# guowentian/dynamicppr

Measured on AMD Instinct MI355X. Metric: edge-updates/sec (ppr_throughput, summed over sources); ms_per_step = mean per-batch PPR update time, higher is better.
Workload: dtype f64

## Files before the change

dynamicppr_amd/csrc/dppr_engine.hip:

```cpp
#include <algorithm>
#include <atomic>
#include <cstdio>
#include <cstdlib>
#include <cstring>
#include <future>
#include <mutex>
#include <ctime>
#include <string>
#include <type_traits>
#include <unordered_map>
#include <vector>

#include <hip/hip_runtime.h>
#include <rocprim/rocprim.hpp>

#include "../../include/dppr.h"
#include "dppr_churn_plan.hpp"
#include "dppr_cut.hpp"
#include "dppr_devbuf.hpp"
#include "dppr_idspace.hpp"
#include "dppr_kernels.hpp"
#include "dppr_multi.hpp"
#include "dppr_gpush.hpp"
#include "dppr_binned.hpp"
#include "dppr_calib.hpp"
#include "dppr_topk.hpp"

using namespace dppr;

#include "dppr_host_state.hpp"
#include "dppr_host_graph.hpp"
#include "dppr_host_loop.hpp"
#include "dppr_host_group.hpp"
#include "dppr_host_query.hpp"


extern "C" {

int dppr_abi_version(void) { return DPPR_ABI_VERSION; }

const char *dppr_strerror(int status) {
    switch (status) {
    case DPPR_OK: return "ok";
    case DPPR_ERR_INVALID: return "invalid argument or call order";
    case DPPR_ERR_HIP: return "HIP runtime error";
    case DPPR_ERR_NOMEM: return "out of device memory";
    case DPPR_ERR_NO_DEVICE: return "no usable HIP device (the HIP path is mandatory; there is no CPU fallback)";
    case DPPR_ERR_NOT_CONVERGED: return "iteration cap hit before the frontier emptied";
    default: return "unknown status";
    }
}

const char *dppr_last_error(const dppr_engine *e) { return e ? e->err.c_str() : ""; }

int dppr_device_count(void) {
    int n = 0;
    return hipGetDeviceCount(&n) == hipSuccess ? n : 0;
}

int dppr_create(dppr_engine **out, int device, int32_t V, int32_t W, int directed, int32_t c, int32_t n_epochs) {
    if (!out || V <= 0 || W < 0 || c < 0 || n_epochs < 1) return DPPR_ERR_INVALID;
    *out = nullptr;
    int ndev = 0;
    if (hipGetDeviceCount(&ndev) != hipSuccess || ndev <= 0 || device < 0 || device >= ndev) return DPPR_ERR_NO_DEVICE;
    dppr_engine *e = new dppr_engine();
    dppr::g_live_engines.fetch_add(1, std::memory_order_relaxed);
    auto bail = [&](int code) {
        dppr_destroy(e);
        return code;
    };
#define HIP_TRY_C(call)                                                                 \
    do {                                                                                \
        const hipError_t _e = static_cast<hipError_t>(call);                            \
        if (_e != hipSuccess) {                                                         \
            fprintf(stderr, "dppr_create: %s at line %d\n", hipGetErrorString(_e), __LINE__); \
            return bail(_e == hipErrorOutOfMemory ? DPPR_ERR_NOMEM : DPPR_ERR_HIP);     \
        }                                                                               \
    } while (0)
    auto diag_env = [](const char *name) -> const char * {
        const char *v = getenv(name);
        if (v && !getenv("DPPR_QUIET_SWITCHES")) fprintf(stderr, "dppr_create: diagnostic switch %s=%s in effect (INTEGRATION.md, Environment variables)\n", name, v);
        return v;
    };
    if (const char *v = diag_env("DPPR_SWEEP_BITS")) e->sweep_bits = atoi(v) != 0;
    if (const char *v = diag_env("DPPR_HOT_BLOCKS")) e->hot_blocks = atoi(v) != 0;
    if (const char *v = diag_env("DPPR_GSWEEP_HOT")) e->gsweep_hot_rows = std::max(0, atoi(v));
    if (const char *v = diag_env("DPPR_GSWEEP_GRID")) e->gsweep_grid_cap = std::max(1, std::min(atoi(v), STAT_SLOTS));
    if (const char *v = diag_env("DPPR_RENUMBER")) e->renumber_on = atoi(v) != 0;
    if (const char *v = diag_env("DPPR_RENUMBER_PCT")) e->renumber_growth_pct = std::max(1, atoi(v));
    if (const char *v = diag_env("DPPR_RENUMBER_MIN")) e->renumber_min_parked = std::max(1, atoi(v));
    if (const char *v = diag_env("DPPR_GROUP_PUSH")) e->gpush_enter_pairs = std::max(-1, atoi(v));
    if (const char *v = diag_env("DPPR_GROUP_PUSH_FACTOR")) e->gpush_auto_factor = std::max(1, atoi(v));
    if (const char *v = diag_env("DPPR_GGROUPS_MIN")) e->ggroups_min = std::max(1, atoi(v));
    if (const char *v = diag_env("DPPR_COST_MODEL")) e->cost_model = atoi(v) != 0;
    if (const char *v = diag_env("DPPR_GROUPING_RADIX")) e->force_radix_grouping = atoi(v) != 0;
    if (const char *v = diag_env("DPPR_TEST_MERGE_MISS")) e->test_force_merge_miss = atoi(v) != 0;
    if (const char *v = diag_env("DPPR_BIN_INCREMENTAL")) e->bin_incremental = atoi(v) != 0;
    if (const char *v = diag_env("DPPR_BIN_RECUT_EVERY")) e->bin_recut_every = std::max(1, atoi(v));
    if (const char *v = diag_env("DPPR_BIN_FROZEN_REBUILD")) e->bin_frozen_rebuild = atoi(v) != 0;
    if (const char *v = diag_env("DPPR_GROUP_AT_SLIDE")) e->group_at_slide = atoi(v) != 0;
    if (const char *v = diag_env("DPPR_GROUP_FULL_ROWS")) e->group_full_rows = atoi(v) != 0;
    e->device = device;
    e->V = V;
    e->W = W;
    e->c = c;
    e->directed = directed ? 1 : 0;
    e->n_epochs = n_epochs;
    e->Ed = directed ? W : 2 * W;
    e->bits = 1;
    while ((1ll << e->bits) < (long long)V) e->bits++;
    HIP_TRY_C(hipSetDevice(device));
    HIP_TRY_C(hipStreamCreateWithFlags(&e->stream, hipStreamNonBlocking));
    {
        int least = 0, greatest = 0;
        if (hipDeviceGetStreamPriorityRange(&least, &greatest) != hipSuccess) least = 0;
        HIP_TRY_C(hipStreamCreateWithPriority(&e->bs, hipStreamNonBlocking, least));
    }
    HIP_TRY_C(hipEventCreate(&e->ev0));
    HIP_TRY_C(hipEventCreate(&e->ev1));
    for (auto &ev : e->evpool) HIP_TRY_C(hipEventCreate(&ev));
    HIP_TRY_C(e->dump_pin.alloc(dppr_engine::DUMP_PIN_BYTES));
    HIP_TRY_C(e->pinned.alloc((GMULTI_MAX + 2) * GS_MAX + 3 * GS_MAX + MAX_CHUNK * GS_MAX + 16));
    const size_t Wn = (size_t)std::max(W, 1), Edn = (size_t)std::max(e->Ed, 1), Ln = (size_t)std::max(4 * c, 1);
    HIP_TRY_C(e->w1.alloc(Wn));
    HIP_TRY_C(e->w2.alloc(Wn));
    HIP_TRY_C(e->outdeg.alloc((size_t)V));
    HIP_TRY_C(hipMemsetAsync(e->outdeg, 0, sizeof(int) * (size_t)V, e->stream));
    HIP_TRY_C(e->hub_slot_of.alloc((size_t)V));
    HIP_TRY_C(e->d_ext2int.alloc((size_t)V));
    HIP_TRY_C(e->d_xfer.alloc((size_t)V));
    e->init_ids(V);
    HIP_TRY_C(e->hub_hist.alloc(64));
    HIP_TRY_C(e->bar.alloc(1));
    HIP_TRY_C(e->keys_a.alloc(Edn));
    HIP_TRY_C(e->keys_b.alloc(Edn));
    HIP_TRY_C(e->in_sorted.alloc(Edn));
    if (e->directed) HIP_TRY_C(e->out_sorted.alloc(Edn));
    HIP_TRY_C(e->delpos.alloc((size_t)2 * (size_t)std::max(c, 1) + 16));
    {
        const size_t bn = (size_t)std::max(2 * c, 1);
        for (int k = 0; k < 4; ++k) {
            HIP_TRY_C(e->bk[k].alloc(bn));
            HIP_TRY_C(e->bks[k].alloc(bn));
        }
    }
    HIP_TRY_C(rocprim::radix_sort_keys(nullptr, e->sort_tmp_bytes, e->keys_a.get(), e->keys_b.get(), Edn, 0u,
                                       (unsigned)(2 * e->bits), e->stream));
    HIP_TRY_C(e->sort_tmp.alloc(std::max<size_t>(e->sort_tmp_bytes, 16)));
    for (int k = 0; k < 2; ++k) {
        HIP_TRY_C(e->su_k[k].alloc(Ln));
        HIP_TRY_C(e->su_v[k].alloc(Ln));
    }
    HIP_TRY_C(e->su_grp.alloc(4 * SU_GRP_MAX_BUCKETS + 8));
    HIP_TRY_C(hipMemsetAsync(e->su_grp, 0, sizeof(int) * (4 * SU_GRP_MAX_BUCKETS + 8), e->stream));
    HIP_TRY_C(e->su_term.alloc(Ln * GS_MAX));
    HIP_TRY_C(e->su_ins.alloc(Ln));
    HIP_TRY_C(rocprim::radix_sort_pairs(nullptr, e->su_tmp_bytes, e->su_k[0].get(), e->su_k[1].get(), e->su_v[0].get(), e->su_v[1].get(), Ln,
                                        0u, (unsigned)e->bits, e->stream));
    HIP_TRY_C(e->su_tmp.alloc(std::max<size_t>(e->su_tmp_bytes, 16)));
    e->epochs.resize((size_t)n_epochs);
    for (auto &ep : e->epochs) {
        HIP_TRY_C(ep.row_ptr.alloc((size_t)V + 1));
        HIP_TRY_C(ep.adj.alloc(Edn));
        HIP_TRY_C(ep.out_row_ptr.alloc((size_t)V + 1));
        HIP_TRY_C(ep.out_col.alloc(Edn));
        HIP_TRY_C(ep.b1.alloc(Ln));
        HIP_TRY_C(ep.b2.alloc(Ln));
        HIP_TRY_C(ep.deg_after.alloc(Ln));
        HIP_TRY_C(ep.ins.alloc(Ln));
        HIP_TRY_C(ep.sk.alloc(Ln));
        HIP_TRY_C(ep.sv.alloc(Ln));
        HIP_TRY_C(ep.grp_tile.alloc((size_t)V / WAVE + 3));
        HIP_TRY_C(ep.ggrp_tile.alloc((size_t)V / WAVE + 3));
        HIP_TRY_C(ep.hub_v.alloc(HUB_CAP));
        HIP_TRY_C(ep.hub_degp1.alloc(HUB_CAP));
    }
    HIP_TRY_C(hipStreamSynchronize(e->stream));
#undef HIP_TRY_C
    *out = e;
    return DPPR_OK;
}

void dppr_destroy(dppr_engine *e) {
    if (!e) return;
    if (e->pre.task.valid()) e->pre.task.wait();
    (void)hipSetDevice(e->device);
    if (e->stream) (void)hipStreamSynchronize(e->stream);
    if (e->bs) (void)hipStreamSynchronize(e->bs);
    if (e->ev0) (void)hipEventDestroy(e->ev0);
    if (e->ev1) (void)hipEventDestroy(e->ev1);
    for (auto &ev : e->evpool)
        if (ev) (void)hipEventDestroy(ev);
    if (e->stream) (void)hipStreamDestroy(e->stream);
    if (e->bs) (void)hipStreamDestroy(e->bs);
    dppr::g_live_engines.fetch_sub(1, std::memory_order_relaxed);
    delete e;
}

int dppr_set_schedule(dppr_engine *e, int schedule) {
    if (!e || (schedule != DPPR_SCHEDULE_EAGER && schedule != DPPR_SCHEDULE_SYNC)) return DPPR_ERR_INVALID;
    e->schedule = schedule;
    return DPPR_OK;
}

int dppr_set_batch_grouping(dppr_engine *e, int at_slide) {
    if (!e) return DPPR_ERR_INVALID;
    e->group_at_slide = at_slide != 0;
    return DPPR_OK;
}

int dppr_set_variant(dppr_engine *e, int variant) {
    if (!e || variant < 0 || variant > 3) return fail(e, DPPR_ERR_INVALID, "set_variant: 0 OPTIMIZED, 1 FAST_FRONTIER, 2 EAGER, 3 VANILLA");
    e->schedule = (variant == 1 || variant == 3) ? DPPR_SCHEDULE_SYNC : DPPR_SCHEDULE_EAGER;
    e->pre_extract = variant == 1 || variant == 3;
    e->status_dedup = variant == 2 || variant == 3;
    return DPPR_OK;
}

int dppr_set_phase_merge(dppr_engine *e, int on, int eps_divisor) {
    if (!e || eps_divisor < 0 || eps_divisor > 1024) return fail(e, DPPR_ERR_INVALID, "set_phase_merge: eps_divisor 1..1024 (0 keeps it)");
    e->merge_phases = on != 0;
    if (eps_divisor > 0) e->merge_div = eps_divisor;
    return DPPR_OK;
}

int dppr_set_profiling(dppr_engine *e, int on) {
    if (!e) return DPPR_ERR_INVALID;
    e->profiling = on != 0;
    return DPPR_OK;
}

int dppr_set_persistent(dppr_engine *e, int mode, int64_t timeout_us) {
    if (!e || mode < 0 || mode > 2 || e->loaded || !e->slots.empty())
        return fail(e, DPPR_ERR_INVALID, "set_persistent: call right after dppr_create, mode 0, 1 or 2");
    e->persist_mode = mode;
    if (timeout_us > 0) e->persist_ticks = (unsigned long long)timeout_us * 100ull;
    if (timeout_us < 0) {
        e->persist_ticks = 20000ull;
        e->persist_rollcall_extra = 1;
    }
    return DPPR_OK;
}

int dppr_set_tuning(dppr_engine *e, int hub_min_degree, int big_row_edges, int pull_min_frontier, int chunk_iters,
                    int pull_block) {
    if (!e || hub_min_degree < 1 || big_row_edges < 1 || e->loaded || !e->slots.empty())
        return fail(e, DPPR_ERR_INVALID, "set_tuning: call right after dppr_create, values >= 1");
    e->hub_min_degree = hub_min_degree;
    e->big_row = big_row_edges;
    e->pull_min_frontier = pull_min_frontier;
    if (chunk_iters > 0) {
        e->chunk_iters = std::min(chunk_iters, MAX_CHUNK);
        e->chunk_explicit = true;
    }
    if (pull_block >= 256 && pull_block <= 1024 && pull_block % 64 == 0) e->pull_block = pull_block;
    return DPPR_OK;
}

int dppr_set_sweep_bitmap(dppr_engine *e, int on) {
    if (!e) return DPPR_ERR_INVALID;
    e->sweep_bits = on != 0;
    return DPPR_OK;
}

int dppr_set_binned_sweep(dppr_engine *e, int mode, int ha_tiles, int hb_tiles, int64_t target_edges, int64_t min_ids, int64_t chunk_edges,
                          int64_t target_a_edges) {
    if (!e || mode < 0 || mode > 2 || ha_tiles < 0 || ha_tiles > BIN_MAX_HA_TILES || hb_tiles < 0 || hb_tiles > BIN_MAX_HB_TILES || target_edges < 0 || min_ids < 0 ||
        chunk_edges < 0 || target_a_edges < 0 || e->bin_ready || e->loaded)
        return fail(e, DPPR_ERR_INVALID, "set_binned_sweep: call right after dppr_create; mode 0..2, ha_tiles <= 272, hb_tiles <= 120");
    e->bin_mode = mode;
    if (ha_tiles > 0) e->bin_ha_tiles = ha_tiles;
    if (hb_tiles > 0) e->bin_hb_tiles = hb_tiles;
    if (target_edges > 0) e->bin_target = target_edges;
    if (min_ids > 0) e->bin_min_ids = min_ids;
    if (chunk_edges > 0) e->bin_chunk = chunk_edges;
    if (target_a_edges > 0) e->bin_target_a = target_a_edges;
    return DPPR_OK;
}

int dppr_set_resident_slots(dppr_engine *e, int sorted) {
    if (!e) return DPPR_ERR_INVALID;
    e->res_slots = sorted != 0;
    if (!e->res_slots)
        for (auto &ep : e->epochs) ep.res_valid = false;
    return DPPR_OK;
}

int dppr_set_resident_update(dppr_engine *e, int on) {
    if (!e) return DPPR_ERR_INVALID;
    e->res_update = on != 0;
    if (!e->res_update)
        for (auto &ep : e->epochs) ep.su_inline = false;
    return DPPR_OK;
}

int dppr_set_group_resident(dppr_engine *e, int on) {
    if (!e) return DPPR_ERR_INVALID;
    e->group_resident = on != 0;
    return DPPR_OK;
}

int dppr_set_group_push(dppr_engine *e, int enter_pairs, int list_cap, int64_t max_edges) {
    if (!e || enter_pairs < -1 || list_cap < 0 || max_edges < 0) return fail(e, DPPR_ERR_INVALID, "set_group_push: bad argument");
    e->gpush_enter_pairs = enter_pairs;
    if (list_cap > 0) e->gpush_list_cap = list_cap;
    e->gpush_max_edges = max_edges;
    return DPPR_OK;
}

int dppr_set_group_seeding(dppr_engine *e, int from_tails) {
    if (!e) return DPPR_ERR_INVALID;
    e->group_tail_seeding = from_tails != 0;
    return DPPR_OK;
}

int dppr_set_renumbering(dppr_engine *e, int on, int growth_pct, int min_parked) {
    if (!e || growth_pct < 0 || min_parked < 0) return fail(e, DPPR_ERR_INVALID, "set_renumbering: bad argument");
    e->renumber_on = on != 0;
    if (growth_pct > 0) e->renumber_growth_pct = growth_pct;
    if (min_parked > 0) e->renumber_min_parked = min_parked;
    e->renumber_next = std::min(e->renumber_next, renumber_threshold(e->n_int, e->renumber_growth_pct));
    return DPPR_OK;
}

int dppr_id_space(dppr_engine *e, int32_t *n_ids, int32_t *n_parked, int32_t *renumberings, int64_t *revivals) {
    if (!e) return DPPR_ERR_INVALID;
    if (n_ids) *n_ids = e->n_int;
    if (n_parked) *n_parked = e->n_parked;
    if (renumberings) *renumberings = e->renumberings;
    if (revivals) *revivals = e->revivals;
    return DPPR_OK;
}

int dppr_set_incremental_graph(dppr_engine *e, int on) {
    if (!e) return DPPR_ERR_INVALID;
    e->incremental = on != 0;
    return DPPR_OK;
}

int dppr_synchronize(dppr_engine *e) {
    if (!e) return DPPR_ERR_INVALID;
    HIP_TRY(hipSetDevice(e->device));
    HIP_TRY(hipStreamSynchronize(e->stream));
    HIP_TRY(hipStreamSynchronize(e->bs));
    return DPPR_OK;
}

int dppr_load_window(dppr_engine *e, const int32_t *e1, const int32_t *e2, int32_t n) {
    if (!e || n != e->W || (n > 0 && (!e1 || !e2))) return fail(e, DPPR_ERR_INVALID, "load_window: n must equal W");
    HIP_TRY(hipSetDevice(e->device));
    {
        std::vector<std::pair<uint64_t, int32_t>> fresh;
        for (int k = 0; k < 2; ++k) {
            const int32_t *a = k ? e2 : e1;
            for (int i = 0; i < n; ++i) {
                const int v = a[i];
                if (v < 0 || v >= e->V) return fail(e, DPPR_ERR_INVALID, "load_window: vertex id out of range");
                if (e->ext2int[(size_t)v] == -1) {
                    e->ext2int[(size_t)v] = -2;
                    fresh.emplace_back(id_hash(v), v);
                }
            }
        }
        std::vector<int32_t> indeg;
        if (fresh.size() > HOT_WINDOW_MIN) {
            indeg.assign((size_t)e->V, 0);
            for (int i = 0; i < n; ++i) {
                indeg[(size_t)e2[i]]++;
                if (!e->directed) indeg[(size_t)e1[i]]++;
            }
        }
        numbering_order(fresh, indeg.empty() ? nullptr : indeg.data(), e->hot_blocks);
        for (auto &kv : fresh) {
            e->ext2int[(size_t)kv.second] = -1;
            (void)to_int(e, kv.second);
        }
    }
    if (!translate(e, e1, n, e->h_tmp1) || !translate(e, e2, n, e->h_tmp2))
        return fail(e, DPPR_ERR_INVALID, "load_window: vertex id out of range");
    if (n > 0) {
        HIP_TRY(hipMemcpyAsync(e->w1, e->h_tmp1.data(), sizeof(int) * (size_t)n, hipMemcpyHostToDevice, e->bs));
        HIP_TRY(hipMemcpyAsync(e->w2, e->h_tmp2.data(), sizeof(int) * (size_t)n, hipMemcpyHostToDevice, e->bs));
    }
    e->head = 0;
    HIP_TRY(hipMemsetAsync(e->outdeg, 0, sizeof(int) * (size_t)e->V, e->bs));
    if (n > 0) {
        hipLaunchKernelGGL(k_deg_update, dim3(grid_for(n)), dim3(BLOCK), 0, e->bs, e->w1, e->w2, n, e->directed, 1,
                           e->outdeg);
        HIP_TRY(hipGetLastError());
    }
    for (auto &ep : e->epochs) ep.id = -1;
    Epoch &ep = e->epochs[0];
    ep.L = 0;
    ep.grouped = false;
    ep.su_inline = false;
    int rc = query_persist_cap(e);
    if (rc) return rc;
    rc = sort_window_full(e);
    if (rc) return rc;
    rc = build_epoch(e, ep);
    if (rc) return rc;
    ep.id = 0;
    e->newest = 0;
    e->renumber_next = renumber_threshold(e->n_int, e->renumber_growth_pct);
    e->loaded = true;
    e->batch_staged = false;
    HIP_TRY(hipStreamSynchronize(e->bs));
    return DPPR_OK;
}

int dppr_hint_next_batch(dppr_engine *e, const int32_t *b1, const int32_t *b2, int32_t L, const int32_t *n1, const int32_t *n2, int32_t c) {
    if (!e || e->broken || L < 0 || L > 4 * e->c || c < 0 || c > e->c || (L > 0 && (!b1 || !b2)) || (c > 0 && (!n1 || !n2))) return DPPR_ERR_INVALID;
    pre_join(e);
    dppr_engine::Pre &pr = e->pre;
    const int32_t *src[4] = {b1, b2, n1, n2};
    const int n[4] = {L, L, c, c};
    for (int k = 0; k < 4; ++k) {
        pr.src[k] = src[k];
        pr.n[k] = n[k];
        pr.out[k].resize((size_t)std::max(n[k], 1));
    }
    pr.epoch = e->renumber_epoch;
    pr.armed = true;
    pr.ok = false;
    pr.task = std::async(std::launch::async, [e] {
        bool ok = true;
        for (int k = 0; k < 4; ++k)
            if (e->pre.n[k] > 0) ok = e->lookup_only(e->pre.src[k], (size_t)e->pre.n[k], e->pre.out[k].data(), e->pre.miss[k]) && ok;
        return ok;
    });
    return DPPR_OK;
}

int dppr_set_batch(dppr_engine *e, const int32_t *b1, const int32_t *b2, const uint8_t *ins, int32_t L) {
    if (!e || e->broken || L < 0 || L > 4 * e->c || (L > 0 && (!b1 || !b2 || !ins)))
        return fail(e, DPPR_ERR_INVALID, "set_batch: length exceeds 4*max_batch");
    std::lock_guard<std::mutex> map_lk(e->map_mu);
    if (!ids_in_range(e, b1, L) || !ids_in_range(e, b2, L) || !translate(e, b1, L, e->st_b1) || !translate(e, b2, L, e->st_b2))
        return fail(e, DPPR_ERR_INVALID, "set_batch: vertex id out of range");
    e->st_b1.resize((size_t)L);
    e->st_b2.resize((size_t)L);
    e->st_ins.assign(ins, ins + L);
    e->batch_staged = true;
    HIP_TRY(hipSetDevice(e->device));
    return flush_moves(e);
}

static int slide_impl(dppr_engine *e, const int32_t *n1, const int32_t *n2, int32_t c, int32_t *out_epoch);

int dppr_slide(dppr_engine *e, const int32_t *n1, const int32_t *n2, int32_t c, int32_t *out_epoch) {
    if (e) e->build_concurrent = false;
    return slide_impl(e, n1, n2, c, out_epoch);
}

int dppr_slide_concurrent(dppr_engine *e, const int32_t *n1, const int32_t *n2, int32_t c, int32_t *out_epoch) {
    if (!e || e->n_epochs < 2) return fail(e, DPPR_ERR_INVALID, "slide_concurrent: needs n_epochs >= 2 (the epoch being built must not be the one being solved)");
    e->build_concurrent = true;
    const int rc = slide_impl(e, n1, n2, c, out_epoch);
    e->build_concurrent = false;
    return rc;
}

int dppr_renumbering_due(const dppr_engine *e) {
    return e && e->renumber_on && e->W > 0 && e->n_int >= e->renumber_next ? 1 : 0;
}

static int slide_impl(dppr_engine *e, const int32_t *n1, const int32_t *n2, int32_t c, int32_t *out_epoch) {
    if (!e || e->broken || !e->loaded || c < 0 || c > e->W || c > e->c || (c > 0 && (!n1 || !n2)))
        return fail(e, DPPR_ERR_INVALID, "slide: window not loaded, or c exceeds the window / max_batch of dppr_create");
    if (!ids_in_range(e, n1, c) || !ids_in_range(e, n2, c))
        return fail(e, DPPR_ERR_INVALID, "slide: vertex id out of range");
    HIP_TRY(hipSetDevice(e->device));
    const int W = e->W;
    static const bool slide_trace = getenv("DPPR_SLIDE_TRACE") != nullptr;
    timespec t_mark;
    clock_gettime(CLOCK_MONOTONIC, &t_mark);
    auto mark = [&](const char *what) {
        if (!slide_trace) return;
        (void)hipStreamSynchronize(e->bs);
        timespec now;
        clock_gettime(CLOCK_MONOTONIC, &now);
        fprintf(stderr, "[slide] %-34s %8.1f us\n", what, (now.tv_sec - t_mark.tv_sec) * 1e6 + (now.tv_nsec - t_mark.tv_nsec) * 1e-3);
        t_mark = now;
    };
    bool renumbered = false;
    {
        std::lock_guard<std::mutex> map_lk(e->map_mu);
        if (int rc = compact_ids(e, &renumbered)) return rc;
        if (renumbered) e->bin_words_valid = false;
        mark("renumbering check");
        if (!translate(e, n1, c, e->h_tmp1) || !translate(e, n2, c, e->h_tmp2))
            return fail(e, DPPR_ERR_INVALID, "slide: vertex id out of range");
        if (int rc = flush_moves(e)) return rc;
    }
    mark("translate new edges");
    n1 = e->h_tmp1.data();
    n2 = e->h_tmp2.data();
    const bool inc = e->incremental && c > 0 && 2 * c <= e->Ed && !renumbered;
    const int per = e->directed ? 1 : 2;
    int done = 0;
    while (done < c) {
        const int pos = (e->head + done) % W;
        const int len = std::min(c - done, W - pos);
        hipLaunchKernelGGL(k_deg_update, dim3(grid_for(len)), dim3(BLOCK), 0, e->bs, e->w1 + pos, e->w2 + pos, len,
                           e->directed, -1, e->outdeg);
        if (inc)
            hipLaunchKernelGGL(k_make_keys_seg, dim3(grid_for(len)), dim3(BLOCK), 0, e->bs, e->w1 + pos, e->w2 + pos,
                               len, e->directed, e->bits, e->bk[0] + (size_t)done * per, e->bk[2] + done);
        HIP_TRY(hipMemcpyAsync(e->w1 + pos, n1 + done, sizeof(int) * (size_t)len, hipMemcpyHostToDevice, e->bs));
        HIP_TRY(hipMemcpyAsync(e->w2 + pos, n2 + done, sizeof(int) * (size_t)len, hipMemcpyHostToDevice, e->bs));
        hipLaunchKernelGGL(k_deg_update, dim3(grid_for(len)), dim3(BLOCK), 0, e->bs, e->w1 + pos, e->w2 + pos, len,
                           e->directed, 1, e->outdeg);
        if (inc)
            hipLaunchKernelGGL(k_make_keys_seg, dim3(grid_for(len)), dim3(BLOCK), 0, e->bs, e->w1 + pos, e->w2 + pos,
                               len, e->directed, e->bits, e->bk[1] + (size_t)done * per, e->bk[3] + done);
        HIP_TRY(hipGetLastError());
        done += len;
    }
    if (W > 0) e->head = (e->head + c) % W;
    mark("ring, degrees, batch keys");
    const int id = e->newest + 1;
    Epoch &ep = e->epochs[id % e->n_epochs];
    ep.id = -1;
    ep.L = 0;
    ep.grouped = false;
    ep.su_inline = false;
    int rc;
    e->merge_miss_host = 0;
    if (inc) {
        HIP_TRY(hipMemsetAsync(e->hub_hist + MERGE_MISS_WORD, 0, sizeof(int), e->bs));
        rc = merge_batch_keys(e, e->in_sorted, e->bk[0], e->bks[0], c * per, e->bk[1], e->bks[1], c * per);
        if (!rc && e->directed) rc = merge_batch_keys(e, e->out_sorted, e->bk[2], e->bks[2], c, e->bk[3], e->bks[3], c);
        if (!rc) HIP_TRY(hipMemcpyAsync(&e->merge_miss_host, e->hub_hist + MERGE_MISS_WORD, sizeof(int), hipMemcpyDeviceToHost, e->bs));
    } else {
        rc = sort_window_full(e);
    }
    if (rc) return rc;
    mark("sorted keys (merge / full sort)");
    BinBatch bb;
    if (inc) {
        bb.del = e->bk[0];
        bb.ins = e->bk[1];
        bb.nd = bb.ni = c * per;
    }
    rc = build_epoch(e, ep, inc ? &bb : nullptr);
    if (rc) return rc;
    HIP_TRY(hipStreamSynchronize(e->bs));
    if (inc && (e->merge_miss_host != 0 || e->test_force_merge_miss)) {
        e->bin_force_full = true;
        e->merge_fallbacks++;
        rc = sort_window_full(e);
        if (rc) return rc;
        rc = build_epoch(e, ep);
        if (rc) return rc;
    }
    mark("hubs, CSRs, group cut + tables");
    ep.L = 0;
    ep.grouped = false;
    ep.max_bucket = 0;
    if (e->batch_staged) {
        const int L = (int)e->st_b1.size();
        ep.L = L;
        ep.max_bucket = largest_bucket(e->st_b1.data(), L);
        if (L > 0) {
            HIP_TRY(hipMemcpyAsync(ep.b1, e->st_b1.data(), sizeof(int) * (size_t)L, hipMemcpyHostToDevice, e->bs));
            HIP_TRY(hipMemcpyAsync(ep.b2, e->st_b2.data(), sizeof(int) * (size_t)L, hipMemcpyHostToDevice, e->bs));
            HIP_TRY(hipMemcpyAsync(ep.ins, e->st_ins.data(), (size_t)L, hipMemcpyHostToDevice, e->bs));
            if (e->group_at_slide) {
                hipLaunchKernelGGL(k_gather_deg, dim3(grid_for(L)), dim3(BLOCK), 0, e->bs, ep.b1, L, e->outdeg,
                                   ep.deg_after);
                HIP_TRY(hipGetLastError());
                if (int grc = epoch_group_records(e, ep)) return grc;
            }
        }
    }
    HIP_TRY(hipStreamSynchronize(e->bs));
    mark("batch records");
    e->batch_staged = false;
    ep.id = id;
    e->newest = id;
    if (out_epoch) *out_epoch = id;
    return DPPR_OK;
}

int dppr_add_source(dppr_engine *e, int32_t source, int32_t *out_slot) {
    if (!e || e->broken || source < 0 || source >= e->V) return fail(e, DPPR_ERR_INVALID, "add_source: vertex out of range");
    HIP_TRY(hipSetDevice(e->device));
    Slot s;
    s.source_ext = source;
    s.source = to_int(e, source);
    source = s.source;
    if (int rc = flush_moves(e)) return rc;
    const size_t V = (size_t)e->V;
    HIP_TRY(s.p.alloc(V));
    HIP_TRY(s.r.alloc(V));
    HIP_TRY(s.x.alloc(V));
    HIP_TRY(s.x2.alloc(V));
    HIP_TRY(hipMemsetAsync(s.x, 0, sizeof(double) * V, e->stream));
    HIP_TRY(hipMemsetAsync(s.x2, 0, sizeof(double) * V, e->stream));
    s.act_bytes = (V / 32 + 64) * sizeof(uint32_t);
    HIP_TRY(s.act[0].alloc(s.act_bytes / sizeof(uint32_t)));
    HIP_TRY(s.act[1].alloc(s.act_bytes / sizeof(uint32_t)));
    HIP_TRY(hipMemsetAsync(s.act[0], 0, s.act_bytes, e->stream));
    HIP_TRY(hipMemsetAsync(s.act[1], 0, s.act_bytes, e->stream));
    HIP_TRY(s.ft[0].alloc(V));
    HIP_TRY(s.ft[1].alloc(V));
    HIP_TRY(s.neg.alloc((size_t)std::max(4 * e->c, 1)));
    HIP_TRY(s.cnt.alloc(CNT_HDR + 2 * MAX_CHUNK));
    s.log = s.cnt + CNT_HDR;
// ... 516 lines not shown
    s.trace = on != 0;
    s.trace_ids.clear();
    s.trace_off.assign(1, 0);
    return DPPR_OK;
}

int dppr_trace_get(dppr_engine *e, int32_t slot, int64_t *n_iters, int64_t *n_ids, int64_t *offsets, int32_t *ids) {
    GET_SLOT(e, slot);
    const int64_t ni = s.trace_off.empty() ? 0 : (int64_t)s.trace_off.size() - 1;
    if (n_iters) *n_iters = ni;
    if (n_ids) *n_ids = (int64_t)s.trace_ids.size();
    if (offsets && !s.trace_off.empty()) memcpy(offsets, s.trace_off.data(), sizeof(int64_t) * s.trace_off.size());
    if (ids && !s.trace_ids.empty()) memcpy(ids, s.trace_ids.data(), sizeof(int32_t) * s.trace_ids.size());
    return DPPR_OK;
}

#define GET_GROUP(e, gid)                                                                             \
    if (!(e) || (gid) < 0 || (gid) >= (int)(e)->groups.size()) return fail((e), DPPR_ERR_INVALID, "bad group"); \
    if ((e)->broken) return fail((e), DPPR_ERR_INVALID, "engine unusable after a failed renumbering");           \
    Group &g = (e)->groups[(size_t)(gid)]

int dppr_add_source_group(dppr_engine *e, const int32_t *sources, int32_t n, int32_t *out_group) {
    if (!e || e->broken || !sources || n < 1 || n > GS_MAX) return fail(e, DPPR_ERR_INVALID, "add_source_group: 1..16 sources");
    if (!ids_in_range(e, sources, n)) return fail(e, DPPR_ERR_INVALID, "add_source_group: vertex out of range");
    HIP_TRY(hipSetDevice(e->device));
    Group g;
    g.n = n;
    g.gw = e->group_full_rows ? (n > OCT ? 2 * OCT : OCT) : row_width(n);
    g.spl = row_spl(g.gw);
    for (int s = 0; s < GS_MAX; ++s) g.src.s[s] = -1;
    for (int s = 0; s < n; ++s) g.src_ext[s] = sources[s];
    const size_t V = (size_t)e->V;
    g.act_bytes = (V / 32 + 1024 / 32 + 4) * sizeof(uint32_t);
    const size_t xw = (size_t)x_stride(g.gw);
    HIP_TRY_MSG("add_source_group: ", g.p.alloc((size_t)g.gw * V));
    HIP_TRY_MSG("add_source_group: ", g.r.alloc((size_t)g.gw * V));
    HIP_TRY_MSG("add_source_group: ", g.x.alloc(xw * V));
    HIP_TRY_MSG("add_source_group: ", g.x2.alloc(xw * V));
    HIP_TRY_MSG("add_source_group: ", g.act[0].alloc(g.act_bytes / sizeof(uint32_t)));
    HIP_TRY_MSG("add_source_group: ", g.act[1].alloc(g.act_bytes / sizeof(uint32_t)));
    HIP_TRY_MSG("add_source_group: ", g.cnt.alloc(5 * GS_MAX + MAX_CHUNK * GS_MAX));
    HIP_TRY_MSG("add_source_group: ", g.mlog.alloc((size_t)(GMULTI_MAX + 2) * GS_MAX));
    HIP_TRY_MSG("add_source_group: ", g.dstats.alloc(2));
    HIP_TRY_MSG("add_source_group: ", g.gq.alloc(3 * GQ_PAD));
    HIP_TRY_MSG("add_source_group: ", hipMemsetAsync(g.gq, 0, sizeof(int) * 3 * GQ_PAD, e->stream));
    HIP_TRY_MSG("add_source_group: ", hipMemsetAsync(g.act[0], 0, g.act_bytes, e->stream));
    HIP_TRY_MSG("add_source_group: ", hipMemsetAsync(g.act[1], 0, g.act_bytes, e->stream));
    HIP_TRY_MSG("add_source_group: ", hipMemsetAsync(g.cnt, 0, sizeof(int) * (5 * GS_MAX + MAX_CHUNK * GS_MAX), e->stream));
    HIP_TRY_MSG("add_source_group: ", hipMemsetAsync(g.dstats, 0, 2 * sizeof(IterStats), e->stream));
    for (int s = 0; s < n; ++s) (void)to_int(e, sources[s]);
    for (int s = 0; s < n; ++s) g.src.s[s] = e->ext2int[(size_t)sources[s]];
    if (int rc = flush_moves(e)) return rc;
    hipLaunchKernelGGL(k_ginit, dim3(grid_for((int64_t)e->V * g.gw)), dim3(BLOCK), 0, e->stream, g.p, g.r, e->V, g.gw, g.src);
    HIP_TRY_MSG("add_source_group: ", hipGetLastError());
    HIP_TRY_MSG("add_source_group: ", hipStreamSynchronize(e->stream));
    if (g.spl == 2) e->wide_groups = true;
    e->groups.push_back(std::move(g));
    e->any_groups = true;
    if (int rc = recut_stale_groups(e)) return rc;
    if (out_group) *out_group = (int)e->groups.size() - 1;
    return DPPR_OK;
}

int dppr_group_init_solve(dppr_engine *e, int32_t group, double eps, float *out_ms) {
    return dppr_group_init_solve_at(e, group, -1, eps, out_ms);
}

int dppr_group_init_solve_at(dppr_engine *e, int32_t group, int32_t epoch, double eps, float *out_ms) {
    GET_GROUP(e, group);
    GET_EPOCH(e, epoch);
    if (!(eps > 0)) return fail(e, DPPR_ERR_INVALID, "eps must be positive");
    HIP_TRY(hipSetDevice(e->device));
    HIP_TRY(hipEventRecord(e->ev0, e->stream));
    hipLaunchKernelGGL(k_ginit, dim3(grid_for((int64_t)e->V * g.gw)), dim3(BLOCK), 0, e->stream, g.p, g.r, e->V, g.gw, g.src);
    HIP_TRY(hipGetLastError());
    g.converged = false;
    g.park_eps = 0.0;
    int rc = group_loop(e, g, ep, 0, eps, false);
    if (rc) return rc;
    HIP_TRY(hipEventRecord(e->ev1, e->stream));
    HIP_TRY(hipEventSynchronize(e->ev1));
    float ms = 0;
    HIP_TRY(hipEventElapsedTime(&ms, e->ev0, e->ev1));
    if (out_ms) *out_ms = ms;
    g.converged = true;
    g.conv_eps = eps;
    g.last_epoch = ep.id;
    return DPPR_OK;
}

int dppr_group_update(dppr_engine *e, int32_t group, int32_t epoch, double eps, float *out_ms) {
    GET_GROUP(e, group);
    GET_EPOCH(e, epoch);
    if (!(eps > 0)) return fail(e, DPPR_ERR_INVALID, "eps must be positive");
    if (!epoch_in_sequence(g.last_epoch, ep.id)) return fail(e, DPPR_ERR_INVALID, "epoch out of sequence for this group");
    HIP_TRY(hipSetDevice(e->device));
    const bool merged = e->merge_phases && e->schedule == DPPR_SCHEDULE_EAGER;
    if (merged) eps = eps / e->merge_div;
    const bool tails = g.converged && g.conv_eps <= eps && e->group_tail_seeding;
    int rc = settle_parked(e, g.p, g.r, g.gw, eps, &g.park_eps, &g.st);
    if (rc) return rc;
    rc = prepare_epoch(e, ep);
    if (rc) return rc;
    HIP_TRY(hipEventRecord(e->ev0, e->stream));
    rc = group_stream_update(e, g, ep);
    if (rc) return rc;
    g.converged = false;
    if (merged) {
        rc = group_loop(e, g, ep, PHASE_BOTH, eps, tails);
        if (rc) return rc;
    } else {
        rc = group_loop(e, g, ep, 0, eps, tails);
        if (rc) return rc;
        rc = group_loop(e, g, ep, 1, eps, tails);
        if (rc) return rc;
    }
    HIP_TRY(hipEventRecord(e->ev1, e->stream));
    HIP_TRY(hipEventSynchronize(e->ev1));
    float ms = 0;
    HIP_TRY(hipEventElapsedTime(&ms, e->ev0, e->ev1));
    if (out_ms) *out_ms = ms;
    g.st.gpu_ms += ms;
    g.st.batches++;
    g.converged = true;
    g.conv_eps = eps;
    g.last_epoch = ep.id;
    return DPPR_OK;
}

int dppr_group_read(dppr_engine *e, int32_t group, int32_t index, double *p, double *r) {
    GET_GROUP(e, group);
    if (index < 0 || index >= g.n) return fail(e, DPPR_ERR_INVALID, "group_read: bad source index");
    HIP_TRY(hipSetDevice(e->device));
    std::lock_guard<std::mutex> map_lk(e->map_mu);
    int rc = sync_map(e);
    if (rc) return rc;
    const double *src[2] = {g.p, g.r};
    double *dst[2] = {p, r};
    for (int k = 0; k < 2; ++k) {
        if (!dst[k]) continue;
        hipLaunchKernelGGL(k_gint_to_ext, dim3(grid_for(e->V)), dim3(BLOCK), 0, e->stream, src[k], g.gw, index, e->d_ext2int,
                           e->V, e->d_xfer);
        HIP_TRY(hipMemcpyAsync(dst[k], e->d_xfer, sizeof(double) * (size_t)e->V, hipMemcpyDeviceToHost, e->stream));
        HIP_TRY(hipStreamSynchronize(e->stream));
    }
    return DPPR_OK;
}

static_assert(CHURN_LANES == GS_MAX, "dppr_churn_plan.hpp plans for the group size of dppr_multi.hpp");
static constexpr bool churn_geometry_agrees() {
    for (int n = 1; n <= GS_MAX; ++n)
        if (churn_row_width(n, false) != row_width(n) || churn_row_spl(row_width(n)) != row_spl(row_width(n)) ||
            churn_row_width(n, true) != (n > OCT ? 2 * OCT : OCT))
            return false;
    return true;
}
static_assert(churn_geometry_agrees(), "dppr_churn_plan.hpp restates row_width / row_spl of dppr_multi.hpp");

int dppr_group_sources(dppr_engine *e, int32_t group, int32_t *out_sources, int32_t *out_n) {
    GET_GROUP(e, group);
    if (out_sources)
        for (int s = 0; s < g.n; ++s) out_sources[s] = g.src_ext[s];
    if (out_n) *out_n = g.n;
    return DPPR_OK;
}

static int group_churn(dppr_engine *e, int32_t group, ChurnOp op, int32_t index, int32_t new_source, int32_t *out_index, float *out_ms) {
    static const char *const what[3] = {"group_replace_source", "group_add_source", "group_remove_source"};
    auto refuse = [&](const char *why) { return fail(e, DPPR_ERR_INVALID, (std::string(what[op]) + ": " + why).c_str()); };
    GET_GROUP(e, group);
    const ChurnPlan pl = churn_plan(op, g.n, g.gw, index, e->group_full_rows, e->wide_groups);
    if (!pl.ok) return refuse(op == CHURN_ADD ? "the group holds 16 sources" : op == CHURN_REMOVE && g.n <= 1 ? "the last source of a group cannot be removed" : "bad source index");
    if (op != CHURN_REMOVE && (new_source < 0 || new_source >= e->V)) return refuse("vertex out of range");
    if (!g.converged || g.last_epoch < 0) return refuse("the group is not converged (solve or update it first)");
    Epoch *epp = find_epoch(e, g.last_epoch);
    if (!epp) return refuse("the epoch the group was last solved on is not resident any more");
    const Epoch &ep = *epp;
    HIP_TRY(hipSetDevice(e->device));
    const size_t V = (size_t)e->V;
    const bool new_x = x_stride(pl.gw) != x_stride(g.gw);
    DevBuf<double> p2, r2, x_new, x2_new;
    if (pl.relayout) {
        HIP_TRY(p2.alloc((size_t)pl.gw * V));
        HIP_TRY(r2.alloc((size_t)pl.gw * V));
    }
    if (new_x) {
        HIP_TRY(x_new.alloc((size_t)x_stride(pl.gw) * V));
        HIP_TRY(x2_new.alloc((size_t)x_stride(pl.gw) * V));
    }
    int src_int = -1;
    if (op != CHURN_REMOVE) {
        (void)to_int(e, new_source);
        if (int rc = flush_moves(e)) return rc;
        src_int = e->ext2int[(size_t)new_source];
        if (pl.recut) e->wide_groups = true;
        if (int rc = recut_stale_groups(e)) return rc;
    }
    HIP_TRY(hipEventRecord(e->ev0, e->stream));
    if (pl.relayout) {
        ColMap cm;
        for (int s = 0; s < GS_MAX; ++s) cm.m[s] = pl.map[s];
        const int grid = grid_for((int64_t)e->V, BLOCK / pl.gw);
        hipLaunchKernelGGL(k_grow_remap, dim3(grid), dim3(BLOCK), 0, e->stream, p2.get(), g.p.get(), e->V, pl.gw, g.gw, cm);
        hipLaunchKernelGGL(k_grow_remap, dim3(grid), dim3(BLOCK), 0, e->stream, r2.get(), g.r.get(), e->V, pl.gw, g.gw, cm);
        HIP_TRY(hipGetLastError());
        g.p.swap(p2);
        g.r.swap(r2);
    }
    if (new_x) {
        g.x.swap(x_new);
        g.x2.swap(x2_new);
    }
    SrcN src;
    int src_ext[GS_MAX] = {0};
    for (int s = 0; s < GS_MAX; ++s) {
        src.s[s] = s < pl.n && pl.map[s] >= 0 ? g.src.s[pl.map[s]] : -1;
        src_ext[s] = s < pl.n && pl.map[s] >= 0 ? g.src_ext[pl.map[s]] : 0;
    }
    if (pl.lane >= 0) {
        src.s[pl.lane] = src_int;
        src_ext[pl.lane] = new_source;
    }
    g.src = src;
    memcpy(g.src_ext, src_ext, sizeof(src_ext));
    g.n = pl.n;
    g.gw = pl.gw;
    g.spl = pl.spl;
    if (pl.lane >= 0) {
        hipLaunchKernelGGL(k_gcol_init, dim3(grid_for(e->V)), dim3(BLOCK), 0, e->stream, g.p.get(), g.r.get(), e->V, g.gw, pl.lane, src_int);
        HIP_TRY(hipGetLastError());
        g.converged = false;
        if (int rc = group_solve_column(e, g, ep)) return rc;
    }
    HIP_TRY(hipEventRecord(e->ev1, e->stream));
    HIP_TRY(hipEventSynchronize(e->ev1));
    float ms = 0;
    HIP_TRY(hipEventElapsedTime(&ms, e->ev0, e->ev1));
    if (out_ms) *out_ms = ms;
    if (out_index) *out_index = pl.lane;
    g.converged = true;
    return DPPR_OK;
}

int dppr_group_replace_source(dppr_engine *e, int32_t group, int32_t index, int32_t new_source, float *out_ms) {
    return group_churn(e, group, CHURN_REPLACE, index, new_source, nullptr, out_ms);
}

int dppr_group_add_source(dppr_engine *e, int32_t group, int32_t new_source, int32_t *out_index, float *out_ms) {
    return group_churn(e, group, CHURN_ADD, -1, new_source, out_index, out_ms);
}

int dppr_group_remove_source(dppr_engine *e, int32_t group, int32_t index) {
    return group_churn(e, group, CHURN_REMOVE, index, -1, nullptr, nullptr);
}

static bool topk_args_ok(int32_t k, double min_p, const void *ids, const void *p, const void *cnt) {
    return k >= 1 && k <= DPPR_TOPK_MAX && min_p >= 0.0 && ids && p && cnt;
}
static bool read_at_args_ok(const dppr_engine *e, const int32_t *ids, int32_t m) {
    if (m < 0 || (m > 0 && !ids)) return false;
    for (int32_t i = 0; i < m; ++i)
        if (ids[i] < 0 || ids[i] >= e->V) return false;
    return true;
}

int dppr_topk(dppr_engine *e, int32_t slot, int32_t k, double min_p, int32_t *out_ids, double *out_p, double *out_r,
              int32_t *out_count) {
    GET_SLOT(e, slot);
    if (!topk_args_ok(k, min_p, out_ids, out_p, out_count))
        return fail(e, DPPR_ERR_INVALID, "topk: k in [1, DPPR_TOPK_MAX], min_p >= 0, non-null ids / p / count");
    std::lock_guard<std::mutex> map_lk(e->map_mu);
    return run_topk(e, s.p, s.r, 1, 1, k, min_p, out_ids, out_p, out_r, out_count);
}

int dppr_group_topk(dppr_engine *e, int32_t group, int32_t k, double min_p, int32_t *out_ids, double *out_p, double *out_r,
                    int32_t *out_counts) {
    GET_GROUP(e, group);
    if (!topk_args_ok(k, min_p, out_ids, out_p, out_counts))
        return fail(e, DPPR_ERR_INVALID, "group_topk: k in [1, DPPR_TOPK_MAX], min_p >= 0, non-null ids / p / counts");
    std::lock_guard<std::mutex> map_lk(e->map_mu);
    return run_topk(e, g.p, g.r, g.gw, g.n, k, min_p, out_ids, out_p, out_r, out_counts);
}

int dppr_read_at(dppr_engine *e, int32_t slot, const int32_t *ids, int32_t m, double *out_p, double *out_r) {
    GET_SLOT(e, slot);
    if (!read_at_args_ok(e, ids, m)) return fail(e, DPPR_ERR_INVALID, "read_at: ids in [0, V)");
    if (m == 0 || (!out_p && !out_r)) return DPPR_OK;
    std::lock_guard<std::mutex> map_lk(e->map_mu);
    return run_read_at(e, s.p, s.r, 1, 1, ids, m, out_p, out_r);
}

int dppr_group_read_at(dppr_engine *e, int32_t group, const int32_t *ids, int32_t m, double *out_p, double *out_r) {
    GET_GROUP(e, group);
    if (!read_at_args_ok(e, ids, m)) return fail(e, DPPR_ERR_INVALID, "group_read_at: ids in [0, V)");
    if (m == 0 || (!out_p && !out_r)) return DPPR_OK;
    std::lock_guard<std::mutex> map_lk(e->map_mu);
    return run_read_at(e, g.p, g.r, g.gw, g.n, ids, m, out_p, out_r);
}

int dppr_group_reset_stats(dppr_engine *e, int32_t group) {
    GET_GROUP(e, group);
    HIP_TRY(hipSetDevice(e->device));
    g.st = dppr_stats_t{};
    HIP_TRY(hipMemsetAsync(g.dstats, 0, 2 * sizeof(IterStats), e->stream));
    HIP_TRY(hipStreamSynchronize(e->stream));
    return DPPR_OK;
}

int dppr_group_stats(dppr_engine *e, int32_t group, dppr_stats_t *out) {
    GET_GROUP(e, group);
    if (!out) return DPPR_ERR_INVALID;
    HIP_TRY(hipSetDevice(e->device));
    static thread_local IterStats h[2];
    HIP_TRY(hipMemcpyAsync(h, g.dstats, sizeof(h), hipMemcpyDeviceToHost, e->stream));
    HIP_TRY(hipStreamSynchronize(e->stream));
    unsigned long long t = 0, ts = 0;
    for (int i = 0; i < STAT_SLOTS; ++i) {
        t += h[0].blk_E[i];
        ts += h[1].blk_E[i];
    }
    g.st.sum_E = (int64_t)(t + ts);
    g.st.sweep_E = (int64_t)ts;
    g.st.sum_N = g.st.sum_F;
    g.st.algorithmic_bytes = 8ll * g.st.inspected + 45ll * g.st.records + 72ll * g.st.sum_F + 24ll * g.st.sum_E +
                             4ll * g.st.sum_N;
    *out = g.st;
    return DPPR_OK;
}

#ifdef DPPR_STAMPS
extern "C" int dppr_debug_bin_stamps(unsigned long long *out, int which, int rows) {
    return hipMemcpyFromSymbol(out, HIP_SYMBOL(dppr::g_bin_stamps), sizeof(unsigned long long) * 6 * (size_t)rows,
                               sizeof(unsigned long long) * 6 * 16384 * (size_t)which) == hipSuccess ? 0 : -2;
}
extern "C" int dppr_debug_stamps(unsigned long long *out, int rows) {
    return hipMemcpyFromSymbol(out, HIP_SYMBOL(dppr::g_stamps), sizeof(unsigned long long) * 8 * (size_t)rows) == hipSuccess
               ? 0 : -2;
}
#endif

int dppr_bench_atomics(int device, int64_t table_elems, int64_t n, int scope, int reps, float *out_ms) {
    if (table_elems <= 0 || (table_elems & (table_elems - 1)) || n <= 0 || reps <= 0 || !out_ms) return DPPR_ERR_INVALID;
    int ndev = 0;
    if (hipGetDeviceCount(&ndev) != hipSuccess || device < 0 || device >= ndev) return DPPR_ERR_NO_DEVICE;
    if (hipSetDevice(device) != hipSuccess) return DPPR_ERR_HIP;
    DevBuf<double> table, sink;
    hipEvent_t a, b;
    if (table.alloc((size_t)table_elems) != 0) return DPPR_ERR_NOMEM;
    (void)sink.alloc(1);
    (void)hipMemset(table, 0, sizeof(double) * (size_t)table_elems);
    (void)hipEventCreate(&a);
    (void)hipEventCreate(&b);
    const int grid = 2048;
    auto launch = [&]() {
        if (scope == 2)
            hipLaunchKernelGGL(k_bench_scatter<0>, dim3(grid), dim3(BLOCK), 0, 0, table, (uint64_t)table_elems - 1, n);
        else if (scope == 3)
            hipLaunchKernelGGL(k_bench_scatter<1>, dim3(grid), dim3(BLOCK), 0, 0, table, (uint64_t)table_elems - 1, n);
        else if (scope == 0)
            hipLaunchKernelGGL(k_bench_atomics<__HIP_MEMORY_SCOPE_AGENT>, dim3(grid), dim3(BLOCK), 0, 0, table,
                               (uint64_t)table_elems - 1, n, sink);
        else
            hipLaunchKernelGGL(k_bench_atomics<__HIP_MEMORY_SCOPE_WORKGROUP>, dim3(grid), dim3(BLOCK), 0, 0, table,
                               (uint64_t)table_elems - 1, n, sink);
    };
    launch();
    (void)hipEventRecord(a, 0);
    for (int i = 0; i < reps; ++i) launch();
    (void)hipEventRecord(b, 0);
    hipError_t err = hipEventSynchronize(b);
    float ms = 0;
    (void)hipEventElapsedTime(&ms, a, b);
    *out_ms = ms / reps;
    (void)hipEventDestroy(a);
    (void)hipEventDestroy(b);
    return err == hipSuccess ? DPPR_OK : DPPR_ERR_HIP;
}

int dppr_bench_line_fills(int device, int64_t table_bytes, int64_t lines, int reps, float *out_ms) {
    if (table_bytes < 128 || (table_bytes & (table_bytes - 1)) || lines <= 0 || reps <= 0 || !out_ms) return DPPR_ERR_INVALID;
    int ndev = 0;
    if (hipGetDeviceCount(&ndev) != hipSuccess || device < 0 || device >= ndev) return DPPR_ERR_NO_DEVICE;
    if (hipSetDevice(device) != hipSuccess) return DPPR_ERR_HIP;
    DevBuf<double2> table;
    DevBuf<double> sink;
    if (table.alloc((size_t)table_bytes / sizeof(double2)) != 0) return DPPR_ERR_NOMEM;
    (void)sink.alloc(1);
    (void)hipMemset(table, 0, (size_t)table_bytes);
    hipEvent_t a, b;
    (void)hipEventCreate(&a);
    (void)hipEventCreate(&b);
    const int grid = 2048;
    const int per = (int)std::max<int64_t>(8, (lines + (int64_t)grid * 128 - 1) / ((int64_t)grid * 128) / 8 * 8);
    auto launch = [&]() {
        hipLaunchKernelGGL(k_bench_lines<8>, dim3(grid), dim3(1024), 0, 0, table, (uint64_t)(table_bytes / 128) - 1, per, sink);
    };
    launch();
    (void)hipEventRecord(a, 0);
    for (int i = 0; i < reps; ++i) launch();
    (void)hipEventRecord(b, 0);
    hipError_t err = hipEventSynchronize(b);
    float ms = 0;
    (void)hipEventElapsedTime(&ms, a, b);
    *out_ms = ms / reps * (float)((double)lines / ((double)grid * 128.0 * per));
    (void)hipEventDestroy(a);
    (void)hipEventDestroy(b);
    return err == hipSuccess ? DPPR_OK : DPPR_ERR_HIP;
}

int dppr_bench_stream_copy(int device, int64_t bytes, int reps, float *out_ms) {
    if (bytes < 16 || reps <= 0 || !out_ms) return DPPR_ERR_INVALID;
    int ndev = 0;
    if (hipGetDeviceCount(&ndev) != hipSuccess || device < 0 || device >= ndev) return DPPR_ERR_NO_DEVICE;
    if (hipSetDevice(device) != hipSuccess) return DPPR_ERR_HIP;
    DevBuf<unsigned char> src, dst;
    if (src.alloc((size_t)bytes) != 0 || dst.alloc((size_t)bytes) != 0) return DPPR_ERR_NOMEM;
    (void)hipMemset(src, 0, (size_t)bytes);
    (void)hipMemset(dst, 0, (size_t)bytes);
    hipEvent_t a, b;
    (void)hipEventCreate(&a);
    (void)hipEventCreate(&b);
    auto launch = [&]() { hipLaunchKernelGGL(k_bench_copy, dim3(4096), dim3(1024), 0, 0, reinterpret_cast<const double2 *>(src.get()),
                                            reinterpret_cast<double2 *>(dst.get()), bytes / 16); };
    launch();
    (void)hipEventRecord(a, 0);
    for (int i = 0; i < reps; ++i) launch();
    (void)hipEventRecord(b, 0);
    hipError_t err = hipEventSynchronize(b);
    float ms = 0;
    (void)hipEventElapsedTime(&ms, a, b);
    *out_ms = ms / reps;
    (void)hipEventDestroy(a);
    (void)hipEventDestroy(b);
    return err == hipSuccess ? DPPR_OK : DPPR_ERR_HIP;
}

int dppr_debug_bin_tables(dppr_engine *e, int32_t epoch, int32_t *n_a, int32_t *n_b, int32_t *n_edges, int32_t *n_runs, int32_t *n_tiles,
                          int32_t *acut, int32_t *bcut, uint16_t *hl, int32_t *tdelta, int32_t *tb, uint16_t *dl, int32_t *vb,
                          int64_t *patched, int64_t *rebuilt) {
    if (!e) return DPPR_ERR_INVALID;
    GET_EPOCH(e, epoch);
    if (patched) *patched = e->bin_patched;
    if (rebuilt) *rebuilt = e->bin_rebuilt;
    if (!ep.bin_valid) return fail(e, DPPR_ERR_INVALID, "debug_bin_tables: this epoch has no binned tables");
    HIP_TRY(hipSetDevice(e->device));
    if (n_a) *n_a = ep.n_a;
    if (n_b) *n_b = ep.n_b;
    if (n_edges) *n_edges = ep.Ed;
    if (n_runs) *n_runs = ep.n_runs;
    if (n_tiles) *n_tiles = ep.n_tiles;
    const size_t n_blk = ((size_t)ep.Ed + WAVE - 1) / WAVE, n_rb = ((size_t)ep.n_runs + WAVE - 1) / WAVE;
    if (acut) HIP_TRY(hipMemcpy(acut, ep.acut, sizeof(int) * ((size_t)ep.n_a + 1), hipMemcpyDeviceToHost));
    if (bcut) HIP_TRY(hipMemcpy(bcut, ep.bcut, sizeof(int) * ((size_t)ep.n_b + 1), hipMemcpyDeviceToHost));
    if (hl) HIP_TRY(hipMemcpy(hl, ep.hl, sizeof(uint16_t) * (size_t)ep.n_runs, hipMemcpyDeviceToHost));
    if (tdelta) HIP_TRY(hipMemcpy(tdelta, ep.tdelta, sizeof(int) * (size_t)ep.n_tiles, hipMemcpyDeviceToHost));
    if (tb) HIP_TRY(hipMemcpy(tb, ep.tb, sizeof(int) * (n_rb + 1), hipMemcpyDeviceToHost));
    if (dl) HIP_TRY(hipMemcpy(dl, ep.dl, sizeof(uint16_t) * (size_t)ep.Ed, hipMemcpyDeviceToHost));
    if (vb) HIP_TRY(hipMemcpy(vb, ep.vb, sizeof(int) * (n_blk + 1), hipMemcpyDeviceToHost));
    return DPPR_OK;
}

int dppr_debug_live_bytes(int64_t *device_bytes, int64_t *pinned_bytes) {
    if (device_bytes) *device_bytes = dppr::g_device_bytes.load(std::memory_order_relaxed);
    if (pinned_bytes) *pinned_bytes = dppr::g_pinned_bytes.load(std::memory_order_relaxed);
    return DPPR_OK;
}

unsigned long long dppr_heartbeat(const dppr_engine *e) { return e ? e->heartbeat.load(std::memory_order_relaxed) : 0ull; }

#ifndef DPPR_BUILD_ID
#define DPPR_BUILD_ID "unstamped"
#endif
const char *dppr_build_id(void) { return DPPR_BUILD_ID; }

}
```

dynamicppr_amd/csrc/dppr_host_group.hpp:

```cpp
#pragma once

namespace {

template <int N> using IC = std::integral_constant<int, N>;
template <class F>
void with_row(int gw, F &&f) {
    switch (gw) {
    case 2: f(IC<1>{}, IC<2>{}); break;
    case 4: f(IC<1>{}, IC<4>{}); break;
    case 6: f(IC<1>{}, IC<6>{}); break;
    case 8: f(IC<1>{}, IC<8>{}); break;
    case 10: f(IC<2>{}, IC<10>{}); break;
    case 12: f(IC<2>{}, IC<12>{}); break;
    case 14: f(IC<2>{}, IC<14>{}); break;
    default: f(IC<2>{}, IC<16>{}); break;
    }
}

int group_multi_capacity(dppr_engine *e, int spl) {
    int &cap = e->gmulti_cap[spl - 1];
    if (cap < 0) {
        int per_cu = 0, cus = 0;
        hipError_t rc = spl == 1 ? hipOccupancyMaxActiveBlocksPerMultiprocessor(&per_cu, k_gsweep<1, 8, 1024, true, 2>, GNT, 0)
                                 : hipOccupancyMaxActiveBlocksPerMultiprocessor(&per_cu, k_gsweep<2, 16, 512, true, 2>, GNT, 0);
        if (rc != hipSuccess || hipDeviceGetAttribute(&cus, hipDeviceAttributeMultiprocessorCount, e->device) != hipSuccess)
            per_cu = 0;
        cap = std::min(per_cu * cus, STAT_SLOTS);
    }
    return cap;
}

int group_push_tail(dppr_engine *e, Group &g, const Epoch &ep, int phase, double eps, long long pairs_at_entry, int *iters, bool *entered,
                    bool *converged, bool *owed) {
    *entered = false;
    *converged = false;
    const int GWM = GS_MAX;
    const int cap = std::max(1024, std::min(e->gpush_list_cap, e->V));
    if (g.plist[0].capacity() != (size_t)cap || !g.pctl) {
        HIP_TRY(loop_wait(e));
        g.plist[0].reset(); g.plist[1].reset(); g.ppre.reset(); g.pctl.reset();
        HIP_TRY(g.plist[0].alloc((size_t)cap));
        HIP_TRY(g.plist[1].alloc((size_t)cap));
        HIP_TRY(g.ppre.alloc((size_t)cap + 1));
        HIP_TRY(g.pctl.alloc(1));
    }
    static thread_local GPushCtl h;
    HIP_TRY(hipMemsetAsync(g.pctl, 0, sizeof(GPushCtl), e->stream));
    const int n_words = (ep.grp_n_int + 31) / 32;
    hipLaunchKernelGGL(k_gpush_list, dim3(grid_for(n_words)), dim3(BLOCK), 0, e->stream, g.act[0], n_words, g.plist[0], cap, g.pctl);
    const int rows_grid = grid_for(std::min<long long>(pairs_at_entry, cap), BLOCK / OCT);
    with_row(g.gw, [&](auto spl, auto gw) {
        hipLaunchKernelGGL((k_gpush_rows<decltype(spl)::value, decltype(gw)::value>), dim3(rows_grid), dim3(BLOCK), 0, e->stream, g.plist[0],
                           g.pctl, 0, g.x, g.r, false);
    });
    HIP_TRY(hipGetLastError());
    *entered = true;
    const int credit_first = *owed ? 1 : 0;
    const long long max_edges = e->gpush_max_edges > 0 ? e->gpush_max_edges : std::max<long long>(4096, 20ll * std::max(ep.n_ggroups, 1));
    const int grid = 256;
    static const bool trace = getenv("DPPR_GROUP_TRACE") != nullptr;
    int it_done = 0;
    long long known_n = pairs_at_entry;
    bool tiny_declined = false;
    long long last_adds = pairs_at_entry <= 64 ? 0 : -1;
    for (;;) {
        if (known_n <= TINY_N && last_adds >= 0 && last_adds <= TINY_E / 2 && !tiny_declined) {
            with_row(g.gw, [&](auto spl, auto gw) {
                hipLaunchKernelGGL((k_gpush_tiny<decltype(spl)::value, decltype(gw)::value>), dim3(1), dim3(1024), 0, e->stream, g.pctl, g.plist[0],
                                   g.plist[1], ep.row_ptr, ep.adj, ep.hub_degp1, g.r, g.p, g.act[0], phase, eps, g.dstats, GPUSH_LOG, credit_first);
            });
        } else {
        int m = 2;
        if (it_done == 0)
            for (long long f = pairs_at_entry; f > 128 && m < GPUSH_LOG; f >>= 2) ++m;
        tiny_declined = false;
        for (int k = 0; k < m; ++k) {
            hipLaunchKernelGGL(k_gpush_scan, dim3(1), dim3(1024), 0, e->stream, g.pctl, g.plist[0], g.plist[1], ep.row_ptr, g.ppre, cap - 1, max_edges);
            with_row(g.gw, [&](auto spl, auto gw) {
                constexpr int SPL = decltype(spl)::value, GW = decltype(gw)::value;
                hipLaunchKernelGGL((k_gpush_snap<SPL, GW>), dim3(grid), dim3(BLOCK), 0, e->stream, g.plist[0], g.plist[1], g.pctl, g.x, g.r, g.p,
                                   g.act[0], phase, eps, credit_first);
                hipLaunchKernelGGL((k_gpush_expand<SPL, GW>), dim3(grid), dim3(BLOCK), 0, e->stream, g.plist[0], g.plist[1], g.pctl, g.ppre,
                                   ep.row_ptr, ep.adj, ep.hub_degp1, g.x, g.r, g.act[0], g.plist[0], g.plist[1], cap, phase, eps, g.dstats);
            });
        }
        }
        HIP_TRY(hipGetLastError());
        HIP_TRY(hipMemcpyAsync(&h, g.pctl, sizeof(GPushCtl), hipMemcpyDeviceToHost, e->stream));
        HIP_TRY(loop_wait(e));
        for (int i = it_done; i < h.it; ++i) {
            long long F = 0;
            for (int s = 0; s < GWM; ++s) F += h.F[i & (GPUSH_LOG - 1)][s];
            if (F == 0) continue;
            g.st.iterations++;
            g.st.sum_F += F;
            ++*iters;
            if (trace)
                fprintf(stderr, "[gpush ] phase %d iteration +%d  frontier pairs %9lld  adds %lld\n", phase, i, F, h.atomics[i & (GPUSH_LOG - 1)]);
        }
        if (h.it == it_done && !h.stop && known_n <= TINY_N) tiny_declined = true;
        if (h.it > it_done) last_adds = h.atomics[(h.it - 1) & (GPUSH_LOG - 1)];
        it_done = h.it;
        known_n = h.n[h.it & 1];
        if (h.stop && h.it == 0 && h.overflow) {
            *entered = false;
            return DPPR_OK;
        }
        if (h.stop) {
            if (trace) fprintf(stderr, "[gpush ] phase %d: an iteration of %d vertices called itself off after %d iterations\n", phase, h.n[h.it & 1], h.it);
            HIP_TRY(hipMemsetAsync(g.cnt, 0, sizeof(int) * 3 * GWM, e->stream));
            with_row(g.gw, [&](auto spl, auto gw) {
                hipLaunchKernelGGL((k_gpush_leave<decltype(spl)::value, decltype(gw)::value>), dim3(grid_for(ep.grp_n_int, BLOCK / OCT)), dim3(BLOCK), 0,
                                   e->stream, ep.grp_n_int, g.act[0], g.x, g.r, g.p, h.it > 0 ? 1 : 0, phase, eps, g.cnt);
            });
            HIP_TRY(hipGetLastError());
            if (h.it > 0) *owed = false;
            return DPPR_OK;
        }
        if (h.n[h.it & 1] == 0) {
            *converged = true;
            return DPPR_OK;
        }
        if (it_done >= e->max_iters) return fail(e, DPPR_ERR_NOT_CONVERGED, "iteration cap hit");
    }
}

int group_loop(dppr_engine *e, Group &g, const Epoch &ep, int phase, double eps, bool tails) {
    const int hp = phase == PHASE_BOTH ? 0 : phase;
    int cur = 0;
    const int GWM = GS_MAX;
    HIP_TRY(hipMemsetAsync(g.cnt, 0, sizeof(int) * 3 * GWM, e->stream));
    if (tails) {
        HIP_TRY(hipMemsetAsync(g.act[0], 0, g.act_bytes, e->stream));
        if (ep.L > 0) {
            with_row(g.gw, [&](auto spl, auto gw) {
                hipLaunchKernelGGL((k_gseed_tails<decltype(spl)::value, decltype(gw)::value>), dim3(grid_for(ep.L, BLOCK / OCT)), dim3(BLOCK), 0,
                                   e->stream, batch_tails(e, ep), ep.L, g.r, g.x, g.p, g.act[0], phase, eps, g.cnt + cur * GWM);
            });
        }
    } else {
        with_row(g.gw, [&](auto spl, auto gw) {
            hipLaunchKernelGGL((k_gseed_dense<decltype(spl)::value, decltype(gw)::value>), dim3(grid_for(ep.grp_n_int, BLOCK / OCT)), dim3(BLOCK), 0,
                               e->stream, ep.grp_n_int, g.r, g.x, g.p, g.act[0], phase, eps, g.cnt + cur * GWM);
        });
        g.st.inspected += (int64_t)ep.grp_n_int * g.n;
    }
    HIP_TRY(hipGetLastError());
    int *log = g.cnt + 5 * GWM;
    auto any_left = [&](const int *c) {
        for (int s = 0; s < GWM; ++s)
            if (c[s] > 0) return true;
        return false;
    };
    HIP_TRY(hipMemcpyAsync(e->pinned, g.cnt + cur * GWM, sizeof(int) * GWM, hipMemcpyDeviceToHost, e->stream));
    HIP_TRY(loop_wait(e));
    bool more = any_left(e->pinned);
    int active_iters = 0;
    if (e->gsweep_grid_cap <= 0) {
        int cus = 0;
        if (hipDeviceGetAttribute(&cus, hipDeviceAttributeMultiprocessorCount, e->device) != hipSuccess || cus <= 0) cus = 256;
        e->gsweep_grid_cap = std::min(2 * cus, STAT_SLOTS);
    }
    const int sweep_grid = std::min(std::max(ep.n_ggroups, 1), e->gsweep_grid_cap);
    int follow = 4;
    bool owed = false;
    long long push_thr = e->gpush_enter_pairs == 0 ? 0 : e->gpush_enter_pairs > 0 ? e->gpush_enter_pairs : std::max(64, ep.n_ggroups * e->gpush_auto_factor);
    bool push_gave_up = false;
    int dense_len = -1;
    const int nvx = ep.ggrp_max_tiles * WAVE;
    for (int it = 0; more;) {
        if (it >= e->max_iters) return fail(e, DPPR_ERR_NOT_CONVERGED, "iteration cap hit");
        const int mcap = e->group_resident && e->persist_mode && e->persist_ok && e->chunk_iters > 1 ? group_multi_capacity(e, g.spl) : 0;
        if (mcap > 0 && ep.n_ggroups > 0 && ep.n_ggroups <= mcap) {
            int n = g.iter_hint[hp] > it ? g.iter_hint[hp] - it + RESIDENT_MARGIN : 2 * e->chunk_iters;
            n = std::max(2, std::min(n, GMULTI_MAX));
            if (e->chunk_explicit) n = std::min(n, std::max(e->chunk_iters, 2));
            HIP_TRY(hipMemsetAsync(g.mlog, 0, sizeof(int) * (size_t)(n + 2) * GWM, e->stream));
            HIP_TRY(hipMemsetAsync(e->bar, 0, sizeof(GridBar), e->stream));
            if (e->profiling) HIP_TRY(hipEventRecord(e->evpool[0], e->stream));
            int *status = g.mlog, *rows = g.mlog + GWM;
#define DPPR_LAUNCH_GMULTI(SPL, GW, NVX)                                                                                 \
    hipLaunchKernelGGL((k_gsweep<SPL, GW, NVX, true, 2>), dim3(ep.n_ggroups), dim3(GNT), 0, e->stream, ep.grp_n_int, ep.gtab,   \
                       ep.n_ggroups, g.cnt + cur * GWM, e->gsweep_hot_rows, ep.out_col, g.x, g.x2, g.act[0], g.act[1], g.r, g.p, \
                       g.cnt + 3 * GWM, g.cnt + 4 * GWM, phase, eps, g.dstats + 1, rows, n, e->bar, status, e->persist_ticks,    \
                       e->persist_rollcall_extra, owed ? 1 : 0, (int *)nullptr, (int *)nullptr)
            with_row(g.gw, [&](auto spl, auto gw) {
                constexpr int SPL = decltype(spl)::value, GW = decltype(gw)::value;
                if constexpr (SPL == 2) DPPR_LAUNCH_GMULTI(2, GW, 512);
                else if (nvx == 512) DPPR_LAUNCH_GMULTI(1, GW, 512);
                else DPPR_LAUNCH_GMULTI(1, GW, 1024);
            });
#undef DPPR_LAUNCH_GMULTI
            if (e->profiling) HIP_TRY(hipEventRecord(e->evpool[1], e->stream));
            HIP_TRY(hipGetLastError());
            HIP_TRY(hipMemcpyAsync(e->pinned, g.mlog, sizeof(int) * (size_t)(n + 2) * GWM, hipMemcpyDeviceToHost, e->stream));
            HIP_TRY(loop_wait(e));
            const int st = e->pinned[0];
            g.st.persist_launches++;
            if (st & GSM_FAULT) return fail(e, DPPR_ERR_HIP, "a grid barrier of the multi-sweep group launch timed out");
            if (st & GSM_ABORTED) {
                g.st.persist_aborts++;
                e->persist_ok = false;
                e->persist_retry = PERSIST_RETRY_BATCHES;
                continue;
            }
            const int sweeps = st & GSM_SWEEPS;
            for (int k = 0; k < sweeps; ++k) {
                const int *f = e->pinned + GWM + k * GWM;
                g.st.iterations++;
                g.st.pull_iterations++;
                for (int s = 0; s < GWM; ++s) g.st.sum_F += f[s];
                for (int s = 0; s < GWM; ++s) g.st.sweep_F += f[s];
                active_iters = it + k + 1;
            }
            if (e->profiling) {
                float ms = 0;
                HIP_TRY(hipEventElapsedTime(&ms, e->evpool[0], e->evpool[1]));
                g.st.push_ms += ms;
                g.st.push_launches++;
            }
            if (sweeps & 1) {
                std::swap(g.x, g.x2);
                std::swap(g.act[0], g.act[1]);
                owed = !owed;
            }
            it += sweeps;
            if (st & GSM_CONVERGED) break;
            HIP_TRY(hipMemcpyAsync(g.cnt, g.cnt + 3 * GWM, sizeof(int) * GWM, hipMemcpyDeviceToDevice, e->stream));
            HIP_TRY(hipMemsetAsync(g.cnt + GWM, 0, sizeof(int) * 2 * GWM, e->stream));
            cur = 0;
            more = any_left(e->pinned + GWM + sweeps * GWM);
            continue;
        }
        int n;
        if (it == 0) {
            int lo = 0;
            for (int h : (push_thr > 0 ? g.dense_hist : g.iter_hist)[hp]) lo = h > 0 && (lo == 0 || h < lo) ? h : lo;
            n = lo > 0 ? lo : e->chunk_iters;
            follow = 4;
        } else if (push_thr > 0 && !push_gave_up) {
            long long F = 0;
            for (int s = 0; s < GWM; ++s) F += e->pinned[cur * GWM + s];
            n = 1;
            for (long long f = F / 4; f > push_thr && n < e->chunk_iters; f /= 4) ++n;
        } else {
            n = std::min(follow, e->chunk_iters);
            follow *= 2;
        }
        if (e->chunk_explicit) n = std::min(n, std::max(e->chunk_iters, 1));
        n = std::max(1, std::min(n, MAX_CHUNK));
        for (int k = 0; k < n; ++k) {
            const int nxt = (cur + 1) % 3, zer = (cur + 2) % 3;
            if (e->profiling) HIP_TRY(hipEventRecord(e->evpool[2 * k], e->stream));
#define DPPR_LAUNCH_GSWEEP(SPL, GW, NVX) do { if (owed) DPPR_LAUNCH_GSWEEP_CM(SPL, GW, NVX, 1); else DPPR_LAUNCH_GSWEEP_CM(SPL, GW, NVX, 0); } while (0)
#define DPPR_LAUNCH_GSWEEP_CM(SPL, GW, NVX, CM)                                                                          \
    hipLaunchKernelGGL((k_gsweep<SPL, GW, NVX, false, CM>), dim3(sweep_grid), dim3(GNT), 0, e->stream, ep.grp_n_int, ep.gtab,  \
                       ep.n_ggroups, g.cnt + cur * GWM, e->gsweep_hot_rows, ep.out_col, g.x, g.x2, g.act[0], g.act[1], g.r, g.p,  \
                       g.cnt + nxt * GWM, g.cnt + zer * GWM, phase, eps, g.dstats + 1, log + k * GWM, 1, (GridBar *)nullptr,      \
                       (int *)nullptr, 0ull, 0, owed ? 1 : 0, g.gq + (g.gq_seq % 3) * GQ_PAD, g.gq + ((g.gq_seq + 1) % 3) * GQ_PAD)
            with_row(g.gw, [&](auto spl, auto gw) {
                constexpr int SPL = decltype(spl)::value, GW = decltype(gw)::value;
                if constexpr (SPL == 2) DPPR_LAUNCH_GSWEEP(2, GW, 512);
                else if (nvx == 512) DPPR_LAUNCH_GSWEEP(1, GW, 512);
                else DPPR_LAUNCH_GSWEEP(1, GW, 1024);
            });
#undef DPPR_LAUNCH_GSWEEP
#undef DPPR_LAUNCH_GSWEEP_CM
            if (e->profiling) HIP_TRY(hipEventRecord(e->evpool[2 * k + 1], e->stream));
            std::swap(g.x, g.x2);
            std::swap(g.act[0], g.act[1]);
            cur = nxt;
            g.gq_seq++;
            owed = !owed;
        }
        HIP_TRY(hipGetLastError());
        HIP_TRY(hipMemcpyAsync(e->pinned, g.cnt, sizeof(int) * (size_t)(5 * GWM + n * GWM), hipMemcpyDeviceToHost,
                               e->stream));
        HIP_TRY(loop_wait(e));
        for (int k = 0; k < n; ++k) {
            const int *f = e->pinned + 5 * GWM + k * GWM;
            if (!any_left(f)) continue;
            if (push_thr > 0 && dense_len < 0) {
                long long F = 0;
                for (int s = 0; s < GWM; ++s) F += f[s];
                if (F <= push_thr) dense_len = it + k;
            }
            g.st.iterations++;
            g.st.pull_iterations++;
            for (int s = 0; s < GWM; ++s) g.st.sum_F += f[s];
            for (int s = 0; s < GWM; ++s) g.st.sweep_F += f[s];
            active_iters = it + k + 1;
            if (e->profiling) {
                float ms = 0;
                HIP_TRY(hipEventElapsedTime(&ms, e->evpool[2 * k], e->evpool[2 * k + 1]));
                g.st.push_ms += ms;
                g.st.push_launches++;
                g.st.sweep_ms += ms;
                g.st.sweep_launches++;
                static const bool trace = getenv("DPPR_GROUP_TRACE") != nullptr;
                if (trace) {
                    long long F = 0;
                    for (int s = 0; s < GWM; ++s) F += f[s];
                    fprintf(stderr, "[gsweep] phase %d sweep %3d  frontier pairs %9lld  %7.1f us\n", phase, it + k, F, ms * 1e3);
                }
            }
        }
        more = any_left(e->pinned + cur * GWM);
        it += n;
        if (more && push_thr > 0 && !push_gave_up) {
            long long F = 0;
            for (int s = 0; s < GWM; ++s) F += e->pinned[cur * GWM + s];
            if (F <= push_thr) {
                if (dense_len < 0) dense_len = it;
                int pushed = 0;
                bool entered = false, conv = false;
                int rc = group_push_tail(e, g, ep, phase, eps, F, &pushed, &entered, &conv, &owed);
                if (rc) return rc;
                if (entered) {
                    active_iters = it + pushed;
                    it += pushed;
                    if (conv) more = false;
                    else {
                        cur = 0;
                        HIP_TRY(hipMemcpyAsync(e->pinned, g.cnt, sizeof(int) * GWM, hipMemcpyDeviceToHost, e->stream));
                        HIP_TRY(loop_wait(e));
                        more = any_left(e->pinned);
                        push_thr = std::max<long long>(F / 8, 1);
                        dense_len = -1;
                    }
                } else {
                    push_thr = std::max<long long>(F / 8, 1);
                    dense_len = -1;
                }
            }
        }
    }
    if (push_thr > 0) {
        for (int k = 3; k > 0; --k) g.dense_hist[hp][k] = g.dense_hist[hp][k - 1];
        g.dense_hist[hp][0] = dense_len >= 0 ? std::max(dense_len, 1) : std::max(active_iters, 1);
    }
    g.iter_hint[hp] = active_iters;
    for (int k = 3; k > 0; --k) g.iter_hist[hp][k] = g.iter_hist[hp][k - 1];
    g.iter_hist[hp][0] = active_iters;
    return DPPR_OK;
}

int group_solve_column(dppr_engine *e, Group &g, const Epoch &ep) {
    int hint[2], hist[2][4], dense[2][4];
    memcpy(hint, g.iter_hint, sizeof(hint));
    memcpy(hist, g.iter_hist, sizeof(hist));
    memcpy(dense, g.dense_hist, sizeof(dense));
    const int rc = group_loop(e, g, ep, 0, g.conv_eps, false);
    memcpy(g.iter_hint, hint, sizeof(hint));
    memcpy(g.iter_hist, hist, sizeof(hist));
    memcpy(g.dense_hist, dense, sizeof(dense));
    return rc;
}

int group_stream_update(dppr_engine *e, Group &g, const Epoch &ep) {
    const int L = ep.L;
    if (L == 0) return DPPR_OK;
    int rc = group_records_by_tail(e, ep, nullptr, 0, nullptr, 0);
    if (rc) return rc;
    SuSources srcs{};
    for (int s = 0; s < GS_MAX; ++s) srcs.s[s] = g.src.s[s];
    hipLaunchKernelGGL(k_su_terms, dim3(grid_for(L), g.n), dim3(BLOCK), 0, e->stream, batch_tails(e, ep), batch_order(e, ep), ep.b2,
                       ep.ins, L, g.p, g.gw, e->su_term, e->su_ins);
    hipLaunchKernelGGL(k_su_apply, dim3(grid_for(L), g.n), dim3(BLOCK), 0, e->stream, batch_tails(e, ep), batch_order(e, ep), e->su_term,
                       e->su_ins, ep.deg_after, L, g.r, g.gw, srcs, 0.0, (int *)nullptr, (int *)nullptr, (int *)nullptr,
                       (int *)nullptr);
    HIP_TRY(hipGetLastError());
    g.st.records += (int64_t)L * g.n;
    return DPPR_OK;
}

}
```

dynamicppr_amd/csrc/dppr_host_state.hpp:

```cpp
#pragma once

static constexpr int MAX_CHUNK = 64;
static constexpr int CNT_HDR = 16;
static constexpr int PERSIST_RETRY_BATCHES = 64;
static constexpr int GMULTI_MAX = 2 * MAX_CHUNK;
static constexpr int GQ_PAD = 32;
static constexpr int BIN_MAX_BLOCKS = 1 << 16, BIN_MAX_BIG = 4096, BIN_SMALL_INTS = BIN_MAX_BLOCKS + BIN_MAX_BIG + 1 + 64;
static constexpr int SU_SPLIT_MIN = 1 << 16;
static constexpr int MERGE_MISS_WORD = 44;
static constexpr int RESIDENT_MARGIN = 8;

namespace dppr {

inline std::atomic<long long> g_device_bytes{0}, g_pinned_bytes{0};

struct DeviceAlloc {
    static int alloc(void **p, size_t bytes) {
        const hipError_t rc = hipMalloc(p, bytes);
        if (rc == hipSuccess) g_device_bytes.fetch_add((long long)bytes, std::memory_order_relaxed);
        return (int)rc;
    }
    static int free(void *p, size_t bytes) {
        g_device_bytes.fetch_sub((long long)bytes, std::memory_order_relaxed);
        return (int)hipFree(p);
    }
};

struct PinnedAlloc {
    static int alloc(void **p, size_t bytes) {
        const hipError_t rc = hipHostMalloc(p, bytes, hipHostMallocDefault);
        if (rc == hipSuccess) g_pinned_bytes.fetch_add((long long)bytes, std::memory_order_relaxed);
        return (int)rc;
    }
    static int free(void *p, size_t bytes) {
        g_pinned_bytes.fetch_sub((long long)bytes, std::memory_order_relaxed);
        return (int)hipHostFree(p);
    }
};

template <class T> using DevBuf = Buf<T, DeviceAlloc>;
template <class T> using PinBuf = Buf<T, PinnedAlloc>;

}

namespace {

struct Epoch {
    DevBuf<int> row_ptr;
    DevBuf<Adj> adj;
    DevBuf<int> out_row_ptr;
    DevBuf<int> out_col;
    int Ed = 0;
    DevBuf<int> b1, b2, deg_after;
    DevBuf<uint8_t> ins;
    int L = 0;
    DevBuf<uint32_t> sk, sv;
    int max_bucket = 0;
    bool grouped = false;
    int id = -1;
    DevBuf<int> grp_tile;
    int n_groups = 0;
    int grp_n_int = 0;
    DevBuf<int> ggrp_tile;
    int n_ggroups = 0;
    int ggrp_max_tiles = 0;
    DevBuf<int> gtab;
    DevBuf<int> hub_v, hub_degp1;
    int n_hubs = 0;
    DevBuf<int> acut; int *bcut = nullptr;
    int n_a = 0, n_b = 0;
    DevBuf<BinChunk> chunks;
    int n_chunks = 0;
    DevBuf<uint16_t> hl, dl;
    DevBuf<int> vb, tb;
    DevBuf<int> tdelta;
    int n_runs = 0, n_tiles = 0;
    bool bin_valid = false;
    int bin_n_int = 0;
    DevBuf<uint32_t> res_pk;
    bool res_valid = false;
    DevBuf<int> su_rng;
    bool su_inline = false;
};

struct Slot {
    int source = 0;
    int source_ext = 0;
    DevBuf<double> p, r;
    DevBuf<double> x, x2;
    DevBuf<uint32_t> act[2];
    size_t act_bytes = 0;
    DevBuf<int> ft[2];
    DevBuf<int> neg;
    DevBuf<int> status;
    DevBuf<int> cnt;
    DevBuf<BigItem> big;
    int *log = nullptr;
    long long iter_seq = 0;
    double sweep_us = 0;
    double atomic_ns = 1.0 / 23.5;
    int iter_hint[2] = {0, 0};
    int iter_hist[2][4] = {{0, 0, 0, 0}, {0, 0, 0, 0}};
    bool start_dense[2] = {false, false};
    int last_F0[2] = {0, 0};
    DevBuf<IterStats> dstats;
    bool converged = false;
    double conv_eps = 0.0;
    double park_eps = 0.0;
    int last_epoch = -2;
    bool seed_lists_valid = false;
    bool phase0_done = false;
    double phase0_eps = 0.0;
    dppr_stats_t st{};
    bool trace = false;
    std::vector<int64_t> trace_off;
    std::vector<int32_t> trace_ids;
};

struct Group {
    int n = 0;
    int spl = 1;
    int gw = OCT;
    int src_ext[GS_MAX] = {0};
    SrcN src{};
    DevBuf<double> p, r, x, x2;
    DevBuf<uint32_t> act[2];
    size_t act_bytes = 0;
    DevBuf<int> cnt;
    DevBuf<int> gq;
    unsigned gq_seq = 0;
    DevBuf<int> mlog;
    DevBuf<IterStats> dstats;
    dppr_stats_t st{};
    int iter_hint[2] = {0, 0};
    int iter_hist[2][4] = {{0, 0, 0, 0}, {0, 0, 0, 0}};
    int dense_hist[2][4] = {{0, 0, 0, 0}, {0, 0, 0, 0}};
    DevBuf<int> plist[2];
    DevBuf<int> ppre;
    DevBuf<GPushCtl> pctl;
    bool converged = false;
    double conv_eps = 0.0;
    double park_eps = 0.0;
    int last_epoch = -2;
};

}

struct dppr_engine : dppr::IdSpace {
    int device = 0;
    int V = 0, W = 0, c = 0, directed = 1, n_epochs = 1;
    int Ed = 0;
    int bits = 1;
    int schedule = DPPR_SCHEDULE_EAGER;
    bool status_dedup = false;
    bool pre_extract = false;
    bool group_at_slide = false;
    int merge_miss_host = 0;
    long long merge_fallbacks = 0;
    bool test_force_merge_miss = false;
    bool launch_called_off = false;
    int raw_backoff = 0;
    bool merge_phases = false;
    int merge_div = 4;
    hipStream_t stream = nullptr;
    hipStream_t bs = nullptr;
    bool build_concurrent = false;
    std::mutex err_mu;
    std::mutex map_mu;
    unsigned map_gen_on_device = 0;
    hipEvent_t ev0 = nullptr, ev1 = nullptr;
    hipEvent_t evpool[2 * 64] = {};
    bool profiling = false;
    int pull_block = 0;
    int chunk_iters = 24;
    bool chunk_explicit = false;
    int persist_mode = 1;
    bool persist_ok = true;
    int persist_retry = 0;
    int persist_cap = 0;
    int res_slots = 1;
    int res_update = 1;
    DevBuf<double> res_arena;
    long long res_arena_stride = 0;
    unsigned long long persist_ticks = 5000000ull;
    int persist_rollcall_extra = 0;
    DevBuf<GridBar> bar;
    DevBuf<int> w1, w2;
    int head = 0;
    bool loaded = false;
    bool broken = false;
    DevBuf<int> outdeg;
    DevBuf<int> hub_slot_of;
    DevBuf<int> hub_hist;
    int hub_min_degree = HUB_MIN_DEGREE_DEFAULT;
    int big_row = BIG_ROW_DEFAULT;
    int pull_min_frontier = 0;
    DevBuf<uint64_t> in_sorted, out_sorted;
    DevBuf<uint64_t> keys_a, keys_b;
    DevBuf<unsigned char> sort_tmp;
    size_t sort_tmp_bytes = 0;
    DevBuf<int> su_grp;
    DevBuf<uint64_t> bk[4];
    DevBuf<uint64_t> bks[4];
    DevBuf<int> delpos;
    struct Pre {
        std::future<bool> task;
        const int32_t *src[4] = {nullptr, nullptr, nullptr, nullptr};
        int n[4] = {0, 0, 0, 0};
        std::vector<int32_t> out[4];
        std::vector<uint32_t> miss[4];
        unsigned long long epoch = 0;
        bool armed = false, ok = false;
    } pre;
    long long pre_hits = 0, pre_misses = 0;
    bool incremental = true;
    bool sweep_bits = false;
    bool hot_blocks = true;
    int gsweep_hot_rows = 24576;
    int gsweep_grid_cap = 0;
    bool group_resident = true;
    int gmulti_cap[2] = {-1, -1};
    bool any_groups = false;
    int ggroups_min = 256;
    bool force_radix_grouping = false;
    bool cost_model = true;
    bool group_full_rows = false;
    bool wide_groups = false;
    bool group_tail_seeding = true;
    int gpush_enter_pairs = -1;
    int gpush_list_cap = 1 << 20;
    long long gpush_max_edges = 0;
    int gpush_auto_factor = 2;
    int bin_mode = 1;
    int bin_ha_tiles = 128, bin_hb_tiles = 60;
    long long bin_target = 0;
    long long bin_target_a = 4ll << 20;
    long long bin_min_ids = 1ll << 19;
    DevBuf<int> bin_vblk_a;
    DevBuf<unsigned long long> bin_scan;
    DevBuf<int> bin_small;
    long long bin_chunk = 32768;
    DevBuf<double> bin_vals;
    DevBuf<uint64_t> bin_wb, bin_wa;
    DevBuf<int> bin_first;
    std::vector<int32_t> bin_cut_a, bin_cut_b;
    int bin_abits = 0, bin_bbits = 0;
    int bin_cut_ids = 0;
    bool bin_words_valid = false;
    int bin_slides_since_cut = 0;
    bool bin_incremental = true;
    int bin_recut_every = 32;
    bool bin_frozen_rebuild = false;
    bool bin_force_full = false;
    int bin_miss_host = 0;
    long long bin_patched = 0, bin_rebuilt = 0;
    DevBuf<unsigned char> bin_tmp;
    size_t bin_tmp_bytes = 0;
    bool bin_ready = false;
    std::vector<int32_t> h_tiles_in;
    DevBuf<uint32_t> su_k[2], su_v[2];
    DevBuf<double> su_term;
    DevBuf<uint8_t> su_ins;
    DevBuf<unsigned char> su_tmp;
    size_t su_tmp_bytes = 0;
    std::vector<int32_t> st_b1, st_b2;
    std::vector<uint8_t> st_ins;
    bool batch_staged = false;
    std::vector<Epoch> epochs;
    int newest = -1;
    std::vector<Slot> slots;
    std::vector<Group> groups;
    PinBuf<int> pinned;
    std::atomic<unsigned long long> heartbeat{0};
    PinBuf<char> dump_pin;
    static constexpr size_t DUMP_PIN_BYTES = sizeof(GridBar) + 4096;
    bool renumber_on = true;
    int renumber_growth_pct = 15;
    int renumber_min_parked = 1024;
    int renumber_next = 0;
    int renumberings = 0;
    std::vector<int32_t> mv_src, mv_dst, mv_zero;
    DevBuf<int> mv_idx;
    DevBuf<double> mv_tmp;
    DevBuf<int> d_ext2int;
    DevBuf<double> d_xfer;
    DevBuf<int> d_int2ext;
    unsigned i2e_gen_on_device = 0;
    DevBuf<unsigned char> tk_ws;
    DevBuf<unsigned long long> tk_out_key;
    DevBuf<int> tk_out_row;
    DevBuf<int> tk_cand;
    DevBuf<unsigned char> tk_res; PinBuf<unsigned char> tk_pin;
    DevBuf<unsigned char> ra_buf;
    std::vector<int32_t> h_tmp1, h_tmp2;
    std::vector<int32_t> h_tiles;
    int max_iters = 1 << 20;
    std::string err;
};

namespace {

inline void set_err(dppr_engine *e, const char *msg) {
    std::lock_guard<std::mutex> lk(e->err_mu);
    e->err = msg;
}

#define HIP_TRY(call)                                                                                   \
    do {                                                                                                \
        const hipError_t _e = static_cast<hipError_t>(call);                                            \
        if (_e != hipSuccess) {                                                                         \
            char _b[512];                                                                               \
            snprintf(_b, sizeof(_b), "%s in %s at line %d", hipGetErrorString(_e), __FILE__, __LINE__); \
            set_err(e, _b);                                                                             \
            return _e == hipErrorOutOfMemory ? DPPR_ERR_NOMEM : DPPR_ERR_HIP;                           \
        }                                                                                               \
    } while (0)

#define HIP_TRY_MSG(prefix, call)                                                 \
    do {                                                                          \
        const hipError_t _e = static_cast<hipError_t>(call);                      \
        if (_e != hipSuccess) {                                                   \
            set_err(e, (std::string(prefix) + hipGetErrorString(_e)).c_str());    \
            return _e == hipErrorOutOfMemory ? DPPR_ERR_NOMEM : DPPR_ERR_HIP;     \
        }                                                                         \
    } while (0)

inline int grid_for(int64_t n, int per_block = BLOCK, int cap = 2048) {
    int64_t g = (n + per_block - 1) / per_block;
    if (g < 1) g = 1;
    if (g > cap) g = cap;
    return (int)g;
}

constexpr long LOOP_SPIN_US = 2000;
inline hipError_t loop_sync(hipStream_t st) {
    static const bool spin = !(getenv("DPPR_SYNC_SPIN") && atoi(getenv("DPPR_SYNC_SPIN")) == 0);
    if (!spin) return hipStreamSynchronize(st);
    timespec t0;
    clock_gettime(CLOCK_MONOTONIC, &t0);
    hipError_t r;
    unsigned polls = 0;
    while ((r = hipStreamQuery(st)) == hipErrorNotReady) {
        if ((++polls & 15u) == 0) {
            timespec now;
            clock_gettime(CLOCK_MONOTONIC, &now);
            if ((now.tv_sec - t0.tv_sec) * 1000000L + (now.tv_nsec - t0.tv_nsec) / 1000L > LOOP_SPIN_US) return hipStreamSynchronize(st);
        }
        __builtin_ia32_pause();
    }
    return r;
}

inline hipError_t loop_wait(dppr_engine *e) {
    e->heartbeat.fetch_add(1, std::memory_order_relaxed);
    return loop_sync(e->stream);
}

int fail(dppr_engine *e, int code, const char *msg) {
    if (e) set_err(e, msg);
    return code;
}

inline void pre_join(dppr_engine *e) {
    if (e->pre.task.valid()) e->pre.ok = e->pre.task.get();
}

inline int to_int(dppr_engine *e, int ext) {
    pre_join(e);
    return e->to_int(ext);
}

int pre_find(dppr_engine *e, const int32_t *src, int n) {
    pre_join(e);
    if (!e->pre.armed || !e->pre.ok || e->pre.epoch != e->renumber_epoch || n <= 0) return -1;
    for (int k = 0; k < 4; ++k)
        if (e->pre.src[k] == src && e->pre.n[k] == n) {
            const std::vector<int32_t> &o = e->pre.out[k];
            const int step = std::max(1, n / 64);
            for (int i = 0; i < n; i = (i + step < n || i == n - 1) ? i + step : n - 1) {
                const int m = o[(size_t)i];
                if (m >= 0 && (m >= (int)e->int2ext.size() || e->int2ext[(size_t)m] != src[i])) {
                    e->pre.armed = false;
                    return -1;
                }
                if (i == n - 1) break;
            }
            return k;
        }
    return -1;
}

bool ids_in_range(dppr_engine *e, const int32_t *src, int n) {
    if (pre_find(e, src, n) >= 0) return true;
    for (int i = 0; i < n; ++i)
        if (src[i] < 0 || src[i] >= e->V) return false;
    return true;
}

bool translate(dppr_engine *e, const int32_t *src, int n, std::vector<int32_t> &dst) {
    const int k = pre_find(e, src, n);
    if (k >= 0) {
        e->pre.src[k] = nullptr;
        dst.swap(e->pre.out[k]);
        e->resolve(src, dst.data(), e->pre.miss[k]);
        e->pre_hits++;
        e->pre_misses += (long long)e->pre.miss[k].size();
        return true;
    }
    if (n > 0) e->pre.armed = false;
    dst.resize((size_t)std::max(n, 1));
    return e->translate(src, (size_t)std::max(n, 0), dst.data());
}

}
```

dynamicppr_amd/csrc/dppr_multi.hpp:

```cpp
#pragma once

#include "dppr_kernels.hpp"

namespace dppr {

constexpr int GS_MAX = 16;
constexpr int OCT = 8;

struct SrcN {
    int s[GS_MAX];
};

__device__ __forceinline__ unsigned oct_mask(uint64_t ballot) {
    return (unsigned)(ballot >> (lane_id() & ~(OCT - 1))) & 0xffu;
}

__host__ __device__ constexpr int row_width(int n_sources) { return n_sources <= 2 ? 2 : (n_sources + 1) / 2 * 2; }
__host__ __device__ constexpr int row_spl(int gw) { return gw > OCT ? 2 : 1; }
#ifndef DPPR_X_COMPACT
#define DPPR_X_COMPACT 0
#endif
__host__ __device__ constexpr int x_stride(int gw) { return DPPR_X_COMPACT ? gw : gw > 8 ? 16 : gw > 4 ? 8 : gw; }
template <int SPL, int GW>
__device__ __forceinline__ bool oct_live(int j) {
    static_assert(GW >= 2 && GW <= OCT * SPL && GW % 2 == 0 && (SPL == 1 || GW > OCT), "row width / lane split");
    if constexpr (GW == OCT * SPL) return true;
    else return j * SPL < GW;
}

__global__ __launch_bounds__(BLOCK) void k_ginit(double *__restrict__ p, double *__restrict__ r, int V, int gw, SrcN src) {
    const int64_t n = (int64_t)V * gw;
    for (int64_t i = (int64_t)blockIdx.x * BLOCK + threadIdx.x; i < n; i += (int64_t)gridDim.x * BLOCK) {
        const int v = (int)(i / gw), s = (int)(i % gw);
        p[i] = 0.0;
        r[i] = (src.s[s] == v) ? 1.0 : 0.0;
    }
}

template <int SPL, int GW>
__global__ __launch_bounds__(BLOCK) void k_gseed_dense(int V, const double *__restrict__ r, double *__restrict__ x,
                                                       double *__restrict__ p, uint32_t *__restrict__ act, int phase,
                                                       double eps, int *__restrict__ cnt_out) {
    __shared__ int s_cnt[GS_MAX];
    if (threadIdx.x < GS_MAX) s_cnt[threadIdx.x] = 0;
    __syncthreads();
    const int j = threadIdx.x & (OCT - 1);
    const bool live = oct_live<SPL, GW>(j);
    int nleg[SPL];
#pragma unroll
    for (int q = 0; q < SPL; ++q) nleg[q] = 0;
    uint8_t *act8 = reinterpret_cast<uint8_t *>(act);
    const int vper = BLOCK / OCT;
    const int Vpad = (V + 7) & ~7;
    for (int vb = blockIdx.x * vper; vb < Vpad; vb += gridDim.x * vper) {
        const int v = vb + (int)threadIdx.x / OCT;
        bool any = false;
        double rv[SPL];
        bool lg[SPL];
#pragma unroll
        for (int q = 0; q < SPL; ++q) {
            rv[q] = v < V && live ? r[(size_t)v * GW + j * SPL + q] : 0.0;
            lg[q] = v < V && live && legal(rv[q], phase, eps);
            any |= lg[q];
            nleg[q] += lg[q] ? 1 : 0;
        }
        const uint64_t bal = __ballot(any);
        const unsigned m = oct_mask(bal);
        if (m && live) {
#pragma unroll
            for (int q = 0; q < SPL; ++q) {
                const size_t i = (size_t)v * GW + j * SPL + q;
                x[(size_t)v * x_stride(GW) + j * SPL + q] = rv[q];
                if (lg[q]) p[i] = p[i] + ALPHA * rv[q];
            }
        }
        if (lane_id() == 0) {
            unsigned byte = 0;
#pragma unroll
            for (int k = 0; k < 8; ++k) byte |= ((bal >> (k * OCT)) & 0xffull) ? (1u << k) : 0u;
            const int v0 = vb + wave_id() * 8;
            if (v0 < Vpad) act8[v0 >> 3] = (uint8_t)byte;
        }
    }
#pragma unroll
    for (int q = 0; q < SPL; ++q)
        if (nleg[q]) atomicAdd(&s_cnt[j * SPL + q], nleg[q]);
    __syncthreads();
    if (threadIdx.x < GW && s_cnt[threadIdx.x]) atomicAdd(&cnt_out[threadIdx.x], s_cnt[threadIdx.x]);
}

template <int SPL, int GW>
__global__ __launch_bounds__(BLOCK) void k_gseed_tails(const uint32_t *__restrict__ skeys, int L, const double *__restrict__ r,
                                                       double *__restrict__ x, double *__restrict__ p,
                                                       uint32_t *__restrict__ act, int phase, double eps,
                                                       int *__restrict__ cnt_out) {
    __shared__ int s_cnt[GS_MAX];
    if (threadIdx.x < GS_MAX) s_cnt[threadIdx.x] = 0;
    __syncthreads();
    const int j = threadIdx.x & (OCT - 1);
    const bool live = oct_live<SPL, GW>(j);
    int nleg[SPL];
#pragma unroll
    for (int q = 0; q < SPL; ++q) nleg[q] = 0;
    const int per = BLOCK / OCT;
    const int Lpad = (L + per - 1) / per * per;
    for (int i0 = blockIdx.x * per; i0 < Lpad; i0 += gridDim.x * per) {
        const int i = i0 + (int)threadIdx.x / OCT;
        int u = -1;
        if (i < L) {
            u = (int)skeys[i];
            if (i > 0 && (int)skeys[i - 1] == u) u = -1;
        }
        bool any = false;
        double rv[SPL];
        bool lg[SPL];
#pragma unroll
        for (int q = 0; q < SPL; ++q) {
            rv[q] = u >= 0 && live ? r[(size_t)u * GW + j * SPL + q] : 0.0;
            lg[q] = u >= 0 && live && legal(rv[q], phase, eps);
            any |= lg[q];
            nleg[q] += lg[q] ? 1 : 0;
        }
        if (oct_mask(__ballot(any))) {
            if (live) {
#pragma unroll
                for (int q = 0; q < SPL; ++q) {
                    const size_t k = (size_t)u * GW + j * SPL + q;
                    x[(size_t)u * x_stride(GW) + j * SPL + q] = rv[q];
                    if (lg[q]) p[k] = p[k] + ALPHA * rv[q];
                }
            }
            if (j == 0) atomicOr(&act[u >> 5], 1u << (u & 31));
        }
    }
#pragma unroll
    for (int q = 0; q < SPL; ++q)
        if (nleg[q]) atomicAdd(&s_cnt[j * SPL + q], nleg[q]);
    __syncthreads();
    if (threadIdx.x < GW && s_cnt[threadIdx.x]) atomicAdd(&cnt_out[threadIdx.x], s_cnt[threadIdx.x]);
}

constexpr int GNT = 1024;
constexpr int GT_HDR = 8;
__host__ __device__ constexpr int GT_STRIDE(int nvx) { return (GT_HDR + nvx + 1 + GNT / OCT + nvx / 2 + 3) / 4 * 4; }

template <int NVX>
__global__ __launch_bounds__(GNT) void k_gtables(int V, const int *__restrict__ grp_tile, int n_groups,
                                                 const int *__restrict__ out_row_ptr, int *__restrict__ tables) {
    constexpr int NW = GNT / WAVE, NOCT = GNT / OCT, EB = 8;
    __shared__ int s_wcnt[NW];
    const int tid = threadIdx.x, lane = lane_id(), w = wave_id();
    for (int g = blockIdx.x; g < n_groups; g += gridDim.x) {
        __syncthreads();
        int *T = tables + (size_t)g * GT_STRIDE(NVX);
        const int t0 = grp_tile[g], t1 = grp_tile[g + 1];
        const int v0 = t0 * WAVE;
        const int nv = min((t1 - t0) * WAVE, V - v0);
        const int E0 = out_row_ptr[v0];
        const int Eg = out_row_ptr[v0 + nv] - E0;
        int rs = 0, d = 0;
        if (tid < nv) {
            rs = out_row_ptr[v0 + tid] - E0;
            d = out_row_ptr[v0 + tid + 1] - E0 - rs;
        }
        const int per = ((Eg + NOCT - 1) / NOCT + EB - 1) / EB * EB;
        const uint64_t ne = __ballot(d > 0);
        if (lane == 0) s_wcnt[w] = __popcll(ne);
        __syncthreads();
        int woff = 0, ncomp = 0;
#pragma unroll
        for (int k = 0; k < NW; ++k) {
            const int c = s_wcnt[k];
            woff += k < w ? c : 0;
            ncomp += c;
        }
        int *cstart = T + GT_HDR, *ostart = T + GT_HDR + NVX + 1;
        unsigned short *cvid = reinterpret_cast<unsigned short *>(T + GT_HDR + NVX + 1 + NOCT);
        if (tid <= NVX && tid >= ncomp) cstart[tid] = Eg;
        if (tid == 0 && NVX >= GNT) cstart[NVX] = Eg;
        if (tid < NOCT) ostart[tid] = 0;
        if (tid < NVX && tid >= ncomp) cvid[tid] = 0;
        if (tid == 0) {
            T[0] = v0; T[1] = nv; T[2] = E0; T[3] = Eg; T[4] = per; T[5] = ncomp; T[6] = 0; T[7] = 0;
        }
        asm volatile("s_waitcnt vmcnt(0)" ::: "memory");
        __syncthreads();
        if (d > 0) {
            const int idx = woff + mbcnt(ne);
            cstart[idx] = rs;
            cvid[idx] = (unsigned short)tid;
            const int o_first = (rs + per - 1) / per, o_last = min((rs + d + per - 1) / per - 1, NOCT - 1);
            for (int o = o_first; o <= o_last; ++o) ostart[o] = idx;
        }
    }
}

template <bool COH>
__device__ __forceinline__ double gs_ld(const double *p) {
    if constexpr (COH)
        return __longlong_as_double((long long)__hip_atomic_load(reinterpret_cast<const unsigned long long *>(p),
                                                                 __ATOMIC_RELAXED, __HIP_MEMORY_SCOPE_AGENT));
    else
        return *p;
}
template <bool COH>
__device__ __forceinline__ uint32_t gs_ldu(const uint32_t *p) {
    if constexpr (COH) return __hip_atomic_load(p, __ATOMIC_RELAXED, __HIP_MEMORY_SCOPE_AGENT);
    else return *p;
}
template <bool COH>
__device__ __forceinline__ void gs_st(double *p, double v) {
    if constexpr (COH)
        __hip_atomic_store(reinterpret_cast<unsigned long long *>(p), (unsigned long long)__double_as_longlong(v),
                           __ATOMIC_RELAXED, __HIP_MEMORY_SCOPE_AGENT);
    else
        *p = v;
}
template <bool COH>
__device__ __forceinline__ void gs_stu(uint32_t *p, uint32_t v) {
    if constexpr (COH) __hip_atomic_store(p, v, __ATOMIC_RELAXED, __HIP_MEMORY_SCOPE_AGENT);
    else *p = v;
}

#ifndef DPPR_GS_NT
#define DPPR_GS_NT 0
#endif
#ifndef DPPR_WHATIF
#define DPPR_WHATIF 0
#endif
template <bool COH, int BIT>
__device__ __forceinline__ double gs_ld_once(const double *p) {
    if constexpr (!COH && (DPPR_GS_NT & BIT)) return __builtin_nontemporal_load(p);
    else return gs_ld<COH>(p);
}
template <bool COH, int BIT>
__device__ __forceinline__ void gs_st_once(double *p, double v) {
    if constexpr (!COH && (DPPR_GS_NT & BIT)) __builtin_nontemporal_store(v, p);
    else gs_st<COH>(p, v);
}

constexpr int GSM_ABORTED = 1 << 30;
constexpr int GSM_FAULT = 1 << 29;
constexpr int GSM_CONVERGED = 1 << 28;
constexpr int GSM_SWEEPS = (1 << 16) - 1;

template <int SPL, int GW, int NVX, bool MULTI, int CM>
__global__ __launch_bounds__(GNT, MULTI ? 4 : 8) void k_gsweep(int V, const int *__restrict__ gtab, int n_groups,
                                                   const int *cnt_in, int hot_rows,
                                                   const int *__restrict__ out_col, double *x_a, double *x_b,
                                                   uint32_t *act_a, uint32_t *act_b, double *r, double *p, int *cnt_out,
                                                   int *cnt_zero, int phase, double eps, IterStats *__restrict__ stats,
                                                   int *log_slot, int n_iter, GridBar *bar, int *status,
                                                   unsigned long long limit_ticks, int rollcall_extra, int credit0,
                                                   int *q_take, int *q_zero) {
    constexpr int NOCT = GNT / OCT, WORDS = NVX / 32, XS = x_stride(GW);
    static_assert(sizeof(double) * NVX * GW <= 64 * 1024, "two workgroups per CU");
    constexpr int EB = 8;
    constexpr int GB = EB / SPL;
#ifndef DPPR_GS_FU
#define DPPR_GS_FU (4 / SPL)
#endif
    constexpr int FU_WANT = CM == 0 && SPL == 2 ? 2 * (DPPR_GS_FU) : (DPPR_GS_FU);
    constexpr int FU = MULTI ? NVX / NOCT : FU_WANT <= NVX / NOCT ? FU_WANT : NVX / NOCT;
    static_assert(MULTI == (CM == 2), "the multi-sweep form decides per sweep, a one-sweep launch is compiled for its mode");
    static_assert(NVX % NOCT == 0 && (NVX / NOCT) % FU == 0, "vertex phase covers the group in whole steps");
    __shared__ double s_acc[NVX * GW];
    __shared__ int s_cstart[NVX + 1];
    __shared__ unsigned short s_cvid[NVX];
    __shared__ int s_ostart[NOCT];
    __shared__ uint32_t s_actin[WORDS], s_actout[WORDS], s_touched[WORDS];
    __shared__ int s_cnt[GS_MAX];
    __shared__ unsigned long long s_edges;
    __shared__ int s_flag[2];
    __shared__ int s_ticket;
    const int tid0 = threadIdx.x, lane = lane_id(), w = wave_id();
    const int j = tid0 & (OCT - 1);
    auto opaque = [](int v) {
#ifndef DPPR_NO_OPAQUE
        asm volatile("" : "+v"(v));
#endif
        return v;
    };

    bool stamp_dense = false;
    if constexpr (!MULTI) {
        const int my_cnt = lane < GW ? cnt_in[lane] : 0;
        if (blockIdx.x == 0 && tid0 < GW) {
            cnt_zero[tid0] = 0;
            log_slot[tid0] = my_cnt;
        }
        if (blockIdx.x == 0 && tid0 == 0) *q_zero = 0;
        if (__ballot(my_cnt != 0) == 0) return;
#ifdef DPPR_STAMPS
#if defined(DPPR_STAMP_MID)
        {
            const long long tot = __builtin_amdgcn_readlane(wave_inclusive_scan(my_cnt), WAVE - 1);
            stamp_dense = tot * 16 > (long long)V && tot * 2 < (long long)V;
        }
#elif defined(DPPR_STAMP_SPARSE)
        stamp_dense = (long long)__builtin_amdgcn_readlane(wave_inclusive_scan(my_cnt), WAVE - 1) * 64 < (long long)V;
#else
        stamp_dense = (long long)__builtin_amdgcn_readlane(wave_inclusive_scan(my_cnt), WAVE - 1) > 4ll * V;
#endif
#endif
    }
    (void)stamp_dense;
#ifdef DPPR_STAMPS
    if (stamp_dense) STAMP(7);
    if (!MULTI && stamp_dense && tid0 == 0 && blockIdx.x < 4096) g_stamps[blockIdx.x * 8 + 5] = wall_clock64();
#endif
    for (int k = tid0; k < NVX * GW; k += GNT) s_acc[k] = 0.0;
    if (tid0 < WORDS) {
        s_actout[tid0] = 0u;
        s_touched[tid0] = 0u;
    }
    if (tid0 < GS_MAX) s_cnt[tid0] = 0;
    if (tid0 == 0) {
        s_edges = 0ull;
        s_flag[0] = 1;
        s_flag[1] = 0;
    }
    int nleg[SPL];
#pragma unroll
    for (int q = 0; q < SPL; ++q) nleg[q] = 0;
    unsigned ecount = 0;

    const unsigned G = gridDim.x;
    const unsigned subs_used = G < (unsigned)BAR_SUBS ? G : (unsigned)BAR_SUBS;
    const unsigned long long n_sub = lane < (int)subs_used ? (G - lane + BAR_SUBS - 1) / BAR_SUBS : 0;
    const int my_rep = (blockIdx.x / BAR_SUBS) % BAR_REPS;
    if constexpr (MULTI) {
        const unsigned long long t_entry = wall_clock64();
        __syncthreads();
        if (tid0 == 0)
            __hip_atomic_fetch_add(&bar->roll[blockIdx.x % BAR_SUBS].w, 1ull << 32, __ATOMIC_RELAXED, __HIP_MEMORY_SCOPE_AGENT);
        if (w == 0) {
            if (blockIdx.x == 0) {
                unsigned polls = 0;
                bool all_here = false;
                for (;;) {
                    const unsigned long long word = lane < (int)subs_used ? bar_load(&bar->roll[lane].w) : 0;
                    if (__ballot((word >> 32) >= n_sub + (lane == 0 ? (unsigned long long)rollcall_extra : 0ull)) == ~0ull) {
                        all_here = true;
                        break;
                    }
                    if ((polls++ & 31u) == 0 && (bar_load(&bar->gen.w) != 0 || wall_clock64() - t_entry > limit_ticks)) break;
                    __builtin_amdgcn_s_sleep(1);
                }
                if (lane == 0) (void)bar_cas(&bar->gen.w, 0ull, all_here ? BAR_READY : BAR_ABORT);
            }
            if (lane == 0) {
                unsigned long long word;
                unsigned polls = 0;
                while ((word = bar_load(&bar->gen.w)) == 0) {
                    if ((polls++ & 31u) == 0 && wall_clock64() - t_entry > limit_ticks) (void)bar_cas(&bar->gen.w, 0ull, BAR_ABORT);
                    __builtin_amdgcn_s_sleep(1);
                }
                s_flag[0] = word != BAR_ABORT;
            }
        }
        __syncthreads();
        if (!s_flag[0]) {
            if (blockIdx.x == 0 && tid0 == 0) *status = GSM_ABORTED;
            return;
        }
    }

    constexpr int STRIDE = GT_STRIDE(NVX);
    int hv0 = 0, hnv = 0, hE0 = 0, hEg = 0, hper = 0;
    if ((int)blockIdx.x < n_groups) {
        const int *H = gtab + (size_t)blockIdx.x * STRIDE;
        hv0 = H[0]; hnv = H[1]; hE0 = H[2]; hEg = H[3]; hper = H[4];
    }
    int sweeps_done = 0;
    bool converged = false, fault = false;
    for (int g = blockIdx.x; g < n_groups;) {
        __syncthreads();
        int ticket = 0, g_next = n_groups;
        if (!MULTI && tid0 == 0) ticket = (int)gridDim.x + atomicAdd(q_take, 1);
        const int *T = gtab + (size_t)g * STRIDE;
        const int tid = opaque(tid0);
        const int j = tid & (OCT - 1), oid = tid / OCT;
        const bool live = oct_live<SPL, GW>(j);
        const int v0 = hv0, nv = hnv, E0 = hE0, Eg = hEg, per = hper;
        const int e_begin = oid * per, e_end = min(Eg, e_begin + per);
        const int *cols = out_col + E0;
        {
            const int c0 = tid < NVX ? T[GT_HDR + tid] : 0;
            const int os = tid < NOCT ? T[GT_HDR + NVX + 1 + tid] : 0;
            const unsigned short cv = tid < NVX ? reinterpret_cast<const unsigned short *>(T + GT_HDR + NVX + 1 + NOCT)[tid] : 0;
            if (tid < WORDS) s_actin[tid] = tid * 32 < nv ? gs_ldu<MULTI>(act_a + (v0 >> 5) + tid) : 0u;
            if (tid < NVX) {
                s_cstart[tid] = c0;
                s_cvid[tid] = cv;
            }
            if (tid < NOCT) s_ostart[tid] = os;
            if (tid == 0) s_cstart[NVX] = Eg;
        }
        int mycol = e_begin + j < e_end ? ld_stream(&cols[e_begin + j]) : -1;
        int ncol = e_begin + EB + j < e_end ? ld_stream(&cols[e_begin + EB + j]) : -1;

        for (int it = 0; it < (MULTI ? n_iter : 1); ++it) {
            const double *x = (it & 1) ? x_b : x_a;
            double *x_new = (it & 1) ? x_a : x_b;
            const uint32_t *act_in = (it & 1) ? act_b : act_a;
            uint32_t *act_out = (it & 1) ? act_a : act_b;
            const bool credit = CM == 2 ? ((credit0 ^ it) & 1) != 0 : CM == 1;
            if constexpr (MULTI) {
                const int *row = it == 0 ? cnt_in : log_slot + (size_t)it * GS_MAX;
                const int f = lane < GW ? (int)gs_ldu<true>(reinterpret_cast<const uint32_t *>(row + lane)) : 0;
                if (it == 0 && blockIdx.x == 0 && tid < GW) log_slot[tid] = f;
                if (__ballot(f != 0) == 0) {
                    converged = true;
                    break;
                }
            }
#define GSTAMP(i) do { if (MULTI ? it == 12 : stamp_dense) STAMP(i); } while (0)
            GSTAMP(0);
            if (it > 0) {
                if (tid < WORDS) s_actin[tid] = tid * 32 < nv ? gs_ldu<MULTI>(act_in + (v0 >> 5) + tid) : 0u;
                mycol = e_begin + j < e_end ? ld_stream(&cols[e_begin + j]) : -1;
                ncol = e_begin + EB + j < e_end ? ld_stream(&cols[e_begin + EB + j]) : -1;
            }
            __syncthreads();

            if (e_begin < e_end) {
                int crow = s_ostart[oid];
                int row_beg = s_cstart[crow], row_end = s_cstart[crow + 1];
                double den = (double)(row_end - row_beg + 1);
                double rcp = 1.0 / den;
                double acc[SPL];
#pragma unroll
                for (int q = 0; q < SPL; ++q) acc[q] = 0.0;
                auto flush = [&]() {
                    const int vl = s_cvid[crow];
                    bool nz = false;
#pragma unroll
                    for (int q = 0; q < SPL; ++q) {
                        if (acc[q] != 0.0) lds_add(&s_acc[vl * GW + j * SPL + q], acc[q]);
                        nz |= acc[q] != 0.0;
                        acc[q] = 0.0;
                    }
                    if (nz) atomicOr(&s_touched[vl >> 5], 1u << (vl & 31));
                };
                uint32_t aw = mycol >= 0 ? gs_ldu<MULTI>(act_in + (mycol >> 5)) : 0u;
                for (int e = e_begin; e < e_end; e += EB) {
                    const bool a = mycol >= 0 && ((aw >> (mycol & 31)) & 1u);
                    const uint32_t naw = ncol >= 0 ? gs_ldu<MULTI>(act_in + (ncol >> 5)) : 0u;
                    const int nncol = e + 2 * EB + j < e_end ? ld_stream(&cols[e + 2 * EB + j]) : -1;
                    const unsigned m = oct_mask(__ballot(a));
#pragma unroll
                    for (int h = 0; h < EB; h += GB) {
                        const unsigned mh = (m >> h) & ((1u << GB) - 1u);
                        if (mh) {
                            double xv[GB][SPL];
#pragma unroll
                            for (int k = 0; k < GB; ++k) {
                                const int ck = __shfl(mycol, (lane & ~(OCT - 1)) + h + k, WAVE);
#pragma unroll
                                for (int q = 0; q < SPL; ++q) xv[k][q] = 0.0;
#if DPPR_WHATIF & 4
                                if (((mh >> k) & 1u) && live) { xv[k][0] = 1e-7 * (ck & 7); }
                                else
#endif
#if DPPR_WHATIF & 16
                                if (((mh >> k) & 1u) && live) {
#pragma unroll
                                    for (int q = 0; q < SPL; ++q) xv[k][q] = gs_ld<MULTI>(x + (size_t)(ck & 4095) * XS + j * SPL + q);
                                } else
#endif
                                if (((mh >> k) & 1u) && live) {
                                    if (MULTI || !(DPPR_GS_NT & 1) || ck < hot_rows) {
#pragma unroll
                                        for (int q = 0; q < SPL; ++q) xv[k][q] = gs_ld<MULTI>(x + (size_t)ck * XS + j * SPL + q);
                                    } else {
#pragma unroll
                                        for (int q = 0; q < SPL; ++q) xv[k][q] = gs_ld_once<MULTI, 1>(x + (size_t)ck * XS + j * SPL + q);
                                    }
                                }
                            }
#pragma unroll
                            for (int k = 0; k < GB; ++k) {
                                if ((mh >> k) & 1u) {
                                    const int ek = e + h + k;
                                    if (ek >= row_end) {
                                        flush();
                                        do {
                                            ++crow;
                                            row_beg = row_end;
                                            row_end = s_cstart[crow + 1];
                                        } while (ek >= row_end);
                                        den = (double)(row_end - row_beg + 1);
                                        rcp = 1.0 / den;
                                    }
#pragma unroll
                                    for (int q = 0; q < SPL; ++q) {
                                        if (legal(xv[k][q], phase, eps)) {
                                            acc[q] += push_term(xv[k][q], den, rcp);
                                            ++ecount;
                                        }
                                    }
                                }
                            }
                        }
                    }
                    mycol = ncol;
                    aw = naw;
                    ncol = nncol;
                }
                flush();
            }
            if (!MULTI && tid0 == 0) s_ticket = ticket;
            GSTAMP(1);
            __syncthreads();
            GSTAMP(2);
            if constexpr (!MULTI) {
                g_next = __builtin_amdgcn_readfirstlane(s_ticket);
                if (g_next < n_groups) {
                    const int *H = gtab + (size_t)g_next * STRIDE;
                    hv0 = H[0]; hnv = H[1]; hE0 = H[2]; hEg = H[3]; hper = H[4];
                }
            }

            for (int i0 = 0; i0 < NVX / NOCT; i0 += FU) {
                const int tid_v = opaque(tid0);
                const int j = tid_v & (OCT - 1), oid = tid_v / OCT;
                const bool live = oct_live<SPL, GW>(j);
                int vl[FU];
                bool tch[FU], wasact[FU];
                double cur[FU][SPL], pv[FU][SPL];
#pragma unroll
                for (int i = 0; i < FU; ++i) {
                    vl[i] = oid + (i0 + i) * NOCT;
                    const unsigned bit = 1u << (vl[i] & 31);
                    wasact[i] = (s_actin[vl[i] >> 5] & bit) != 0;
                    tch[i] = vl[i] < nv && (wasact[i] || (s_touched[vl[i] >> 5] & bit) != 0);
#pragma unroll
                    for (int q = 0; q < SPL; ++q) {
                        cur[i][q] = 0.0;
                        pv[i][q] = 0.0;
                    }
                    if (tch[i] && live) {
                        const size_t base = (size_t)(v0 + vl[i]) * GW + j * SPL;
                        const double *row = wasact[i] ? x + (size_t)(v0 + vl[i]) * XS + j * SPL : r + base;
#pragma unroll
                        for (int q = 0; q < SPL; ++q) {
#if DPPR_WHATIF & 2
                            if (!wasact[i])
#endif
                            cur[i][q] = gs_ld_once<MULTI, 2>(row + q);
#if DPPR_WHATIF & 2
                            else cur[i][q] = 1.0;
#endif
#if !(DPPR_WHATIF & 1)
                            if (credit) pv[i][q] = gs_ld_once<MULTI, 2>(p + base + q);
#endif
                        }
                    }
                }
#pragma unroll
                for (int i = 0; i < FU; ++i) {
                    if (tch[i]) {
                        const size_t base = (size_t)(v0 + vl[i]) * GW + j * SPL;
                        double rn[SPL];
                        bool lg[SPL], pushed[SPL], any = false, changed = false;
#pragma unroll
                        for (int q = 0; q < SPL; ++q) {
                            double a = 0.0;
                            if (live) {
                                double *ap = &s_acc[vl[i] * GW + j * SPL + q];
                                a = *ap;
                                *ap = 0.0;
                            }
                            pushed[q] = wasact[i] && legal(cur[i][q], phase, eps);
                            rn[q] = pushed[q] ? a : cur[i][q] + a;
                            lg[q] = legal(rn[q], phase, eps);
                            any |= lg[q];
                            changed |= rn[q] != cur[i][q];
                            nleg[q] += lg[q] ? 1 : 0;
                        }
#if !(DPPR_WHATIF & 1)
                        if (credit && live) {
#pragma unroll
                            for (int q = 0; q < SPL; ++q) {
                                if (pushed[q] || lg[q]) {
                                    double pn = pv[i][q];
                                    if (pushed[q]) pn = pn + ALPHA * cur[i][q];
                                    if (lg[q]) pn = pn + ALPHA * rn[q];
                                    gs_st_once<false, 4>(p + base + q, pn);
                                }
                            }
                        }
#endif
                        if (oct_mask(__ballot(any))) {
                            if (live && !(DPPR_WHATIF & 8)) {
#pragma unroll
                                for (int q = 0; q < SPL; ++q) gs_st_once<MULTI, 4>(x_new + (size_t)(v0 + vl[i]) * XS + j * SPL + q, rn[q]);
                            }
                            if (j == 0) atomicOr(&s_actout[vl[i] >> 5], 1u << (vl[i] & 31));
                        } else if ((wasact[i] || changed) && live) {
#pragma unroll
                            for (int q = 0; q < SPL; ++q) gs_st_once<false, 4>(r + base + q, rn[q]);
                        }
                    }
                }
            }
            GSTAMP(3);
            __syncthreads();
            GSTAMP(4);
            if (tid < WORDS) {
                if (tid * 32 < nv) gs_stu<MULTI>(act_out + (v0 >> 5) + tid, s_actout[tid]);
                s_actout[tid] = 0u;
                s_touched[tid] = 0u;
            }
            if constexpr (MULTI) {
#pragma unroll
                for (int q = 0; q < SPL; ++q) {
                    if (nleg[q]) atomicAdd(&s_cnt[j * SPL + q], nleg[q]);
                    nleg[q] = 0;
                }
                asm volatile("s_waitcnt vmcnt(0)" ::: "memory");
                __syncthreads();
                GSTAMP(5);
                if (tid < GW) {
                    if (s_cnt[tid])
                        __hip_atomic_fetch_add(log_slot + (size_t)(it + 1) * GS_MAX + tid, s_cnt[tid], __ATOMIC_RELAXED,
                                               __HIP_MEMORY_SCOPE_AGENT);
                    s_cnt[tid] = 0;
                }
                if (w == 0) {
                    asm volatile("s_waitcnt vmcnt(0)" ::: "memory");
                    if (lane < BAR_REPS)
                        __hip_atomic_fetch_add(&bar->sub[it & 1][lane][blockIdx.x % BAR_SUBS].w, 1ull << 32, __ATOMIC_RELAXED,
                                               __HIP_MEMORY_SCOPE_AGENT);
                    const unsigned long long rounds = (unsigned long long)((it >> 1) + 1);
                    unsigned polls = 0;
                    const unsigned long long t_start = wall_clock64();
                    bool ok = true;
                    for (;;) {
                        const unsigned long long word = lane < (int)subs_used ? bar_load(&bar->sub[it & 1][my_rep][lane].w) : 0;
                        if (__ballot((word >> 32) >= n_sub * rounds) == ~0ull) break;
                        if ((polls++ & 63u) == 63u && wall_clock64() - t_start > limit_ticks + 100000000ull) {
                            ok = false;
                            break;
                        }
                        __builtin_amdgcn_s_sleep(BAR_POLL_SLEEP);
                    }
                    if (lane == 0 && !ok) s_flag[1] = 1;
                }
                __syncthreads();
                GSTAMP(6);
                sweeps_done = it + 1;
                if (s_flag[1]) {
                    fault = true;
                    break;
                }
            }
        }
        if constexpr (MULTI) break;
        g = g_next;
    }
    const int tid = tid0;
    if constexpr (MULTI) {
        if (blockIdx.x == 0 && tid < GS_MAX) {
            const int f = (tid < GW && !converged && !fault)
                              ? (int)gs_ldu<true>(reinterpret_cast<const uint32_t *>(log_slot + (size_t)sweeps_done * GS_MAX + tid)) : 0;
            cnt_out[tid] = f;
            cnt_zero[tid] = 0;
        }
        if (blockIdx.x == 0 && tid == 0)
            *status = sweeps_done | (fault ? GSM_FAULT : 0) | (converged ? GSM_CONVERGED : 0);
        if (ecount) atomicAdd(&s_edges, (unsigned long long)ecount);
        __syncthreads();
        if (tid == 0 && s_edges) stats->blk_E[blockIdx.x] += s_edges;
        return;
    }
#ifdef DPPR_STAMPS
    if (!MULTI && stamp_dense && tid == 0 && blockIdx.x < 4096) g_stamps[blockIdx.x * 8 + 6] = wall_clock64();
#endif
#pragma unroll
    for (int q = 0; q < SPL; ++q)
        if (nleg[q]) atomicAdd(&s_cnt[j * SPL + q], nleg[q]);
    if (ecount) atomicAdd(&s_edges, (unsigned long long)ecount);
    __syncthreads();
    if (tid < GW && s_cnt[tid]) atomicAdd(&cnt_out[tid], s_cnt[tid]);
    if (tid == 0 && s_edges) stats->blk_E[blockIdx.x] += s_edges;
}

__global__ __launch_bounds__(BLOCK) void k_gint_to_ext(const double *__restrict__ a_int, int gw, int lane_s,
                                                       const int *__restrict__ ext2int, int V,
                                                       double *__restrict__ a_ext) {
    for (int v = blockIdx.x * BLOCK + threadIdx.x; v < V; v += gridDim.x * BLOCK) {
        const int m = ext2int[v];
        a_ext[v] = m >= 0 ? a_int[(size_t)m * gw + lane_s] : 0.0;
    }
}

}
```

dynamicppr_amd/engine.py:

```python
from __future__ import annotations

import ctypes as C
import os
import subprocess

import numpy as np

_HERE = os.path.dirname(os.path.abspath(__file__))
LIB_PATH = os.environ.get("DPPR_LIB") or os.path.join(_HERE, "libdppr_hip.so")

SCHEDULE_EAGER = 0
SCHEDULE_SYNC = 1


class DpprError(RuntimeError):
    pass


class Stats(C.Structure):
    _fields_ = [("iterations", C.c_int64), ("sum_F", C.c_int64), ("sum_E", C.c_int64), ("sum_N", C.c_int64),
                ("records", C.c_int64), ("inspected", C.c_int64), ("batches", C.c_int64),
                ("pull_iterations", C.c_int64),
                ("algorithmic_bytes", C.c_int64), ("gpu_ms", C.c_double), ("push_ms", C.c_double),
                ("push_launches", C.c_int64), ("persist_launches", C.c_int64), ("persist_aborts", C.c_int64),
                ("binned_sweeps", C.c_int64), ("sweep_F", C.c_int64), ("sweep_E", C.c_int64), ("sweep_ms", C.c_double),
                ("sweep_launches", C.c_int64)]

    def as_dict(self):
        return {k: getattr(self, k) for k, _ in self._fields_}


def build(force: bool = False) -> str:
    csrc = os.path.join(_HERE, "csrc")
    srcs = [os.path.join(csrc, f) for f in os.listdir(csrc) if f.endswith((".hip", ".hpp"))]
    srcs.append(os.path.join(os.path.dirname(_HERE), "include", "dppr.h"))
    stale = (not os.path.exists(LIB_PATH)) or any(os.path.getmtime(s) > os.path.getmtime(LIB_PATH) for s in srcs)
    if force or stale:
        subprocess.check_call(["make", "-C", csrc, "-s", "all"])
    return LIB_PATH


_lib = None
EXPORTS = [
    "dppr_abi_version", "dppr_strerror", "dppr_last_error", "dppr_create", "dppr_destroy", "dppr_set_schedule", "dppr_set_profiling", "dppr_set_tuning", "dppr_set_persistent", "dppr_set_incremental_graph",
    "dppr_load_window", "dppr_set_batch", "dppr_slide", "dppr_add_source", "dppr_init_solve", "dppr_update",
    "dppr_incremental_batch_update", "dppr_execute_main_loop", "dppr_read", "dppr_write", "dppr_stats",
    "dppr_reset_stats", "dppr_inspect", "dppr_read_graph", "dppr_graph_edges", "dppr_read_out_graph", "dppr_trace_enable",
    "dppr_trace_get", "dppr_synchronize", "dppr_bench_atomics",
    "dppr_add_source_group", "dppr_group_init_solve", "dppr_group_update", "dppr_group_read", "dppr_group_stats",
    "dppr_group_reset_stats", "dppr_set_group_seeding", "dppr_seed_lists", "dppr_set_sweep_bitmap", "dppr_set_group_resident", "dppr_set_resident_slots", "dppr_set_resident_update",
    "dppr_set_renumbering", "dppr_id_space", "dppr_set_group_push", "dppr_set_binned_sweep", "dppr_device_count", "dppr_set_phase_merge", "dppr_init_solve_at", "dppr_group_init_solve_at", "dppr_set_variant", "dppr_set_batch_grouping",
    "dppr_time_batch_grouping", "dppr_debug_dump", "dppr_hint_next_batch",
    "dppr_bench_line_fills", "dppr_bench_stream_copy", "dppr_build_id", "dppr_heartbeat", "dppr_slide_concurrent", "dppr_renumbering_due", "dppr_debug_bin_tables",
    "dppr_debug_grouping", "dppr_topk", "dppr_group_topk", "dppr_read_at", "dppr_group_read_at", "dppr_debug_live_bytes",
    "dppr_group_sources", "dppr_group_replace_source", "dppr_group_add_source", "dppr_group_remove_source",
]


def lib():
    global _lib
    if _lib is not None:
        return _lib
    if not os.path.exists(LIB_PATH):
        raise DpprError(f"{LIB_PATH} is missing: run `python -c 'import __graft_entry__ as g; g.build()'` "
                        "(the HIP extension is mandatory, there is no CPU fallback)")
    L = C.CDLL(LIB_PATH)
    vp, ip, dp, u8p = C.c_void_p, C.POINTER(C.c_int32), C.POINTER(C.c_double), C.POINTER(C.c_uint8)
    i64p, fp = C.POINTER(C.c_int64), C.POINTER(C.c_float)
    L.dppr_abi_version.restype = C.c_int
    L.dppr_strerror.argtypes = [C.c_int]
    L.dppr_strerror.restype = C.c_char_p
    L.dppr_last_error.argtypes = [vp]
    L.dppr_last_error.restype = C.c_char_p
    L.dppr_create.argtypes = [C.POINTER(vp), C.c_int, C.c_int32, C.c_int32, C.c_int, C.c_int32, C.c_int32]
    L.dppr_destroy.argtypes = [vp]
    L.dppr_destroy.restype = None
    L.dppr_set_schedule.argtypes = [vp, C.c_int]
    L.dppr_set_profiling.argtypes = [vp, C.c_int]
    L.dppr_set_incremental_graph.argtypes = [vp, C.c_int]
    L.dppr_set_renumbering.argtypes = [vp, C.c_int, C.c_int, C.c_int]
    L.dppr_set_group_push.argtypes = [vp, C.c_int, C.c_int, C.c_int64]
    L.dppr_id_space.argtypes = [vp, C.POINTER(C.c_int32), C.POINTER(C.c_int32), C.POINTER(C.c_int32), C.POINTER(C.c_int64)]
    L.dppr_set_tuning.argtypes = [vp, C.c_int, C.c_int, C.c_int, C.c_int, C.c_int]
    L.dppr_set_persistent.argtypes = [vp, C.c_int, C.c_int64]
    L.dppr_load_window.argtypes = [vp, ip, ip, C.c_int32]
    L.dppr_set_batch.argtypes = [vp, ip, ip, u8p, C.c_int32]
    L.dppr_slide.argtypes = [vp, ip, ip, C.c_int32, ip]
    L.dppr_add_source.argtypes = [vp, C.c_int32, ip]
    L.dppr_init_solve.argtypes = [vp, C.c_int32, C.c_double, fp]
    L.dppr_init_solve_at.argtypes = [vp, C.c_int32, C.c_int32, C.c_double, fp]
    L.dppr_group_init_solve_at.argtypes = [vp, C.c_int32, C.c_int32, C.c_double, fp]
    L.dppr_update.argtypes = [vp, C.c_int32, C.c_int32, C.c_double, fp]
    L.dppr_incremental_batch_update.argtypes = [vp, C.c_int32, C.c_int32]
    L.dppr_execute_main_loop.argtypes = [vp, C.c_int32, C.c_int32, C.c_int, C.c_double]
    L.dppr_read.argtypes = [vp, C.c_int32, dp, dp]
    L.dppr_write.argtypes = [vp, C.c_int32, dp, dp]
    L.dppr_stats.argtypes = [vp, C.c_int32, C.POINTER(Stats)]
    L.dppr_reset_stats.argtypes = [vp, C.c_int32]
    L.dppr_inspect.argtypes = [vp, C.c_int32, C.c_int, C.c_double, ip, ip]
    L.dppr_read_graph.argtypes = [vp, C.c_int32, ip, ip, ip]
    L.dppr_graph_edges.argtypes = [vp, C.c_int32, ip]
    L.dppr_read_out_graph.argtypes = [vp, C.c_int32, ip, ip]
    L.dppr_trace_enable.argtypes = [vp, C.c_int32, C.c_int]
    L.dppr_trace_get.argtypes = [vp, C.c_int32, i64p, i64p, i64p, ip]
    L.dppr_synchronize.argtypes = [vp]
    L.dppr_add_source_group.argtypes = [vp, ip, C.c_int32, ip]
    L.dppr_group_init_solve.argtypes = [vp, C.c_int32, C.c_double, fp]
    L.dppr_group_update.argtypes = [vp, C.c_int32, C.c_int32, C.c_double, fp]
    L.dppr_group_read.argtypes = [vp, C.c_int32, C.c_int32, dp, dp]
    L.dppr_group_stats.argtypes = [vp, C.c_int32, C.POINTER(Stats)]
    L.dppr_set_sweep_bitmap.argtypes = [vp, C.c_int]
    L.dppr_set_phase_merge.argtypes = [vp, C.c_int, C.c_int]
    L.dppr_set_variant.argtypes = [vp, C.c_int]
    L.dppr_set_batch_grouping.argtypes = [vp, C.c_int]
    L.dppr_set_binned_sweep.argtypes = [vp, C.c_int, C.c_int, C.c_int, C.c_int64, C.c_int64, C.c_int64, C.c_int64]
    L.dppr_set_group_resident.argtypes = [vp, C.c_int]
    L.dppr_set_resident_slots.argtypes = [vp, C.c_int]
    L.dppr_set_resident_update.argtypes = [vp, C.c_int]
    L.dppr_seed_lists.argtypes = [vp, C.c_int32, C.c_int, ip, ip]
    L.dppr_group_reset_stats.argtypes = [vp, C.c_int32]
    L.dppr_set_group_seeding.argtypes = [vp, C.c_int]
    L.dppr_bench_atomics.argtypes = [C.c_int, C.c_int64, C.c_int64, C.c_int, C.c_int, fp]
    L.dppr_time_batch_grouping.argtypes = [vp, C.c_int32, C.c_int32, fp]
    L.dppr_debug_dump.argtypes = [vp, C.c_char_p, C.c_int32]
    L.dppr_hint_next_batch.argtypes = [vp, ip, ip, C.c_int32, ip, ip, C.c_int32]
    L.dppr_bench_line_fills.argtypes = [C.c_int, C.c_int64, C.c_int64, C.c_int, fp]
    L.dppr_bench_stream_copy.argtypes = [C.c_int, C.c_int64, C.c_int, fp]
    L.dppr_build_id.restype = C.c_char_p
    L.dppr_heartbeat.argtypes = [vp]
    L.dppr_slide_concurrent.argtypes = [vp, ip, ip, C.c_int32, ip]
    L.dppr_renumbering_due.argtypes = [vp]
    u16p = C.POINTER(C.c_uint16)
    L.dppr_debug_bin_tables.argtypes = [vp, C.c_int32, ip, ip, ip, ip, ip, ip, ip, u16p, ip, ip, u16p, ip, i64p, i64p]
    u32p = C.POINTER(C.c_uint32)
    L.dppr_debug_grouping.argtypes = [vp, C.c_int32, C.c_int32, u32p, u32p, ip, ip, ip]
    L.dppr_heartbeat.restype = C.c_ulonglong
    L.dppr_topk.argtypes = [vp, C.c_int32, C.c_int32, C.c_double, ip, dp, dp, ip]
    L.dppr_group_topk.argtypes = [vp, C.c_int32, C.c_int32, C.c_double, ip, dp, dp, ip]
    L.dppr_read_at.argtypes = [vp, C.c_int32, ip, C.c_int32, dp, dp]
    L.dppr_group_read_at.argtypes = [vp, C.c_int32, ip, C.c_int32, dp, dp]
    L.dppr_debug_live_bytes.argtypes = [i64p, i64p]
    L.dppr_group_sources.argtypes = [vp, C.c_int32, ip, ip]
    L.dppr_group_replace_source.argtypes = [vp, C.c_int32, C.c_int32, C.c_int32, fp]
    L.dppr_group_add_source.argtypes = [vp, C.c_int32, C.c_int32, ip, fp]
    L.dppr_group_remove_source.argtypes = [vp, C.c_int32, C.c_int32]
    for name in EXPORTS:
        if name not in ("dppr_strerror", "dppr_last_error", "dppr_destroy", "dppr_build_id", "dppr_heartbeat"):
            getattr(L, name).restype = C.c_int
    _lib = L
    return L


def _i32(a):
    a = np.ascontiguousarray(a, dtype=np.int32)
    return a, a.ctypes.data_as(C.POINTER(C.c_int32))


class Engine:

    def __init__(self, V, W, directed, max_batch, n_epochs=1, device=0, schedule=SCHEDULE_EAGER,
                 hub_min_degree=None, big_row_edges=None, pull_min_frontier=None, chunk_iters=None, pull_block=None,
                 persistent=None, persist_timeout_us=None, sweep_bitmap=None, binned=None, merge_phases=None, variant=None, group_at_slide=None, resident_slots=None, resident_update=None):
        self._L = lib()
        self._h = C.c_void_p()
        self._batch_len, self._staged_len = {0: 0}, 0
        self._group_n = {}
        self.V, self.W, self.directed, self.c = int(V), int(W), int(directed), int(max_batch)
        rc = self._L.dppr_create(C.byref(self._h), int(device), self.V, self.W, self.directed, self.c, int(n_epochs))
        if rc:
            self._h = C.c_void_p()
            raise DpprError(f"dppr_create: {self._L.dppr_strerror(rc).decode()}")
        self.set_schedule(schedule)
        if variant is not None:
            self._ck(self._L.dppr_set_variant(self._h, int(variant)), "set_variant")
        if any(v is not None for v in (hub_min_degree, big_row_edges, pull_min_frontier, chunk_iters, pull_block)):
            self._ck(self._L.dppr_set_tuning(self._h, int(hub_min_degree or 256), int(big_row_edges or 512),
                                             int(pull_min_frontier or 0), int(chunk_iters or 0),
                                             int(pull_block or 0)), "set_tuning")
        if sweep_bitmap is not None:
            self._ck(self._L.dppr_set_sweep_bitmap(self._h, int(sweep_bitmap)), "set_sweep_bitmap")
        if group_at_slide is not None:
            self._ck(self._L.dppr_set_batch_grouping(self._h, int(group_at_slide)), "set_batch_grouping")
        if resident_slots is not None:
            self.set_resident_slots(resident_slots)
        if resident_update is not None:
            self._ck(self._L.dppr_set_resident_update(self._h, int(resident_update)), "set_resident_update")
        if merge_phases is not None:
            self.set_phase_merge(bool(merge_phases), 0 if merge_phases is True or not merge_phases else int(merge_phases))
        if binned is not None:
            args = (binned,) if isinstance(binned, int) else tuple(binned)
            args = tuple(int(a) for a in args) + (0,) * (7 - len(args))
            self._ck(self._L.dppr_set_binned_sweep(self._h, *args), "set_binned_sweep")
        if persistent is not None or persist_timeout_us is not None:
            self._ck(self._L.dppr_set_persistent(self._h, 1 if persistent is None else int(persistent),
                                                 int(persist_timeout_us or 0)), "set_persistent")

    def _ck(self, rc, what):
        if rc:
            raise DpprError(f"{what}: {self._L.dppr_strerror(rc).decode()} ({self._L.dppr_last_error(self._h).decode()})")

    def close(self):
        if getattr(self, "_h", None) and self._h.value:
            self._L.dppr_destroy(self._h)
            self._h = C.c_void_p()

    def __del__(self):
        try:
            self.close()
        except Exception:
            pass

    def set_schedule(self, schedule):
        self._ck(self._L.dppr_set_schedule(self._h, int(schedule)), "set_schedule")

    def set_phase_merge(self, on, eps_divisor=0):
        self._ck(self._L.dppr_set_phase_merge(self._h, int(on), int(eps_divisor)), "set_phase_merge")

    def bin_tables(self, epoch=-1, arrays=True):
        na, nb, ne, nr, nt, pa, rb = C.c_int32(), C.c_int32(), C.c_int32(), C.c_int32(), C.c_int32(), C.c_int64(), C.c_int64()
        rc = self._L.dppr_debug_bin_tables(self._h, int(epoch), C.byref(na), C.byref(nb), C.byref(ne), C.byref(nr), C.byref(nt),
                                           None, None, None, None, None, None, None, C.byref(pa), C.byref(rb))
        out = {"patched": pa.value, "rebuilt": rb.value}
        if rc:
            return None if not arrays else dict(out, valid=False)
        out.update(valid=True, n_a=na.value, n_b=nb.value, n_edges=ne.value, n_runs=nr.value, n_tiles=nt.value)
        if arrays:
            n_blk, n_rb = (ne.value + 63) // 64, (nr.value + 63) // 64
            acut, bcut = np.empty(na.value + 1, np.int32), np.empty(nb.value + 1, np.int32)
            hl, dl = np.empty(max(nr.value, 1), np.uint16), np.empty(max(ne.value, 1), np.uint16)
            tdelta, tb, vb = np.empty(max(nt.value, 1), np.int32), np.empty(n_rb + 1, np.int32), np.empty(n_blk + 1, np.int32)
            i32, u16 = C.POINTER(C.c_int32), C.POINTER(C.c_uint16)
            self._ck(self._L.dppr_debug_bin_tables(self._h, int(epoch), None, None, None, None, None, acut.ctypes.data_as(i32), bcut.ctypes.data_as(i32),
                                                   hl.ctypes.data_as(u16), tdelta.ctypes.data_as(i32), tb.ctypes.data_as(i32), dl.ctypes.data_as(u16),
                                                   vb.ctypes.data_as(i32), None, None), "debug_bin_tables")
            out.update(acut=acut, bcut=bcut, hl=hl[:nr.value], tdelta=tdelta[:nt.value], tb=tb, dl=dl[:ne.value], vb=vb)
        return out

    def renumbering_due(self):
        return bool(self._L.dppr_renumbering_due(self._h))

    def set_batch_grouping(self, at_slide):
        self._ck(self._L.dppr_set_batch_grouping(self._h, int(at_slide)), "set_batch_grouping")

    def set_incremental_graph(self, on):
        self._ck(self._L.dppr_set_incremental_graph(self._h, int(on)), "set_incremental_graph")

    def set_group_push(self, enter_pairs=-1, list_cap=0, max_edges=0):
        self._ck(self._L.dppr_set_group_push(self._h, int(enter_pairs), int(list_cap), int(max_edges)), "set_group_push")

    def set_renumbering(self, on, growth_pct=0, min_parked=0):
        self._ck(self._L.dppr_set_renumbering(self._h, int(on), int(growth_pct), int(min_parked)), "set_renumbering")

    def id_space(self):
        a, b, c, d = C.c_int32(), C.c_int32(), C.c_int32(), C.c_int64()
        self._ck(self._L.dppr_id_space(self._h, C.byref(a), C.byref(b), C.byref(c), C.byref(d)), "id_space")
        return {"ids": a.value, "parked": b.value, "renumberings": c.value, "revivals": d.value}

    def set_profiling(self, on):
        self._ck(self._L.dppr_set_profiling(self._h, int(on)), "set_profiling")

    def load_window(self, e1, e2):
        a, pa = _i32(e1)
        b, pb = _i32(e2)
        self._ck(self._L.dppr_load_window(self._h, pa, pb, len(a)), "load_window")
        self._batch_len = {0: 0}
        self._staged_len = 0

    def set_batch(self, b1, b2, ins):
        a, pa = _i32(b1)
        b, pb = _i32(b2)
        i = np.ascontiguousarray(ins, dtype=np.uint8)
        self._ck(self._L.dppr_set_batch(self._h, pa, pb, i.ctypes.data_as(C.POINTER(C.c_uint8)), len(a)), "set_batch")
        self._staged_len = len(a)

    def hint_next_batch(self, b1, b2, n1, n2):
        arrs = [_i32(x) for x in (b1, b2, n1, n2)]
        if len(arrs[0][0]) != len(arrs[1][0]) or len(arrs[2][0]) != len(arrs[3][0]):
            raise DpprError("hint_next_batch: b1 / b2 and n1 / n2 must have equal lengths")
        self._hint_keep = [a for a, _ in arrs]
        self._ck(self._L.dppr_hint_next_batch(self._h, arrs[0][1], arrs[1][1], len(arrs[0][0]), arrs[2][1], arrs[3][1], len(arrs[2][0])),
                 "hint_next_batch")
        return tuple(self._hint_keep)

    def slide(self, n1, n2, concurrent=False):
        a, pa = _i32(n1)
        b, pb = _i32(n2)
        ep = C.c_int32(-1)
        fn = self._L.dppr_slide_concurrent if concurrent else self._L.dppr_slide
        self._ck(fn(self._h, pa, pb, len(a), C.byref(ep)), "slide")
        self._batch_len[ep.value] = self._staged_len
        self._staged_len = 0
        return ep.value

    def add_source(self, s):
        slot = C.c_int32(-1)
        self._ck(self._L.dppr_add_source(self._h, int(s), C.byref(slot)), "add_source")
        return slot.value

    def init_solve(self, slot, eps, epoch=-1):
        ms = C.c_float(0)
        self._ck(self._L.dppr_init_solve_at(self._h, slot, int(epoch), float(eps), C.byref(ms)), "init_solve")
        return ms.value

    def update(self, slot, eps, epoch=-1):
        ms = C.c_float(0)
        self._ck(self._L.dppr_update(self._h, slot, int(epoch), float(eps), C.byref(ms)), "update")
        return ms.value

    def incremental_batch_update(self, slot, epoch=-1):
        self._ck(self._L.dppr_incremental_batch_update(self._h, slot, int(epoch)), "incremental_batch_update")

    def execute_main_loop(self, slot, phase, eps, epoch=-1):
        self._ck(self._L.dppr_execute_main_loop(self._h, slot, int(epoch), int(phase), float(eps)), "execute_main_loop")

    def read(self, slot):
        p = np.empty(self.V, dtype=np.float64)
        r = np.empty(self.V, dtype=np.float64)
        dp = C.POINTER(C.c_double)
        self._ck(self._L.dppr_read(self._h, slot, p.ctypes.data_as(dp), r.ctypes.data_as(dp)), "read")
        return p, r

    def write(self, slot, p, r):
        p = np.ascontiguousarray(p, dtype=np.float64)
        r = np.ascontiguousarray(r, dtype=np.float64)
        dp = C.POINTER(C.c_double)
        self._ck(self._L.dppr_write(self._h, slot, p.ctypes.data_as(dp), r.ctypes.data_as(dp)), "write")

    def stats(self, slot):
        st = Stats()
        self._ck(self._L.dppr_stats(self._h, slot, C.byref(st)), "stats")
        return st.as_dict()

    def reset_stats(self, slot):
        self._ck(self._L.dppr_reset_stats(self._h, slot), "reset_stats")

    def inspect(self, slot, phase, eps):
        out = np.empty(self.V, dtype=np.int32)
        n = C.c_int32(0)
        self._ck(self._L.dppr_inspect(self._h, slot, int(phase), float(eps),
                                      out.ctypes.data_as(C.POINTER(C.c_int32)), C.byref(n)), "inspect")
        return out[:n.value].copy()

    def seed_lists(self, slot, phase):
        out = np.empty(max(4 * self.c, 1), dtype=np.int32)
        n = C.c_int32(0)
        self._ck(self._L.dppr_seed_lists(self._h, slot, int(phase), out.ctypes.data_as(C.POINTER(C.c_int32)),
                                         C.byref(n)), "seed_lists")
        return out[:n.value].copy()

    def read_graph(self, epoch=-1):
        ne = C.c_int32(0)
        self._ck(self._L.dppr_graph_edges(self._h, int(epoch), C.byref(ne)), "graph_edges")
        row = np.empty(self.V + 1, dtype=np.int32)
        col = np.empty(max(ne.value, 1), dtype=np.int32)
        deg = np.empty(self.V, dtype=np.int32)
        ip = C.POINTER(C.c_int32)
        self._ck(self._L.dppr_read_graph(self._h, int(epoch), row.ctypes.data_as(ip), col.ctypes.data_as(ip),
                                         deg.ctypes.data_as(ip)), "read_graph")
        return row, col[:ne.value], deg

    def read_out_graph(self, epoch=-1):
        ne = C.c_int32(0)
        self._ck(self._L.dppr_graph_edges(self._h, int(epoch), C.byref(ne)), "graph_edges")
        row = np.empty(self.V + 1, dtype=np.int32)
        col = np.empty(max(ne.value, 1), dtype=np.int32)
        ip = C.POINTER(C.c_int32)
        self._ck(self._L.dppr_read_out_graph(self._h, int(epoch), row.ctypes.data_as(ip), col.ctypes.data_as(ip)),
                 "read_out_graph")
        return row, col[:ne.value]

    def trace_enable(self, slot, on=True):
        self._ck(self._L.dppr_trace_enable(self._h, slot, int(on)), "trace_enable")

    def trace_get(self, slot):
        ni, nd = C.c_int64(0), C.c_int64(0)
        self._ck(self._L.dppr_trace_get(self._h, slot, C.byref(ni), C.byref(nd), None, None), "trace_get")
        off = np.zeros(ni.value + 1, dtype=np.int64)
        ids = np.zeros(max(nd.value, 1), dtype=np.int32)
        self._ck(self._L.dppr_trace_get(self._h, slot, None, None, off.ctypes.data_as(C.POINTER(C.c_int64)),
                                        ids.ctypes.data_as(C.POINTER(C.c_int32))), "trace_get")
        return [ids[off[i]:off[i + 1]].copy() for i in range(ni.value)]

    def add_source_group(self, sources):
        a, pa = _i32(sources)
        gid = C.c_int32(-1)
        self._ck(self._L.dppr_add_source_group(self._h, pa, len(a), C.byref(gid)), "add_source_group")
        self._group_n[gid.value] = len(a)
        return gid.value

    def group_init_solve(self, group, eps, epoch=-1):
        ms = C.c_float(0)
        self._ck(self._L.dppr_group_init_solve_at(self._h, group, int(epoch), float(eps), C.byref(ms)), "group_init_solve")
        return ms.value

    def group_update(self, group, eps, epoch=-1):
        ms = C.c_float(0)
        self._ck(self._L.dppr_group_update(self._h, group, int(epoch), float(eps), C.byref(ms)), "group_update")
        return ms.value

    def group_read(self, group, index):
        p = np.empty(self.V, dtype=np.float64)
        r = np.empty(self.V, dtype=np.float64)
        dp = C.POINTER(C.c_double)
        self._ck(self._L.dppr_group_read(self._h, group, int(index), p.ctypes.data_as(dp), r.ctypes.data_as(dp)),
                 "group_read")
        return p, r

    def group_sources(self, group):
        out = np.empty(16, dtype=np.int32)
        n = C.c_int32(0)
        self._ck(self._L.dppr_group_sources(self._h, int(group), out.ctypes.data_as(C.POINTER(C.c_int32)), C.byref(n)), "group_sources")
        self._group_n[group] = n.value
        return [int(v) for v in out[:n.value]]

    def group_replace_source(self, group, index, source):
        ms = C.c_float(0)
        self._ck(self._L.dppr_group_replace_source(self._h, int(group), int(index), int(source), C.byref(ms)), "group_replace_source")
        return ms.value

    def group_add_source(self, group, source):
        idx, ms = C.c_int32(-1), C.c_float(0)
        self._ck(self._L.dppr_group_add_source(self._h, int(group), int(source), C.byref(idx), C.byref(ms)), "group_add_source")
        self._group_n[group] = idx.value + 1
        return idx.value, ms.value

    def group_remove_source(self, group, index):
        self._ck(self._L.dppr_group_remove_source(self._h, int(group), int(index)), "group_remove_source")
        self.group_sources(group)

    def topk(self, slot, k, min_p=0.0):
        ids, p, r, cnt = self._topk(self._L.dppr_topk, slot, 1, k, min_p, "topk")
        return ids[0, :cnt[0]].copy(), p[0, :cnt[0]].copy(), r[0, :cnt[0]].copy()

    def group_topk(self, group, k, min_p=0.0):
        ids, p, r, cnt = self._topk(self._L.dppr_group_topk, group, self._group_n.get(group, 1), k, min_p, "group_topk")
        return [(ids[i, :c].copy(), p[i, :c].copy(), r[i, :c].copy()) for i, c in enumerate(cnt)]

    def _topk(self, fn, which, n, k, min_p, what):
        kk = max(int(k), 1)
        ids = np.empty((n, kk), dtype=np.int32)
        p = np.empty((n, kk), dtype=np.float64)
        r = np.empty((n, kk), dtype=np.float64)
        cnt = np.empty(n, dtype=np.int32)
        ip, dp = C.POINTER(C.c_int32), C.POINTER(C.c_double)
        self._ck(fn(self._h, int(which), int(k), float(min_p), ids.ctypes.data_as(ip), p.ctypes.data_as(dp),
                    r.ctypes.data_as(dp), cnt.ctypes.data_as(ip)), what)
        return ids, p, r, cnt

    def read_at(self, slot, ids):
        a, pa = _i32(ids)
        p = np.empty(len(a), dtype=np.float64)
        r = np.empty(len(a), dtype=np.float64)
        dp = C.POINTER(C.c_double)
        self._ck(self._L.dppr_read_at(self._h, int(slot), pa, len(a), p.ctypes.data_as(dp), r.ctypes.data_as(dp)), "read_at")
        return p, r

    def group_read_at(self, group, ids):
        a, pa = _i32(ids)
        n = self._group_n.get(group, 1)
        p = np.empty((len(a), n), dtype=np.float64)
        r = np.empty((len(a), n), dtype=np.float64)
        dp = C.POINTER(C.c_double)
        self._ck(self._L.dppr_group_read_at(self._h, int(group), pa, len(a), p.ctypes.data_as(dp), r.ctypes.data_as(dp)),
                 "group_read_at")
        return p, r

    def group_stats(self, group):
        st = Stats()
        self._ck(self._L.dppr_group_stats(self._h, group, C.byref(st)), "group_stats")
        return st.as_dict()

    def group_reset_stats(self, group):
        self._ck(self._L.dppr_group_reset_stats(self._h, group), "group_reset_stats")

    def set_resident_slots(self, sorted_slots):
        self._ck(self._L.dppr_set_resident_slots(self._h, int(sorted_slots)), "set_resident_slots")

    def set_group_resident(self, on):
        self._ck(self._L.dppr_set_group_resident(self._h, int(on)), "set_group_resident")

    def set_group_seeding(self, from_tails):
        self._ck(self._L.dppr_set_group_seeding(self._h, int(from_tails)), "set_group_seeding")

    def synchronize(self):
        self._ck(self._L.dppr_synchronize(self._h), "synchronize")

    def time_batch_grouping(self, epoch=-1, reps=5):
        ms = C.c_float(0)
        self._ck(self._L.dppr_time_batch_grouping(self._h, int(epoch), int(reps), C.byref(ms)), "time_batch_grouping")
        return ms.value

    def debug_grouping(self, epoch=-1, path=0):
        L = self._batch_len.get(max(self._batch_len) if epoch < 0 else int(epoch), 0)
        cap = max(4 * self.c, 1)
        tails, index = np.zeros(cap, np.uint32), np.zeros(cap, np.uint32)
        raw = np.zeros(cap, np.int32)
        taken, nb = C.c_int32(0), C.c_int32(0)
        u32p = C.POINTER(C.c_uint32)
        self._ck(self._L.dppr_debug_grouping(self._h, int(epoch), int(path), tails.ctypes.data_as(u32p), index.ctypes.data_as(u32p),
                                             raw.ctypes.data_as(C.POINTER(C.c_int32)), C.byref(taken), C.byref(nb)), "debug_grouping")
        return tails[:L].copy(), index[:L].copy(), raw[:L].copy(), taken.value, nb.value

    def debug_dump(self):
        buf = C.create_string_buffer(1 << 16)
        n = self._L.dppr_debug_dump(self._h, buf, len(buf))
        return buf.raw[:max(n, 0)].decode(errors="replace")


def bench_atomics(table_elems, n, scope=0, reps=5, device=0):
    ms = C.c_float(0)
    rc = lib().dppr_bench_atomics(int(device), int(table_elems), int(n), int(scope), int(reps), C.byref(ms))
    if rc:
        raise DpprError(f"bench_atomics: {lib().dppr_strerror(rc).decode()}")
    return ms.value


def bench_line_fills(table_bytes=1 << 30, lines=1 << 26, reps=3, device=0):
    ms = C.c_float(0)
    rc = lib().dppr_bench_line_fills(int(device), int(table_bytes), int(lines), int(reps), C.byref(ms))
    if rc:
        raise DpprError(f"bench_line_fills: {lib().dppr_strerror(rc).decode()}")
    return ms.value


def bench_stream_copy(nbytes=1 << 30, reps=5, device=0):
    ms = C.c_float(0)
    rc = lib().dppr_bench_stream_copy(int(device), int(nbytes), int(reps), C.byref(ms))
    if rc:
        raise DpprError(f"bench_stream_copy: {lib().dppr_strerror(rc).decode()}")
    return ms.value


def live_bytes():
    dev, pin = C.c_int64(0), C.c_int64(0)
    rc = lib().dppr_debug_live_bytes(C.byref(dev), C.byref(pin))
    if rc:
        raise DpprError(f"debug_live_bytes: {lib().dppr_strerror(rc).decode()}")
    return dev.value, pin.value


def build_id():
    return lib().dppr_build_id().decode()
```

include/dppr.h:

```cpp
#ifndef DPPR_H
#define DPPR_H

#include <stdint.h>

#ifdef __cplusplus
extern "C" {
#endif

#define DPPR_ABI_VERSION 6

typedef struct dppr_engine dppr_engine;

typedef enum dppr_status {
    DPPR_OK = 0,
    DPPR_ERR_INVALID = -1,
    DPPR_ERR_HIP = -2,
    DPPR_ERR_NOMEM = -3,
    DPPR_ERR_NO_DEVICE = -4,
    DPPR_ERR_NOT_CONVERGED = -5
} dppr_status;

#define DPPR_SCHEDULE_EAGER 0
#define DPPR_SCHEDULE_SYNC 1

typedef struct dppr_stats_t {
    int64_t iterations;
    int64_t sum_F;
    int64_t sum_E;
    int64_t sum_N;
    int64_t records;
    int64_t inspected;
    int64_t batches;
    int64_t pull_iterations;
    int64_t algorithmic_bytes;
    double gpu_ms;
    double push_ms;
    int64_t push_launches;
    int64_t persist_launches;
    int64_t persist_aborts;
    int64_t binned_sweeps;
    int64_t sweep_F;
    int64_t sweep_E;
    double sweep_ms;
    int64_t sweep_launches;
} dppr_stats_t;


int dppr_device_count(void);

int dppr_set_batch_grouping(dppr_engine *e, int at_slide);

int dppr_set_variant(dppr_engine *e, int variant);

int dppr_set_phase_merge(dppr_engine *e, int on, int eps_divisor);

int dppr_create(dppr_engine **out, int device, int32_t vertex_count, int32_t window_edges,
                int directed, int32_t max_batch, int32_t n_epochs);
void dppr_destroy(dppr_engine *e);
const char *dppr_strerror(int status);
const char *dppr_last_error(const dppr_engine *e);
int dppr_abi_version(void);
int dppr_set_schedule(dppr_engine *e, int schedule);
int dppr_set_profiling(dppr_engine *e, int on);
int dppr_set_tuning(dppr_engine *e, int hub_min_degree, int big_row_edges, int pull_min_frontier,
                    int chunk_iters, int pull_block);
int dppr_set_persistent(dppr_engine *e, int mode, int64_t timeout_us);

int dppr_set_sweep_bitmap(dppr_engine *e, int on);

int dppr_set_binned_sweep(dppr_engine *e, int mode, int ha_tiles, int hb_tiles, int64_t target_edges, int64_t min_ids,
                          int64_t chunk_edges, int64_t target_a_edges);


int dppr_load_window(dppr_engine *e, const int32_t *e1, const int32_t *e2, int32_t n);

int dppr_set_batch(dppr_engine *e, const int32_t *edge1, const int32_t *edge2,
                   const uint8_t *is_insert, int32_t length);

int dppr_slide(dppr_engine *e, const int32_t *new_e1, const int32_t *new_e2, int32_t c,
               int32_t *out_epoch);

int dppr_slide_concurrent(dppr_engine *e, const int32_t *new_e1, const int32_t *new_e2, int32_t c, int32_t *out_epoch);
int dppr_renumbering_due(const dppr_engine *e);

int dppr_set_incremental_graph(dppr_engine *e, int on);

int dppr_set_renumbering(dppr_engine *e, int on, int growth_pct, int min_parked);
int dppr_id_space(dppr_engine *e, int32_t *n_ids, int32_t *n_parked, int32_t *renumberings, int64_t *revivals);


int dppr_add_source(dppr_engine *e, int32_t source_vertex, int32_t *out_slot);

int dppr_init_solve(dppr_engine *e, int32_t slot, double eps, float *out_ms);
int dppr_init_solve_at(dppr_engine *e, int32_t slot, int32_t epoch, double eps, float *out_ms);

int dppr_update(dppr_engine *e, int32_t slot, int32_t epoch, double eps, float *out_ms);

int dppr_incremental_batch_update(dppr_engine *e, int32_t slot, int32_t epoch);
int dppr_seed_lists(dppr_engine *e, int32_t slot, int phase, int32_t *out_ids, int32_t *out_count);
int dppr_execute_main_loop(dppr_engine *e, int32_t slot, int32_t epoch, int phase, double eps);

int dppr_read(dppr_engine *e, int32_t slot, double *p, double *r);
int dppr_write(dppr_engine *e, int32_t slot, const double *p, const double *r);

int dppr_stats(dppr_engine *e, int32_t slot, dppr_stats_t *out);
int dppr_reset_stats(dppr_engine *e, int32_t slot);

int dppr_add_source_group(dppr_engine *e, const int32_t *sources, int32_t n , int32_t *out_group);
int dppr_group_init_solve(dppr_engine *e, int32_t group, double eps, float *out_ms);
int dppr_group_init_solve_at(dppr_engine *e, int32_t group, int32_t epoch, double eps, float *out_ms);
int dppr_group_update(dppr_engine *e, int32_t group, int32_t epoch, double eps, float *out_ms);
int dppr_group_read(dppr_engine *e, int32_t group, int32_t index, double *p, double *r);
int dppr_group_stats(dppr_engine *e, int32_t group, dppr_stats_t *out);
int dppr_group_reset_stats(dppr_engine *e, int32_t group);

int dppr_group_sources(dppr_engine *e, int32_t group, int32_t *out_sources , int32_t *out_n);
int dppr_group_replace_source(dppr_engine *e, int32_t group, int32_t index, int32_t new_source, float *out_ms);
int dppr_group_add_source(dppr_engine *e, int32_t group, int32_t new_source, int32_t *out_index, float *out_ms);
int dppr_group_remove_source(dppr_engine *e, int32_t group, int32_t index);

#define DPPR_TOPK_MAX 8192
int dppr_topk(dppr_engine *e, int32_t slot, int32_t k, double min_p,
              int32_t *out_ids, double *out_p, double *out_r , int32_t *out_count);
int dppr_group_topk(dppr_engine *e, int32_t group, int32_t k, double min_p,
                    int32_t *out_ids , double *out_p , double *out_r ,
                    int32_t *out_counts );
int dppr_read_at(dppr_engine *e, int32_t slot, const int32_t *ids, int32_t m, double *out_p, double *out_r);
int dppr_group_read_at(dppr_engine *e, int32_t group, const int32_t *ids, int32_t m,
                       double *out_p , double *out_r );

int dppr_set_group_resident(dppr_engine *e, int on);
int dppr_set_resident_slots(dppr_engine *e, int sorted);
int dppr_set_resident_update(dppr_engine *e, int on);
int dppr_set_group_push(dppr_engine *e, int enter_pairs, int list_cap, int64_t max_edges);

int dppr_set_group_seeding(dppr_engine *e, int from_tails);


int dppr_inspect(dppr_engine *e, int32_t slot, int phase, double eps, int32_t *out_ids, int32_t *out_count);

int dppr_read_graph(dppr_engine *e, int32_t epoch, int32_t *row_ptr, int32_t *col, int32_t *out_degree);
int dppr_graph_edges(dppr_engine *e, int32_t epoch, int32_t *out_directed_edges);
int dppr_read_out_graph(dppr_engine *e, int32_t epoch, int32_t *row_ptr, int32_t *col);

int dppr_trace_enable(dppr_engine *e, int32_t slot, int on);
int dppr_trace_get(dppr_engine *e, int32_t slot, int64_t *n_iters, int64_t *n_ids,
                   int64_t *offsets, int32_t *ids);

int dppr_synchronize(dppr_engine *e);

int dppr_hint_next_batch(dppr_engine *e, const int32_t *b1, const int32_t *b2, int32_t L, const int32_t *n1, const int32_t *n2, int32_t c);

int dppr_time_batch_grouping(dppr_engine *e, int32_t epoch, int32_t reps, float *out_ms);
int dppr_debug_grouping(dppr_engine *e, int32_t epoch, int32_t path, uint32_t *tails_out, uint32_t *index_out, int32_t *raw_tails_out,
                        int32_t *path_taken, int32_t *nb_out);

int dppr_debug_dump(dppr_engine *e, char *buf, int32_t cap);
int dppr_debug_bin_tables(dppr_engine *e, int32_t epoch, int32_t *n_a, int32_t *n_b, int32_t *n_edges, int32_t *n_runs, int32_t *n_tiles,
                          int32_t *acut, int32_t *bcut, uint16_t *hl, int32_t *tdelta, int32_t *tb, uint16_t *dl, int32_t *vb,
                          int64_t *patched, int64_t *rebuilt);
int dppr_debug_live_bytes(int64_t *device_bytes, int64_t *pinned_bytes);

unsigned long long dppr_heartbeat(const dppr_engine *e);

int dppr_bench_atomics(int device, int64_t table_elems, int64_t n, int scope, int reps, float *out_ms);
int dppr_bench_line_fills(int device, int64_t table_bytes, int64_t lines, int reps, float *out_ms);
int dppr_bench_stream_copy(int device, int64_t bytes, int reps, float *out_ms);

const char *dppr_build_id(void);

#ifdef __cplusplus
}
#endif
#endif
```

Baseline: 55.26 million.

## Switch group sweeps to a persistent capped-grid tail kernel once frontier shrinks

```diff
diff --git a/dynamicppr_amd/csrc/dppr_engine.hip b/dynamicppr_amd/csrc/dppr_engine.hip
--- a/dynamicppr_amd/csrc/dppr_engine.hip
+++ b/dynamicppr_amd/csrc/dppr_engine.hip
@@ -305,6 +305,13 @@
     e->gpush_enter_pairs = enter_pairs;
     if (list_cap > 0) e->gpush_list_cap = list_cap;
     e->gpush_max_edges = max_edges;
+    return DPPR_OK;
+}
+
+int dppr_set_group_tail(dppr_engine *e, int64_t enter_pairs, int grid_cap) {
+    if (!e || enter_pairs < -1 || enter_pairs > INT32_MAX || grid_cap < 0) return fail(e, DPPR_ERR_INVALID, "set_group_tail: bad argument");
+    e->gtail_enter_pairs = (int)enter_pairs;
+    e->gtail_grid_cap = std::min(grid_cap, STAT_SLOTS);
     return DPPR_OK;
 }
 
@@ -1427,8 +1434,18 @@
     GET_GROUP(e, group);
     HIP_TRY(hipSetDevice(e->device));
     g.st = dppr_stats_t{};
+    g.tail_launches = g.tail_sweeps = 0;
+    g.tail_ms = 0;
     HIP_TRY(hipMemsetAsync(g.dstats, 0, 2 * sizeof(IterStats), e->stream));
     HIP_TRY(hipStreamSynchronize(e->stream));
+    return DPPR_OK;
+}
+
+int dppr_group_tail_stats(dppr_engine *e, int32_t group, int64_t *launches, int64_t *sweeps, double *ms) {
+    GET_GROUP(e, group);
+    if (launches) *launches = g.tail_launches;
+    if (sweeps) *sweeps = g.tail_sweeps;
+    if (ms) *ms = g.tail_ms;
     return DPPR_OK;
 }
 
diff --git a/dynamicppr_amd/csrc/dppr_host_group.hpp b/dynamicppr_amd/csrc/dppr_host_group.hpp
--- a/dynamicppr_amd/csrc/dppr_host_group.hpp
+++ b/dynamicppr_amd/csrc/dppr_host_group.hpp
@@ -23,6 +23,19 @@
         int per_cu = 0, cus = 0;
         hipError_t rc = spl == 1 ? hipOccupancyMaxActiveBlocksPerMultiprocessor(&per_cu, k_gsweep<1, 8, 1024, true, 2>, GNT, 0)
                                  : hipOccupancyMaxActiveBlocksPerMultiprocessor(&per_cu, k_gsweep<2, 16, 512, true, 2>, GNT, 0);
+        if (rc != hipSuccess || hipDeviceGetAttribute(&cus, hipDeviceAttributeMultiprocessorCount, e->device) != hipSuccess)
+            per_cu = 0;
+        cap = std::min(per_cu * cus, STAT_SLOTS);
+    }
+    return cap;
+}
+
+int group_tail_capacity(dppr_engine *e, int spl) {
+    int &cap = e->gtail_cap[spl - 1];
+    if (cap < 0) {
+        int per_cu = 0, cus = 0;
+        hipError_t rc = spl == 1 ? hipOccupancyMaxActiveBlocksPerMultiprocessor(&per_cu, k_gsweep<1, 8, 1024, true, 3>, GNT, 0)
+                                 : hipOccupancyMaxActiveBlocksPerMultiprocessor(&per_cu, k_gsweep<2, 16, 512, true, 3>, GNT, 0);
         if (rc != hipSuccess || hipDeviceGetAttribute(&cus, hipDeviceAttributeMultiprocessorCount, e->device) != hipSuccess)
             per_cu = 0;
         cap = std::min(per_cu * cus, STAT_SLOTS);
@@ -168,10 +181,33 @@
     bool push_gave_up = false;
     int dense_len = -1;
     const int nvx = ep.ggrp_max_tiles * WAVE;
+    const long long tail_thr = e->gtail_enter_pairs == 0 ? 0 : e->gtail_enter_pairs > 0 ? (long long)e->gtail_enter_pairs
+                                                          : std::max<long long>(1, (long long)ep.grp_n_int * g.n / std::max(1, e->gtail_auto_div));
+    auto pairs_of = [&](const int *c) {
+        long long F = 0;
+        for (int s = 0; s < GWM; ++s) F += c[s];
+        return F;
+    };
+    long long F_now = pairs_of(e->pinned);
+    int rb_next = 0;
+    bool first_chunk = true;
+    bool seen_dense = false;
+    int tail_start = -1;
+    auto note_frontier = [&](int sweep, long long F) {
+        if (push_thr > 0 && dense_len < 0 && F <= push_thr) dense_len = sweep;
+        if (tail_thr > 0 && F > tail_thr) seen_dense = true;
+        else if (tail_thr > 0 && seen_dense && tail_start < 0) tail_start = sweep;
+    };
+    static const bool trace = getenv("DPPR_GROUP_TRACE") != nullptr;
     for (int it = 0; more;) {
         if (it >= e->max_iters) return fail(e, DPPR_ERR_NOT_CONVERGED, "iteration cap hit");
         const int mcap = e->group_resident && e->persist_mode && e->persist_ok && e->chunk_iters > 1 ? group_multi_capacity(e, g.spl) : 0;
-        if (mcap > 0 && ep.n_ggroups > 0 && ep.n_ggroups <= mcap) {
+        int tail_grid = 0;
+        if (mcap > 0 && tail_thr > 0 && ep.n_ggroups > 0 && (ep.n_ggroups > mcap || (e->gtail_grid_cap > 0 && ep.n_ggroups > e->gtail_grid_cap))) {
+            tail_grid = std::min(ep.n_ggroups, group_tail_capacity(e, g.spl));
+            if (e->gtail_grid_cap > 0) tail_grid = std::min(tail_grid, e->gtail_grid_cap);
+        }
+        if (mcap > 0 && ep.n_ggroups > 0 && ep.n_ggroups <= mcap && tail_grid == 0) {
             int n = g.iter_hint[hp] > it ? g.iter_hint[hp] - it + RESIDENT_MARGIN : 2 * e->chunk_iters;
             n = std::max(2, std::min(n, GMULTI_MAX));
             if (e->chunk_explicit) n = std::min(n, std::max(e->chunk_iters, 2));
@@ -183,7 +219,7 @@
     hipLaunchKernelGGL((k_gsweep<SPL, GW, NVX, true, 2>), dim3(ep.n_ggroups), dim3(GNT), 0, e->stream, ep.grp_n_int, ep.gtab,   \
                        ep.n_ggroups, g.cnt + cur * GWM, e->gsweep_hot_rows, ep.out_col, g.x, g.x2, g.act[0], g.act[1], g.r, g.p, \
                        g.cnt + 3 * GWM, g.cnt + 4 * GWM, phase, eps, g.dstats + 1, rows, n, e->bar, status, e->persist_ticks,    \
-                       e->persist_rollcall_extra, owed ? 1 : 0, (int *)nullptr, (int *)nullptr)
+                       e->persist_rollcall_extra, owed ? 1 : 0, (int *)nullptr, (int *)nullptr, -1ll, LLONG_MAX, 0, 1)
             with_row(g.gw, [&](auto spl, auto gw) {
                 constexpr int SPL = decltype(spl)::value, GW = decltype(gw)::value;
                 if constexpr (SPL == 2) DPPR_LAUNCH_GMULTI(2, GW, 512);
@@ -230,25 +266,114 @@
             HIP_TRY(hipMemsetAsync(g.cnt + GWM, 0, sizeof(int) * 2 * GWM, e->stream));
             cur = 0;
             more = any_left(e->pinned + GWM + sweeps * GWM);
+            F_now = pairs_of(e->pinned + GWM + sweeps * GWM);
             continue;
         }
-        int n;
-        if (it == 0) {
-            int lo = 0;
-            for (int h : (push_thr > 0 ? g.dense_hist : g.iter_hist)[hp]) lo = h > 0 && (lo == 0 || h < lo) ? h : lo;
-            n = lo > 0 ? lo : e->chunk_iters;
-            follow = 4;
-        } else if (push_thr > 0 && !push_gave_up) {
-            long long F = 0;
-            for (int s = 0; s < GWM; ++s) F += e->pinned[cur * GWM + s];
-            n = 1;
-            for (long long f = F / 4; f > push_thr && n < e->chunk_iters; f /= 4) ++n;
+        auto chunk_after = [&](int at, long long F) {
+            int n;
+            if (at == 0) {
+                int lo = 0;
+                for (int h : (push_thr > 0 ? g.dense_hist : g.iter_hist)[hp]) lo = h > 0 && (lo == 0 || h < lo) ? h : lo;
+                n = lo > 0 ? lo : e->chunk_iters;
+                follow = 4;
+            } else if (push_thr > 0 && !push_gave_up) {
+                n = 1;
+                for (long long f = F / 4; f > push_thr && n < e->chunk_iters; f /= 4) ++n;
+            } else {
+                n = std::min(follow, e->chunk_iters);
+                follow *= 2;
+            }
+            if (e->chunk_explicit) n = std::min(n, std::max(e->chunk_iters, 1));
+            return std::max(1, std::min(n, MAX_CHUNK));
+        };
+        if (it >= rb_next) rb_next = it + chunk_after(it, F_now);
+        if (tail_grid > 0 && F_now <= tail_thr) {
+            int n = GMULTI_MAX;
+            if (e->chunk_explicit) n = std::min(n, std::max(e->chunk_iters, 2));
+            n = std::max(2, std::min(n, e->max_iters - it + 1));
+            const bool lo_on = push_thr > 0 && !push_gave_up;
+            HIP_TRY(hipMemsetAsync(g.mlog, 0, sizeof(int) * (size_t)(n + 2) * GWM, e->stream));
+            HIP_TRY(hipMemsetAsync(e->bar, 0, sizeof(GridBar), e->stream));
+            if (e->profiling) HIP_TRY(hipEventRecord(e->evpool[0], e->stream));
+            int *status = g.mlog, *rows = g.mlog + GWM;
+#define DPPR_LAUNCH_GTAIL(SPL, GW, NVX)                                                                                  \
+    hipLaunchKernelGGL((k_gsweep<SPL, GW, NVX, true, 3>), dim3(tail_grid), dim3(GNT), 0, e->stream, ep.grp_n_int, ep.gtab,      \
+                       ep.n_ggroups, g.cnt + cur * GWM, e->gsweep_hot_rows, ep.out_col, g.x, g.x2, g.act[0], g.act[1], g.r, g.p, \
+                       g.cnt + 3 * GWM, g.cnt + 4 * GWM, phase, eps, g.dstats, rows, n, e->bar, status, e->persist_ticks,        \
+                       e->persist_rollcall_extra, owed ? 1 : 0, (int *)nullptr, (int *)nullptr, lo_on ? push_thr : -1ll, tail_thr, \
+                       rb_next - it, std::max(1, std::min(e->chunk_iters, MAX_CHUNK)))
+            with_row(g.gw, [&](auto spl, auto gw) {
+                constexpr int SPL = decltype(spl)::value, GW = decltype(gw)::value;
+                if constexpr (SPL == 2) DPPR_LAUNCH_GTAIL(2, GW, 512);
+                else if (nvx == 512) DPPR_LAUNCH_GTAIL(1, GW, 512);
+                else DPPR_LAUNCH_GTAIL(1, GW, 1024);
+            });
+#undef DPPR_LAUNCH_GTAIL
+            if (e->profiling) HIP_TRY(hipEventRecord(e->evpool[1], e->stream));
+            HIP_TRY(hipGetLastError());
+            HIP_TRY(hipMemcpyAsync(e->pinned, g.mlog, sizeof(int) * (size_t)(n + 2) * GWM, hipMemcpyDeviceToHost, e->stream));
+            HIP_TRY(loop_wait(e));
+            const int st = e->pinned[0];
+            g.tail_launches++;
+            if (st & GSM_FAULT) return fail(e, DPPR_ERR_HIP, "a grid barrier of the multi-sweep group launch timed out");
+            if (st & GSM_ABORTED) {
+                g.st.persist_aborts++;
+                e->persist_ok = false;
+                e->persist_retry = PERSIST_RETRY_BATCHES;
+                HIP_TRY(hipMemcpyAsync(e->pinned, g.cnt + cur * GWM, sizeof(int) * GWM, hipMemcpyDeviceToHost, e->stream));
+                HIP_TRY(loop_wait(e));
+                continue;
+            }
+            const int sweeps = st & GSM_SWEEPS;
+            for (int k = 0; k < sweeps; ++k) {
+                const long long F = pairs_of(e->pinned + GWM + k * GWM);
+                note_frontier(it + k, F);
+                g.st.iterations++;
+                g.st.pull_iterations++;
+                g.tail_sweeps++;
+                g.st.sum_F += F;
+                active_iters = it + k + 1;
+            }
+            if (e->profiling) {
+                float ms = 0;
+                HIP_TRY(hipEventElapsedTime(&ms, e->evpool[0], e->evpool[1]));
+                g.tail_ms += ms;
+                if (trace) {
+                    fprintf(stderr, "[gtail ] phase %d sweeps %3d..%3d  %7.1f us  (%.1f per sweep)  frontier pairs", phase, it, it + sweeps - 1, ms * 1e3,
+                            ms * 1e3 / std::max(sweeps, 1));
+                    for (int k = 0; k <= sweeps; ++k) fprintf(stderr, " %lld", pairs_of(e->pinned + GWM + k * GWM));
+                    fprintf(stderr, "\n");
+                }
+            }
+            if (sweeps & 1) {
+                std::swap(g.x, g.x2);
+                std::swap(g.act[0], g.act[1]);
+                owed = !owed;
+            }
+            rb_next = lo_on ? it + e->pinned[1] : it + sweeps;
+            it += sweeps;
+            F_now = (st & GSM_CONVERGED) ? 0 : pairs_of(e->pinned + GWM + sweeps * GWM);
+            more = F_now > 0;
+            if (more) {
+                HIP_TRY(hipMemcpyAsync(g.cnt, g.cnt + 3 * GWM, sizeof(int) * GWM, hipMemcpyDeviceToDevice, e->stream));
+                HIP_TRY(hipMemsetAsync(g.cnt + GWM, 0, sizeof(int) * 2 * GWM, e->stream));
+                cur = 0;
+            }
         } else {
-            n = std::min(follow, e->chunk_iters);
-            follow *= 2;
-        }
-        if (e->chunk_explicit) n = std::min(n, std::max(e->chunk_iters, 1));
-        n = std::max(1, std::min(n, MAX_CHUNK));
+        int n = rb_next - it;
+        if (tail_grid > 0) {
+            int m = n;
+            if (first_chunk) {
+                int lo = 0;
+                for (int h : g.tail_hist[hp]) lo = h > 0 && (lo == 0 || h < lo) ? h : lo;
+                if (lo > it) m = lo - it;
+            } else {
+                m = 1;
+                for (long long f = F_now / 4; f > tail_thr && m < e->chunk_iters; f /= 4) ++m;
+            }
+            n = std::max(1, std::min(n, m));
+        }
+        first_chunk = false;
         for (int k = 0; k < n; ++k) {
             const int nxt = (cur + 1) % 3, zer = (cur + 2) % 3;
             if (e->profiling) HIP_TRY(hipEventRecord(e->evpool[2 * k], e->stream));
@@ -257,7 +382,8 @@
     hipLaunchKernelGGL((k_gsweep<SPL, GW, NVX, false, CM>), dim3(sweep_grid), dim3(GNT), 0, e->stream, ep.grp_n_int, ep.gtab,  \
                        ep.n_ggroups, g.cnt + cur * GWM, e->gsweep_hot_rows, ep.out_col, g.x, g.x2, g.act[0], g.act[1], g.r, g.p,  \
                        g.cnt + nxt * GWM, g.cnt + zer * GWM, phase, eps, g.dstats + 1, log + k * GWM, 1, (GridBar *)nullptr,      \
-                       (int *)nullptr, 0ull, 0, owed ? 1 : 0, g.gq + (g.gq_seq % 3) * GQ_PAD, g.gq + ((g.gq_seq + 1) % 3) * GQ_PAD)
+                       (int *)nullptr, 0ull, 0, owed ? 1 : 0, g.gq + (g.gq_seq % 3) * GQ_PAD, g.gq + ((g.gq_seq + 1) % 3) * GQ_PAD, \
+                       -1ll, LLONG_MAX, 0, 1)
             with_row(g.gw, [&](auto spl, auto gw) {
                 constexpr int SPL = decltype(spl)::value, GW = decltype(gw)::value;
                 if constexpr (SPL == 2) DPPR_LAUNCH_GSWEEP(2, GW, 512);
@@ -280,11 +406,7 @@
         for (int k = 0; k < n; ++k) {
             const int *f = e->pinned + 5 * GWM + k * GWM;
             if (!any_left(f)) continue;
-            if (push_thr > 0 && dense_len < 0) {
-                long long F = 0;
-                for (int s = 0; s < GWM; ++s) F += f[s];
-                if (F <= push_thr) dense_len = it + k;
-            }
+            note_frontier(it + k, pairs_of(f));
             g.st.iterations++;
             g.st.pull_iterations++;
             for (int s = 0; s < GWM; ++s) g.st.sum_F += f[s];
@@ -297,7 +419,6 @@
                 g.st.push_launches++;
                 g.st.sweep_ms += ms;
                 g.st.sweep_launches++;
-                static const bool trace = getenv("DPPR_GROUP_TRACE") != nullptr;
                 if (trace) {
                     long long F = 0;
                     for (int s = 0; s < GWM; ++s) F += f[s];
@@ -307,9 +428,10 @@
         }
         more = any_left(e->pinned + cur * GWM);
         it += n;
-        if (more && push_thr > 0 && !push_gave_up) {
-            long long F = 0;
-            for (int s = 0; s < GWM; ++s) F += e->pinned[cur * GWM + s];
+        F_now = pairs_of(e->pinned + cur * GWM);
+        }
+        if (more && push_thr > 0 && !push_gave_up && it >= rb_next) {
+            const long long F = F_now;
             if (F <= push_thr) {
                 if (dense_len < 0) dense_len = it;
                 int pushed = 0;
@@ -319,12 +441,14 @@
                 if (entered) {
                     active_iters = it + pushed;
                     it += pushed;
+                    rb_next = it;
                     if (conv) more = false;
                     else {
                         cur = 0;
                         HIP_TRY(hipMemcpyAsync(e->pinned, g.cnt, sizeof(int) * GWM, hipMemcpyDeviceToHost, e->stream));
                         HIP_TRY(loop_wait(e));
                         more = any_left(e->pinned);
+                        F_now = pairs_of(e->pinned);
                         push_thr = std::max<long long>(F / 8, 1);
                         dense_len = -1;
                     }
@@ -338,6 +462,10 @@
     if (push_thr > 0) {
         for (int k = 3; k > 0; --k) g.dense_hist[hp][k] = g.dense_hist[hp][k - 1];
         g.dense_hist[hp][0] = dense_len >= 0 ? std::max(dense_len, 1) : std::max(active_iters, 1);
+    }
+    if (tail_thr > 0) {
+        for (int k = 3; k > 0; --k) g.tail_hist[hp][k] = g.tail_hist[hp][k - 1];
+        g.tail_hist[hp][0] = tail_start >= 0 ? std::max(tail_start, 1) : std::max(active_iters, 1);
     }
     g.iter_hint[hp] = active_iters;
     for (int k = 3; k > 0; --k) g.iter_hist[hp][k] = g.iter_hist[hp][k - 1];
diff --git a/dynamicppr_amd/csrc/dppr_host_state.hpp b/dynamicppr_amd/csrc/dppr_host_state.hpp
--- a/dynamicppr_amd/csrc/dppr_host_state.hpp
+++ b/dynamicppr_amd/csrc/dppr_host_state.hpp
@@ -132,9 +132,12 @@
     DevBuf<int> mlog;
     DevBuf<IterStats> dstats;
     dppr_stats_t st{};
+    int64_t tail_launches = 0, tail_sweeps = 0;
+    double tail_ms = 0;
     int iter_hint[2] = {0, 0};
     int iter_hist[2][4] = {{0, 0, 0, 0}, {0, 0, 0, 0}};
     int dense_hist[2][4] = {{0, 0, 0, 0}, {0, 0, 0, 0}};
+    int tail_hist[2][4] = {{0, 0, 0, 0}, {0, 0, 0, 0}};
     DevBuf<int> plist[2];
     DevBuf<int> ppre;
     DevBuf<GPushCtl> pctl;
@@ -220,6 +223,10 @@
     int gsweep_grid_cap = 0;
     bool group_resident = true;
     int gmulti_cap[2] = {-1, -1};
+    int gtail_cap[2] = {-1, -1};
+    int gtail_enter_pairs = -1;
+    int gtail_grid_cap = 0;
+    int gtail_auto_div = 8;
     bool any_groups = false;
     int ggroups_min = 256;
     bool force_radix_grouping = false;
diff --git a/dynamicppr_amd/csrc/dppr_multi.hpp b/dynamicppr_amd/csrc/dppr_multi.hpp
--- a/dynamicppr_amd/csrc/dppr_multi.hpp
+++ b/dynamicppr_amd/csrc/dppr_multi.hpp
@@ -243,16 +243,18 @@
 constexpr int GSM_FAULT = 1 << 29;
 constexpr int GSM_CONVERGED = 1 << 28;
 constexpr int GSM_SWEEPS = (1 << 16) - 1;
+constexpr int GM_HDR = 64;
 
 template <int SPL, int GW, int NVX, bool MULTI, int CM>
-__global__ __launch_bounds__(GNT, MULTI ? 4 : 8) void k_gsweep(int V, const int *__restrict__ gtab, int n_groups,
+__global__ __launch_bounds__(GNT, CM == 2 ? 4 : 8) void k_gsweep(int V, const int *__restrict__ gtab, int n_groups,
                                                    const int *cnt_in, int hot_rows,
                                                    const int *__restrict__ out_col, double *x_a, double *x_b,
                                                    uint32_t *act_a, uint32_t *act_b, double *r, double *p, int *cnt_out,
                                                    int *cnt_zero, int phase, double eps, IterStats *__restrict__ stats,
                                                    int *log_slot, int n_iter, GridBar *bar, int *status,
                                                    unsigned long long limit_ticks, int rollcall_extra, int credit0,
-                                                   int *q_take, int *q_zero) {
+                                                   int *q_take, int *q_zero, long long stop_lo, long long stop_hi, int rb_first,
+                                                   int rb_cap) {
     constexpr int NOCT = GNT / OCT, WORDS = NVX / 32, XS = x_stride(GW);
     static_assert(sizeof(double) * NVX * GW <= 64 * 1024, "two workgroups per CU");
     constexpr int EB = 8;
@@ -261,8 +263,9 @@
 #define DPPR_GS_FU (4 / SPL)
 #endif
     constexpr int FU_WANT = CM == 0 && SPL == 2 ? 2 * (DPPR_GS_FU) : (DPPR_GS_FU);
-    constexpr int FU = MULTI ? NVX / NOCT : FU_WANT <= NVX / NOCT ? FU_WANT : NVX / NOCT;
-    static_assert(MULTI == (CM == 2), "the multi-sweep form decides per sweep, a one-sweep launch is compiled for its mode");
+    constexpr bool OWN = CM == 3;
+    constexpr int FU = CM == 2 ? NVX / NOCT : FU_WANT <= NVX / NOCT ? FU_WANT : NVX / NOCT;
+    static_assert(MULTI == (CM >= 2), "the multi-sweep forms decide per sweep, a one-sweep launch is compiled for its mode");
     static_assert(NVX % NOCT == 0 && (NVX / NOCT) % FU == 0, "vertex phase covers the group in whole steps");
     __shared__ double s_acc[NVX * GW];
     __shared__ int s_cstart[NVX + 1];
@@ -273,6 +276,7 @@
     __shared__ unsigned long long s_edges;
     __shared__ int s_flag[2];
     __shared__ int s_ticket;
+    __shared__ int s_hdr[OWN ? GM_HDR : 1][GT_HDR];
     const int tid0 = threadIdx.x, lane = lane_id(), w = wave_id();
     const int j = tid0 & (OCT - 1);
     auto opaque = [](int v) {
@@ -372,10 +376,92 @@
         const int *H = gtab + (size_t)blockIdx.x * STRIDE;
         hv0 = H[0]; hnv = H[1]; hE0 = H[2]; hEg = H[3]; hper = H[4];
     }
-    int sweeps_done = 0;
+    if constexpr (OWN) {
+        for (int k = tid0; k < GM_HDR * GT_HDR; k += GNT) {
+            const long long gk = (long long)blockIdx.x + (long long)(k / GT_HDR) * (long long)G;
+            if (gk < (long long)n_groups) s_hdr[k / GT_HDR][k % GT_HDR] = gtab[(size_t)gk * STRIDE + k % GT_HDR];
+        }
+    }
+    int sweeps_done = 0, rb_next = rb_first;
     bool converged = false, fault = false;
+    auto sweep_head = [&](int it) -> int {
+        const int *row = it == 0 ? cnt_in : log_slot + (size_t)it * GS_MAX;
+        const int f = lane < GW ? (int)gs_ldu<true>(reinterpret_cast<const uint32_t *>(row + lane)) : 0;
+        if (it == 0 && blockIdx.x == 0 && tid0 < GW) log_slot[tid0] = f;
+        if (__ballot(f != 0) == 0) return 1;
+        if (it == 0) return 0;
+        long long F = 0;
+#pragma unroll
+        for (int s = 0; s < GW; ++s) F += (long long)__builtin_amdgcn_readlane(f, s);
+        if (F > stop_hi) return 2;
+        if (it == rb_next) {
+            if (F <= stop_lo) return 2;
+            int n = 1;
+            for (long long q = F / 4; q > stop_lo && n < rb_cap; q /= 4) ++n;
+            rb_next += n;
+        }
+        return 0;
+    };
+    auto sweep_tail = [&](int it) -> bool {
+#pragma unroll
+        for (int q = 0; q < SPL; ++q) {
+            if (nleg[q]) atomicAdd(&s_cnt[j * SPL + q], nleg[q]);
+            nleg[q] = 0;
+        }
+        asm volatile("s_waitcnt vmcnt(0)" ::: "memory");
+        __syncthreads();
+        if (MULTI && it == 12) STAMP(5);
+        if (tid0 < GW) {
+            if (s_cnt[tid0])
+                __hip_atomic_fetch_add(log_slot + (size_t)(it + 1) * GS_MAX + tid0, s_cnt[tid0], __ATOMIC_RELAXED,
+                                       __HIP_MEMORY_SCOPE_AGENT);
+            s_cnt[tid0] = 0;
+        }
+        if (w == 0) {
+            asm volatile("s_waitcnt vmcnt(0)" ::: "memory");
+            if (lane < BAR_REPS)
+                __hip_atomic_fetch_add(&bar->sub[it & 1][lane][blockIdx.x % BAR_SUBS].w, 1ull << 32, __ATOMIC_RELAXED,
+                                       __HIP_MEMORY_SCOPE_AGENT);
+            const unsigned long long rounds = (unsigned long long)((it >> 1) + 1);
+            unsigned polls = 0;
+            const unsigned long long t_start = wall_clock64();
+            bool ok = true;
+            for (;;) {
+                const unsigned long long word = lane < (int)subs_used ? bar_load(&bar->sub[it & 1][my_rep][lane].w) : 0;
+                if (__ballot((word >> 32) >= n_sub * rounds) == ~0ull) break;
+                if ((polls++ & 63u) == 63u && wall_clock64() - t_start > limit_ticks + 100000000ull) {
+                    ok = false;
+                    break;
+                }
+                __builtin_amdgcn_s_sleep(BAR_POLL_SLEEP);
+            }
+            if (lane == 0 && !ok) s_flag[1] = 1;
+        }
+        __syncthreads();
+        if (MULTI && it == 12) STAMP(6);
+        return s_flag[1] == 0;
+    };
+    for (int it_o = 0; it_o < (OWN ? n_iter : 1); ++it_o) {
+    if constexpr (OWN) {
+        const int what = sweep_head(it_o);
+        if (what) {
+            converged = what == 1;
+            break;
+        }
+    }
     for (int g = blockIdx.x; g < n_groups;) {
         __syncthreads();
+        if constexpr (OWN) {
+            const int k = (g - (int)blockIdx.x) / (int)G;
+            if (k < GM_HDR) {
+                hv0 = __builtin_amdgcn_readfirstlane(s_hdr[k][0]); hnv = __builtin_amdgcn_readfirstlane(s_hdr[k][1]);
+                hE0 = __builtin_amdgcn_readfirstlane(s_hdr[k][2]); hEg = __builtin_amdgcn_readfirstlane(s_hdr[k][3]);
+                hper = __builtin_amdgcn_readfirstlane(s_hdr[k][4]);
+            } else {
+                const int *H = gtab + (size_t)g * STRIDE;
+                hv0 = H[0]; hnv = H[1]; hE0 = H[2]; hEg = H[3]; hper = H[4];
+            }
+        }
         int ticket = 0, g_next = n_groups;
         if (!MULTI && tid0 == 0) ticket = (int)gridDim.x + atomicAdd(q_take, 1);
         const int *T = gtab + (size_t)g * STRIDE;
@@ -389,7 +475,7 @@
             const int c0 = tid < NVX ? T[GT_HDR + tid] : 0;
             const int os = tid < NOCT ? T[GT_HDR + NVX + 1 + tid] : 0;
             const unsigned short cv = tid < NVX ? reinterpret_cast<const unsigned short *>(T + GT_HDR + NVX + 1 + NOCT)[tid] : 0;
-            if (tid < WORDS) s_actin[tid] = tid * 32 < nv ? gs_ldu<MULTI>(act_a + (v0 >> 5) + tid) : 0u;
+            if (tid < WORDS) s_actin[tid] = tid * 32 < nv ? gs_ldu<MULTI>(((OWN && (it_o & 1)) ? act_b : act_a) + (v0 >> 5) + tid) : 0u;
             if (tid < NVX) {
                 s_cstart[tid] = c0;
                 s_cvid[tid] = cv;
@@ -400,24 +486,23 @@
         int mycol = e_begin + j < e_end ? ld_stream(&cols[e_begin + j]) : -1;
         int ncol = e_begin + EB + j < e_end ? ld_stream(&cols[e_begin + EB + j]) : -1;
 
-        for (int it = 0; it < (MULTI ? n_iter : 1); ++it) {
+        for (int it_i = 0; it_i < (CM == 2 ? n_iter : 1); ++it_i) {
+            const int it = OWN ? it_o : it_i;
             const double *x = (it & 1) ? x_b : x_a;
             double *x_new = (it & 1) ? x_a : x_b;
             const uint32_t *act_in = (it & 1) ? act_b : act_a;
             uint32_t *act_out = (it & 1) ? act_a : act_b;
-            const bool credit = CM == 2 ? ((credit0 ^ it) & 1) != 0 : CM == 1;
-            if constexpr (MULTI) {
-                const int *row = it == 0 ? cnt_in : log_slot + (size_t)it * GS_MAX;
-                const int f = lane < GW ? (int)gs_ldu<true>(reinterpret_cast<const uint32_t *>(row + lane)) : 0;
-                if (it == 0 && blockIdx.x == 0 && tid < GW) log_slot[tid] = f;
-                if (__ballot(f != 0) == 0) {
-                    converged = true;
+            const bool credit = CM >= 2 ? ((credit0 ^ it) & 1) != 0 : CM == 1;
+            if constexpr (CM == 2) {
+                const int what = sweep_head(it);
+                if (what) {
+                    converged = what == 1;
                     break;
                 }
             }
 #define GSTAMP(i) do { if (MULTI ? it == 12 : stamp_dense) STAMP(i); } while (0)
             GSTAMP(0);
-            if (it > 0) {
+            if (it_i > 0) {
                 if (tid < WORDS) s_actin[tid] = tid * 32 < nv ? gs_ldu<MULTI>(act_in + (v0 >> 5) + tid) : 0u;
                 mycol = e_begin + j < e_end ? ld_stream(&cols[e_begin + j]) : -1;
                 ncol = e_begin + EB + j < e_end ? ld_stream(&cols[e_begin + EB + j]) : -1;
@@ -613,52 +698,26 @@
                 s_actout[tid] = 0u;
                 s_touched[tid] = 0u;
             }
-            if constexpr (MULTI) {
-#pragma unroll
-                for (int q = 0; q < SPL; ++q) {
-                    if (nleg[q]) atomicAdd(&s_cnt[j * SPL + q], nleg[q]);
-                    nleg[q] = 0;
-                }
-                asm volatile("s_waitcnt vmcnt(0)" ::: "memory");
-                __syncthreads();
-                GSTAMP(5);
-                if (tid < GW) {
-                    if (s_cnt[tid])
-                        __hip_atomic_fetch_add(log_slot + (size_t)(it + 1) * GS_MAX + tid, s_cnt[tid], __ATOMIC_RELAXED,
-                                               __HIP_MEMORY_SCOPE_AGENT);
-                    s_cnt[tid] = 0;
-                }
-                if (w == 0) {
-                    asm volatile("s_waitcnt vmcnt(0)" ::: "memory");
-                    if (lane < BAR_REPS)
-                        __hip_atomic_fetch_add(&bar->sub[it & 1][lane][blockIdx.x % BAR_SUBS].w, 1ull << 32, __ATOMIC_RELAXED,
-                                               __HIP_MEMORY_SCOPE_AGENT);
-                    const unsigned long long rounds = (unsigned long long)((it >> 1) + 1);
-                    unsigned polls = 0;
-                    const unsigned long long t_start = wall_clock64();
-                    bool ok = true;
-                    for (;;) {
-                        const unsigned long long word = lane < (int)subs_used ? bar_load(&bar->sub[it & 1][my_rep][lane].w) : 0;
-                        if (__ballot((word >> 32) >= n_sub * rounds) == ~0ull) break;
-                        if ((polls++ & 63u) == 63u && wall_clock64() - t_start > limit_ticks + 100000000ull) {
-                            ok = false;
-                            break;
-                        }
-                        __builtin_amdgcn_s_sleep(BAR_POLL_SLEEP);
-                    }
-                    if (lane == 0 && !ok) s_flag[1] = 1;
-                }
-                __syncthreads();
-                GSTAMP(6);
+            if constexpr (CM == 2) {
+                const bool ok = sweep_tail(it);
                 sweeps_done = it + 1;
-                if (s_flag[1]) {
+                if (!ok) {
                     fault = true;
                     break;
                 }
             }
         }
-        if constexpr (MULTI) break;
-        g = g_next;
+        if constexpr (CM == 2) break;
+        g = OWN ? g + (int)G : g_next;
+    }
+    if constexpr (OWN) {
+        const bool ok = sweep_tail(it_o);
+        sweeps_done = it_o + 1;
+        if (!ok) {
+            fault = true;
+            break;
+        }
+    }
     }
     const int tid = tid0;
     if constexpr (MULTI) {
@@ -668,8 +727,10 @@
             cnt_out[tid] = f;
             cnt_zero[tid] = 0;
         }
-        if (blockIdx.x == 0 && tid == 0)
-            *status = sweeps_done | (fault ? GSM_FAULT : 0) | (converged ? GSM_CONVERGED : 0);
+        if (blockIdx.x == 0 && tid == 0) {
+            status[0] = sweeps_done | (fault ? GSM_FAULT : 0) | (converged ? GSM_CONVERGED : 0);
+            status[1] = rb_next;
+        }
         if (ecount) atomicAdd(&s_edges, (unsigned long long)ecount);
         __syncthreads();
         if (tid == 0 && s_edges) stats->blk_E[blockIdx.x] += s_edges;
diff --git a/dynamicppr_amd/engine.py b/dynamicppr_amd/engine.py
--- a/dynamicppr_amd/engine.py
+++ b/dynamicppr_amd/engine.py
@@ -54,6 +54,7 @@
     "dppr_bench_line_fills", "dppr_bench_stream_copy", "dppr_build_id", "dppr_heartbeat", "dppr_slide_concurrent", "dppr_renumbering_due", "dppr_debug_bin_tables",
     "dppr_debug_grouping", "dppr_topk", "dppr_group_topk", "dppr_read_at", "dppr_group_read_at", "dppr_debug_live_bytes",
     "dppr_group_sources", "dppr_group_replace_source", "dppr_group_add_source", "dppr_group_remove_source",
+    "dppr_set_group_tail", "dppr_group_tail_stats",
 ]
 
 
@@ -80,6 +81,8 @@
     L.dppr_set_incremental_graph.argtypes = [vp, C.c_int]
     L.dppr_set_renumbering.argtypes = [vp, C.c_int, C.c_int, C.c_int]
     L.dppr_set_group_push.argtypes = [vp, C.c_int, C.c_int, C.c_int64]
+    L.dppr_set_group_tail.argtypes = [vp, C.c_int64, C.c_int]
+    L.dppr_group_tail_stats.argtypes = [vp, C.c_int32, i64p, i64p, dp]
     L.dppr_id_space.argtypes = [vp, C.POINTER(C.c_int32), C.POINTER(C.c_int32), C.POINTER(C.c_int32), C.POINTER(C.c_int64)]
     L.dppr_set_tuning.argtypes = [vp, C.c_int, C.c_int, C.c_int, C.c_int, C.c_int]
     L.dppr_set_persistent.argtypes = [vp, C.c_int, C.c_int64]
@@ -160,7 +163,7 @@
 
     def __init__(self, V, W, directed, max_batch, n_epochs=1, device=0, schedule=SCHEDULE_EAGER,
                  hub_min_degree=None, big_row_edges=None, pull_min_frontier=None, chunk_iters=None, pull_block=None,
-                 persistent=None, persist_timeout_us=None, sweep_bitmap=None, binned=None, merge_phases=None, variant=None, group_at_slide=None, resident_slots=None, resident_update=None):
+                 persistent=None, persist_timeout_us=None, sweep_bitmap=None, binned=None, merge_phases=None, variant=None, group_at_slide=None, resident_slots=None, resident_update=None, group_tail=None):
         self._L = lib()
         self._h = C.c_void_p()
         self._batch_len, self._staged_len = {0: 0}, 0
@@ -191,6 +194,8 @@
             args = (binned,) if isinstance(binned, int) else tuple(binned)
             args = tuple(int(a) for a in args) + (0,) * (7 - len(args))
             self._ck(self._L.dppr_set_binned_sweep(self._h, *args), "set_binned_sweep")
+        if group_tail is not None:
+            self.set_group_tail(*((group_tail,) if isinstance(group_tail, int) else tuple(group_tail)))
         if persistent is not None or persist_timeout_us is not None:
             self._ck(self._L.dppr_set_persistent(self._h, 1 if persistent is None else int(persistent),
                                                  int(persist_timeout_us or 0)), "set_persistent")
@@ -248,6 +253,9 @@
     def set_group_push(self, enter_pairs=-1, list_cap=0, max_edges=0):
         self._ck(self._L.dppr_set_group_push(self._h, int(enter_pairs), int(list_cap), int(max_edges)), "set_group_push")
 
+    def set_group_tail(self, enter_pairs=-1, grid_cap=0):
+        self._ck(self._L.dppr_set_group_tail(self._h, int(enter_pairs), int(grid_cap)), "set_group_tail")
+
     def set_renumbering(self, on, growth_pct=0, min_parked=0):
         self._ck(self._L.dppr_set_renumbering(self._h, int(on), int(growth_pct), int(min_parked)), "set_renumbering")
 
@@ -468,7 +476,9 @@
     def group_stats(self, group):
         st = Stats()
         self._ck(self._L.dppr_group_stats(self._h, group, C.byref(st)), "group_stats")
-        return st.as_dict()
+        n, k, ms = C.c_int64(), C.c_int64(), C.c_double()
+        self._ck(self._L.dppr_group_tail_stats(self._h, group, C.byref(n), C.byref(k), C.byref(ms)), "group_tail_stats")
+        return dict(st.as_dict(), tail_launches=n.value, tail_sweeps=k.value, tail_ms=ms.value)
 
     def group_reset_stats(self, group):
         self._ck(self._L.dppr_group_reset_stats(self._h, group), "group_reset_stats")
diff --git a/include/dppr.h b/include/dppr.h
--- a/include/dppr.h
+++ b/include/dppr.h
@@ -113,6 +113,7 @@
 int dppr_group_read(dppr_engine *e, int32_t group, int32_t index, double *p, double *r);
 int dppr_group_stats(dppr_engine *e, int32_t group, dppr_stats_t *out);
 int dppr_group_reset_stats(dppr_engine *e, int32_t group);
+int dppr_group_tail_stats(dppr_engine *e, int32_t group, int64_t *launches, int64_t *sweeps, double *ms);
 
 int dppr_group_sources(dppr_engine *e, int32_t group, int32_t *out_sources , int32_t *out_n);
 int dppr_group_replace_source(dppr_engine *e, int32_t group, int32_t index, int32_t new_source, float *out_ms);
@@ -133,6 +134,8 @@
 int dppr_set_resident_slots(dppr_engine *e, int sorted);
 int dppr_set_resident_update(dppr_engine *e, int on);
 int dppr_set_group_push(dppr_engine *e, int enter_pairs, int list_cap, int64_t max_edges);
+
+int dppr_set_group_tail(dppr_engine *e, int64_t enter_pairs, int grid_cap);
 
 int dppr_set_group_seeding(dppr_engine *e, int from_tails);
 
```

Result: slower. 48.29 million (-12.6%).
